# tongxyh/ImageCompression_Adversarial

Measured on AMD Instinct MI355X. Metric: attack-step·images/sec, Balle2018-hyper 768×512 1001-step PGD, 1/2/4/8 GPU, higher is better.
Workload: dtype f32 (fp32-accurate: exact 3-way bf16 operand splits, 6 MFMA products, f32 accumulate); 1 GPU; attack_rd -m hyper -q 3 -att_metric L2 -noise 1e-4, 32 images/GPU of 768x512, steps of the 1001-step loop, x6 conv operands; per_gpu_batch=32, global_batch=32, height=512, width=768, parallelism=image-shard x1 (no data-path collective)

## Files before the change

imagecompression_adversarial_amd/_lib.py:

```python
from __future__ import annotations

import ctypes as C
import os

import torch

_HERE = os.path.dirname(os.path.abspath(__file__))
LIB_PATH = os.environ.get("ICA_HIP_LIB", os.path.join(_HERE, "libica_hip.so"))

_p = C.c_void_p
_i = C.c_int
_l = C.c_long
_f = C.c_float
_sz = C.c_size_t

_SIGS = {
    "ica_conv_it": [_i],
    "ica_pack_conv_weight_size": [_i, _i, _i, _i, _i],
    "ica_pack_conv_weight": [_p, _p, _i, _i, _i, _l, _l, _i, _i, _i, _i, _p],
    "ica_pack_conv_weight_bf16": [_p, _p, _i, _i, _i, _l, _l, _i, _i, _i, _p],
    "ica_pack_conv_weight_bf16_size": [_i, _i, _i, _i],
    "ica_pack_conv_weight_x6": [_p, _p, _i, _i, _i, _l, _l, _i, _i, _p],
    "ica_pack_conv_weight_x6_size": [_i, _i, _i, _i],
    "ica_pack_gdn_x6": [_p, _p, _i, _p],
    "ica_pack_gdn_x6_size": [_i],
    "ica_pack_up3k3_x6_size": [_i],
    "ica_pack_up3k3_x6": [_p, _p, _p, _i, _p],
    "ica_conv_up3k3_x6": [_p, _p, _p, _p, _i, _i, _i, _i, _i, _i, _p],
    "ica_conv_ex": [_p, _p],
    "ica_last_launch": [_p, _i, _p],
    "ica_x6_tiling": [_i],
    "ica_pack_gdn": [_p, _p, _p, _p, _i, _i, _f, _p],
    "ica_pack_gdn_bf16": [_p, _p, _p, _p, _i, _i, _f, _p],
    "ica_pack_up3_size": [_i],
    "ica_pack_up3": [_p, _p, _i, _i, _p],
    "ica_conv_up3": [_p, _p, _p, _p, _i, _i, _i, _i, _i, _i, _p],
    "ica_elem_blocks_per_image": [],
    "ica_nchw_to_nc4": [_p, _p, _i, _i, _i, _i, _p],
    "ica_nc4_to_nchw": [_p, _p, _i, _i, _i, _i, _p],
    "ica_reduce_rows": [_p, _p, _i, _i, _f, _p],
    "ica_attack_prologue": [_p, _p, _p, _p, _i, _i, _i, _f, _p],
    "ica_attack_prologue_ex": [_p, _p, _p, _p, _i, _i, _i, _f, _i, _p],
    "ica_attack_loss": [_p, _p, _p, _p, _i, _i, _i, _f, _i, _i, _p],
    "ica_attack_adam": [_p, _p, _p, _p, _p, _p, _p, _p, _i, _i, _i, _f, _f, _f, _f, _f, _p, _p, _p, _p],
    "ica_attack_adam_ex": [_p, _p, _p, _p, _p, _p, _p, _p, _i, _i, _i, _f, _f, _f, _f, _f, _p, _p, _p, _i, _p],
    "ica_universal_prologue": [_p, _p, _p, _p, _i, _i, _i, _f, _p],
    "ica_universal_adam": [_p, _p, _p, _p, _p, _p, _p, _i, _i, _i, _f, _f, _f, _f, _f, _p, _p, _p],
    "ica_branch_select": [_p, _f, _i, _p, _p, _p],
    "ica_gather_images": [_p, _p, _p, _i, _l, _p],
    "ica_roi_prologue": [_p, _p, _p, _p, _i, _i, _i, _f, _i, _i, _i, _i, _f, _f, _p],
    "ica_roi_loss": [_p, _p, _p, _p, _p, _i, _i, _i, _i, _i, _i, _i, _f, _f, _i, _p],
    "ica_roi_adam": [_p, _p, _p, _p, _p, _p, _p, _i, _i, _i, _f, _f, _f, _f, _p, _i, _i, _i, _i, _f, _f, _p, _p, _p],
    "ica_ifgsm_step": [_p, _p, _p, _p, _p, _i, _i, _i, _f, _f, _i, _p],
    "ica_l1_partial": [_p, _p, _i, _i, _i, _p],
    "ica_cw_gate": [_p, _i, _f, _p, _p, _p, _p, _i, _p],
    "ica_cw_adam": [_p, _p, _p, _p, _p, _p, _p, _i, _i, _i, _f, _f, _p, _i, _p, _i, _p],
    "ica_cw_round": [_p, _p, _p, _p, _p, _p, _i, _i, _i, _i, _p, _p],
    "ica_cw_reset": [_p, _p, _p, _p, _i, _l, _p],
    "ica_gc_likelihood": [_p, _p, _p, _p, _p, _p, _p, _i, _i, _i, _i, _i, _p],
    "ica_eb_likelihood": [_p, _p, _p, _p, _p, _p, _p, _i, _i, _i, _i, _i, _p],
    "ica_pack_eb": [_p, _p, _p, _i, _p],
    "ica_abs": [_p, _p, _l, _p],
    "ica_cast_f32_bf16": [_p, _p, _l, _p],
    "ica_cast_bf16_f32": [_p, _p, _l, _p],
    "ica_flip_rot": [_p, _p, _l, _i, _i, _i, _p],
    "ica_bitdepth": [_p, _p, _l, _f, _p],
    "ica_resample_axis": [_p, _p, _l, _i, _i, _i, _i, _p, _p, _p, _i, _p],
    "ica_bitdepth_noise": [_p, _p, _p, _l, _f, _p],
    "ica_bitdepth_noise_bwd": [_p, _p, _l, _f, _p],
    "ica_add": [_p, _p, _p, _l, _p],
    "ica_ensemble_grad": [_p, _p, _p, _l, _f, _p],
    "ica_latent_range": [_p, _i, _i, _i, _i, _p, _p, _p, _p],
    "ica_latent_clamp": [_p, _p, _p, _p, _i, _i, _i, _i, _p, _p],
    "ica_latent_clamp_bwd": [_p, _p, _p, _p, _i, _i, _i, _i, _p],
    "ica_latent_detect": [_p, _p, _p, _p, _p, _i, _i, _p],
    "ica_latent_distrib_ws_size": [_i, _i, _i, _i, _i],
    "ica_latent_distrib": [_p, _p, _p, _p, _i, _i, _i, _i, _f, _i, _f, _f, _p, _p, _p, _p, _p],
    "ica_layer_sums_blocks": [_i, _i, _i],
    "ica_layer_sums_ws_size": [_i, _i],
    "ica_layer_sums": [_p, _i, _i, _p, _p, _p],
    "ica_rate_gc_blocks": [],
    "ica_rate_eb_blocks": [_i, _i, _i],
    "ica_rate_gc": [_p, _p, _p, _p, _p, _i, _i, _i, _i, _f, _p],
    "ica_rate_eb": [_p, _p, _p, _p, _i, _i, _i, _i, _f, _p],
    "ica_rd_metrics_blocks": [],
    "ica_rd_metrics": [_p, _p, _p, _p, _p, _p, _p, _i, _i, _i, _i, _i, _i, _i, _i, _i, _p],
    "ica_val_metrics": [_p, _p, _p, _p, _p, _p, _i, _i, _i, _i, _i, _i, _i, _i, _i, _p],
    "ica_patch_vi_ws_size": [_i, _i, _i, _i, _i],
    "ica_patch_vi": [_p, _p, _p, _p, _i, _i, _i, _i, _i, _i, _p, _p, _p, _p, _p, _p, _p, _p],
    "ica_patch_gather": [_p, _p, _p, _p, _p, _p, _i, _i, _i, _i, _i, _p],
    "ica_blur_sweep_chunk": [],
    "ica_gauss_blur_ws_size": [_i, _i, _i],
    "ica_gauss_blur": [_p, _p, _p, _i, _i, _i, _i, _i, _i, _p, _p, _p, _p, _p],
    "ica_blur_sweep_ws_size": [_i, _i, _i],
    "ica_blur_sweep": [_p, _p, _p, _i, _i, _i, _i, _i, _i, _f, _i, _p, _l, _p, _p, _p, _p, _p],
    "ica_noise_apply_ws_size": [_i, _i, _i],
    "ica_noise_apply": [_p, _p, _p, _i, _i, _i, _p, _p, _p, _p],
    "ica_jpeg_sweep_chunk": [],
    "ica_jpeg_roundtrip_ws_size": [_i, _i, _i, _i],
    "ica_jpeg_roundtrip": [_p, _p, _i, _i, _i, _i, _p, _p, _p, _p, _p],
    "ica_jpeg_sweep_ws_size": [_i, _i, _i, _i],
    "ica_jpeg_sweep": [_p, _p, _i, _i, _i, _i, _i, _f, _i, _p, _l, _p, _p, _p, _p, _p],
    "ica_transfer_apply_ws_size": [_i, _i, _i, _i],
    "ica_transfer_apply": [_p, _p, _p, _i, _i, _i, _i, _p, _p, _p],
    "ica_transfer_score_ws_size": [_i, _i, _i, _i],
    "ica_transfer_score": [_p, _p, _i, _i, _i, _i, _i, _p, _p, _p],
    "ica_requant8_ws_size": [_i, _i, _i],
    "ica_requant8": [_p, _p, _p, _i, _i, _i, _p, _p, _p, _p, _p, _p, _p, _p, _p],
    "ica_quant8_pack": [_p, _i, _i, _i, _p, _p, _p],
    "ica_floor_bits_ws_size": [_i, _i, _i, _i],
    "ica_floor_bits": [_p, _i, _i, _i, _i, _f, _p, _p, _p],
    "ica_gc_symbols": [_p, _p, _p, _p, _i, _f, _p, _p, _i, _i, _i, _i, _p],
    "ica_eb_symbols": [_p, _p, _p, _p, _i, _i, _i, _i, _p],
    "ica_dequantize": [_p, _p, _p, _p, _i, _i, _i, _i, _p],
    "ica_pmf_to_quantized_cdf": [_p, _i, _i, _p],
    "ica_rans_encode": [_p, _p, _l, _p, _i, _p, _p, _i, _p, _l, _p],
    "ica_rans_decode": [_p, _l, _p, _l, _p, _i, _p, _p, _i, _p],
    "ica_rans_dec_open": [_p, _l, _p],
    "ica_rans_dec_step": [_p, _i, _p, _l, _p, _i, _p, _p, _i, _p, _p],
    "ica_rans_dec_close": [_p],
    "ica_ar_lds_bytes": [_i, _i, _i],
    "ica_ar_step": [_p, _i, _i, _i, _p],
    "ica_round": [_p, _p, _l, _p],
    "ica_clamp01": [_p, _p, _l, _p],
    "ica_sqdiff_partial": [_p, _p, _p, _i, _l, _i, _p],
    "ica_nc4_bound_to_nchw": [_p, _p, _i, _i, _i, _i, _p],
    "ica_bound_bwd_nc4": [_p, _p, _p, _i, _i, _i, _i, _p],
    "ica_msssim_blocks": [_i, _i, _i, _i],
    "ica_msssim_level": [_p, _p, _i, _i, _i, _p, _i, _i, _f, _f, _p, _p, _p, _p, _p],
    "ica_msssim_level_bwd": [_p, _p, _p, _i, _i, _i, _p, _i, _i, _p, _p, _p],
    "ica_msssim_combine": [_p, _i, _i, _i, _p, _p, _p, _p, _p],
    "ica_avgpool2": [_p, _p, _i, _i, _i, _i, _i, _p],
    "ica_avgpool2_bwd": [_p, _p, _i, _i, _i, _i, _i, _p],
    "ica_scale": [_p, _l, _f, _p],
    "ica_wgrad_ws_size": [_i, _i, _i, _i],
    "ica_wgrad_nsplit": [_i, _i, _l],
    "ica_wgrad": [_p, _p, _p, _p, _i, _i, _i, _i, _i, _i, _i, _i, _i, _i, _i, _i, _p],
    "ica_channel_sum": [_p, _p, _i, _i, _i, _i, _i, _p],
    "ica_relu_bwd": [_p, _p, _l, _p],
    "ica_abs_bwd": [_p, _p, _l, _p],
    "ica_gdn_xsq": [_p, _p, _p, _l, _p],
    "ica_lrelu_bwd": [_p, _p, _p, _l, _p],
    "ica_gdn_t": [_p, _p, _p, _p, _l, _i, _p],
    "ica_reparam_bwd": [_p, _p, _p, _l, _f, _i, _p],
    "ica_bpp_grad": [_p, _p, _l, _f, _p],
    "ica_gc_bwd": [_p, _p, _p, _p, _p, _i, _i, _i, _i, _p],
    "ica_eb_bwd": [_p, _p, _p, _p, _p, _i, _i, _i, _i, _p],
    "ica_eb_param_scatter": [_p, _p, _p, _i, _p],
    "ica_mse_grad": [_p, _p, _p, _i, _i, _i, _f, _p],
}
_RESTYPES = {"ica_pack_conv_weight_size": _sz, "ica_pack_conv_weight_bf16_size": _sz,
             "ica_pack_conv_weight_x6_size": _sz, "ica_pack_gdn_x6_size": _sz, "ica_pack_up3k3_x6_size": _sz, "ica_pack_up3_size": _sz, "ica_wgrad_ws_size": _sz,
             "ica_rans_encode": _l, "ica_ar_lds_bytes": _sz, "ica_patch_vi_ws_size": _sz,
             "ica_gauss_blur_ws_size": _sz, "ica_blur_sweep_ws_size": _sz, "ica_noise_apply_ws_size": _sz,
             "ica_transfer_apply_ws_size": _sz, "ica_transfer_score_ws_size": _sz,
             "ica_requant8_ws_size": _sz, "ica_floor_bits_ws_size": _sz, "ica_latent_distrib_ws_size": _sz,
             "ica_layer_sums_ws_size": _sz, "ica_jpeg_roundtrip_ws_size": _sz, "ica_jpeg_sweep_ws_size": _sz}



class ConvArgs(C.Structure):
    _fields_ = ([(n, C.c_void_p) for n in ("x", "y", "wp", "bias", "gp", "beta", "save_x", "save_s", "in_x", "in_s",
                                            "save_t", "res", "mask")]
                + [(n, C.c_int) for n in ("N", "Cin", "Hin", "Win", "Cout", "Hout", "Wout", "kind", "KS", "S", "epi",
                                           "it", "fill_mode", "ps", "prec", "layout", "order")])


class ArArgs(C.Structure):
    _fields_ = ([(n, C.c_void_p) for n in ("y", "params", "yhat", "sym", "idx", "sym_in", "means", "wc", "bc", "w1",
                                            "b1", "w2", "b2", "w3", "b3", "table")]
                + [("T", C.c_int), ("bound", C.c_float)]
                + [(n, C.c_int) for n in ("B", "M", "H", "W", "E1", "E2")])


class LayerDesc(C.Structure):
    _fields_ = [(n, C.c_void_p) for n in ("a", "b", "c")] + [(n, C.c_int) for n in ("C", "H", "W", "mode")]


_lib = None


def lib():
    global _lib
    if _lib is None:
        if not os.path.exists(LIB_PATH):
            raise RuntimeError(
                f"libica_hip.so not found at {LIB_PATH}: build it with "
                "`python -c 'import __graft_entry__ as g; g.build()'` (hipcc, gfx950). "
                "There is no CPU/PyTorch fallback for the hot path.")
        L = C.CDLL(LIB_PATH)
        for name, args in _SIGS.items():
            fn = getattr(L, name)
            fn.argtypes = args
            fn.restype = _RESTYPES.get(name, _i)
        _lib = L
    return _lib


def exported_symbols():
    return list(_SIGS)


def call(name, *args):
    rc = getattr(lib(), name)(*args)
    if rc != 0:
        raise RuntimeError(f"{name} failed with status {rc}")
    return rc


def ptr(t):
    return None if t is None else C.c_void_p(t.data_ptr())


def stream():
    return C.c_void_p(torch.cuda.current_stream().cuda_stream)
```

imagecompression_adversarial_amd/attack.py:

```python
from __future__ import annotations

import math
import os
import time
from dataclasses import dataclass, field

import torch

from . import dist as D
from . import hip_ops as K
from . import msssim as MS
from ._lib import call, ptr, stream
from .engine import CodecKernels


ATTACK_GRAPH = os.environ.get("ICA_ATTACK_GRAPH", "1") != "0"
GRAPH_STATS = {"captures": 0, "replays": 0}


def _lr_table(steps, lr):
    out, cur, sch = [], lr, 0
    period = max(steps // 3, 1)
    for i in range(steps):
        out.append(cur)
        if i % period == 0:
            sch += 1
            if sch in (1, 2, 3):
                cur = cur * 0.33
    return out


@dataclass
class AttackResult:
    im_adv: torch.Tensor
    output_adv: torch.Tensor
    output_s: torch.Tensor
    bpp_ori: torch.Tensor
    bpp: torch.Tensor
    mse_in: torch.Tensor
    mse_out: torch.Tensor
    msim_in: torch.Tensor | None
    msim_out: torch.Tensor | None
    vi: list = field(default_factory=list)
    vi_msim: list = field(default_factory=list)
    noise: torch.Tensor | None = None
    branches: list = field(default_factory=list)
    output_t: torch.Tensor | None = None
    tar_mse: torch.Tensor | None = None


def eval_forward(kern: CodecKernels, x: torch.Tensor, clamp=True):
    B, _, H, W = x.shape
    res = kern.forward(K.to_nc4(x))
    out = torch.empty_like(x)
    call("ica_nc4_bound_to_nchw", ptr(res["x_hat4"]), ptr(out), B, H, W, int(clamp), stream())
    return out, K.bits_to_bpp(res["sumlog"], H * W)


def padded_eval_forward(kern: CodecKernels, x: torch.Tensor, pad: int, mode="reflect"):
    import torch.nn.functional as F
    B, _, H, W = x.shape
    xp = F.pad(x, (pad, pad, pad, pad), mode=mode).contiguous()
    Hp, Wp = xp.shape[2:]
    if Hp % 64 or Wp % 64:
        raise ValueError(f"-p {pad}: the padded size {Hp}x{Wp} must be a multiple of 64 (the codec's latent grid; "
                         "the reference's crop fails otherwise)")
    out_p, bpp_p = eval_forward(kern, xp, True)
    out = out_p[:, :, pad:pad + H, pad:pad + W].contiguous()
    return out, bpp_p * (Hp * Wp / (H * W))


def evaluate(kern, im_in, im_s, output_s, clamp=True, adv=False, msssim=True):
    im_ = K.clamp01(im_in) if clamp else im_in
    out, bpp = eval_forward(kern, im_, clamp)
    mse_in = K.sqdiff_mean(im_, im_s)
    mse_out = K.sqdiff_mean(out, output_s)
    msim_in = msim_out = None
    if msssim:
        msim_in = MS.ms_ssim_per_image(im_, im_s)
        msim_out = MS.ms_ssim_per_image(out, output_s)
    vi, vi_msim = [], []
    mi_l, mo_l = mse_in.tolist(), mse_out.tolist()
    si_l = msim_in.tolist() if msssim else [None] * len(mi_l)
    so_l = msim_out.tolist() if msssim else [None] * len(mi_l)
    for mi, mo, si, so in zip(mi_l, mo_l, si_l, so_l):
        v = vm = None
        if mi > 1e-20 and mo > 1e-20:
            v = 10.0 * math.log10(mo / mi)
            if not adv and si is not None and si < 0.9999:
                vm = 10.0 * math.log10((1 - so) / (1 - si))
        vi.append(v)
        vi_msim.append(vm)
    return im_, out, bpp, mse_in, mse_out, msim_in, msim_out, vi, vi_msim


class AttackLoop:

    def __init__(self, kern: CodecKernels, im_s: torch.Tensor, steps=1001, epsilon=16.0, noise_thr=1e-4,
                 lr=0.01, att_metric="L2", clamp=True, init_noise=None, coupled=False, group=None,
                 target=None, roi=None, la_tar=1.0, la_bkg_in=1.0, la_bkg_out=1.0, pad=None, padding_mode="reflect"):
        if att_metric not in ("L2", "ms-ssim"):
            raise ValueError(f"att_metric {att_metric!r} not supported (reference: L2, ms-ssim)")
        if target is not None and (att_metric != "L2" or coupled):
            raise NotImplementedError("the targeted / ROI attack is defined for att_metric L2, per-image")
        self.kern = kern
        self.im_s = im_s.contiguous()
        B, C, H, W = im_s.shape
        assert C == 3
        self.B, self.H, self.W = B, H, W
        self.steps, self.eps, self.thr = steps, float(epsilon) / 255.0, float(noise_thr)
        self.metric, self.clamp = att_metric, clamp
        self.invN = float(1.0 / (3 * H * W))
        self.coupled, self.group = coupled, group
        self.B_global = D.global_count(B, im_s.device, group) if coupled else B
        self.gscale = float(1.0 / (self.B_global * 3 * H * W)) if coupled else self.invN
        self.dval = 1.0 / self.B_global if coupled else 1.0
        dev = im_s.device
        self.clamp_in = bool(getattr(kern, "clamp_input", True))
        if init_noise is not None:
            self.noise = init_noise.clone().contiguous()
        elif not self.clamp_in:
            r = float(noise_thr) ** 0.5
            self.noise = torch.empty(tuple(im_s.shape)).uniform_(-r, r).to(dev)
        else:
            self.noise = torch.zeros_like(self.im_s)
        if target is not None and not self.clamp_in:
            raise NotImplementedError("the targeted / ROI attack is defined for the clamped-input models")
        self.m = torch.zeros_like(self.im_s)
        self.v = torch.zeros_like(self.im_s)
        self.im_in4 = K.empty_nc4(B, 3, H, W, dev)
        self.part = torch.empty(B * K.blocks_per_image(), device=dev)
        self.loss_i = torch.empty(B, device=dev)
        self.grad4 = K.empty_nc4(B, 3, H, W, dev)
        self.branch = torch.zeros(B, dtype=torch.int32, device=dev)
        self.im_in = torch.empty_like(self.im_s)
        self.lrs = _lr_table(steps, lr)
        self.t = 0
        self.compact = True
        self.sel = torch.zeros(B + 1, dtype=torch.int32, device=dev)
        self.gpos = torch.zeros(B, dtype=torch.int32, device=dev)
        self.sel_host = torch.zeros(B + 1, dtype=torch.int32).pin_memory() if dev.type == "cuda" else None
        self._sel_ev = torch.cuda.Event() if dev.type == "cuda" else None
        self._sel_pending = False
        self.census = torch.zeros(B, dtype=torch.int32, device=dev)
        self.steps_done = 0
        self.sync_steps = 0
        self.sync_wait_s = 0.0
        self.graph_ok = (ATTACK_GRAPH and dev.type == "cuda" and att_metric == "L2"
                         and type(self).network_grad is AttackLoop.network_grad)
        self._graph, self._graph_out = None, None
        self.graph_replays = 0
        if pad:
            self.output_s, self.bpp_ori = padded_eval_forward(kern, self.im_s, int(pad), padding_mode)
        else:
            self.output_s, self.bpp_ori = eval_forward(kern, self.im_s, clamp)
        self.output_s4 = None
        self.roi = None
        if target is not None:
            t = target.to(self.im_s.device).contiguous()
            if t.shape[0] == 1 and B > 1:
                t = t.expand(B, -1, -1, -1).contiguous()
            if t.shape != self.im_s.shape:
                raise ValueError(f"target {tuple(t.shape)} must match the source batch {tuple(self.im_s.shape)}")
            self.output_t, _ = eval_forward(kern, t, True)
            self.roi = roi_weights(H, W, roi, la_tar, la_bkg_in, la_bkg_out)

    def _adam_scalars(self, i):
        t = i + 1
        bc1 = 1 - 0.9 ** t
        bc2 = 1 - 0.999 ** t
        step_size = self.lrs[i] / bc1
        return float(bc2 ** 0.5), float(-step_size)

    def _select(self):
        B = self.B
        if not self.compact:
            return B, None
        call("ica_branch_select", ptr(self.loss_i), self.thr, B, ptr(self.sel), ptr(self.gpos), stream())
        prev_all = False
        if self._sel_pending:
            self._sel_ev.synchronize()
            prev_all = int(self.sel_host[0]) == B
            self._sel_pending = False
        self.sel_host.copy_(self.sel, non_blocking=True)
        self._sel_ev.record()
        if prev_all and (self.metric == "L2" or self.roi is not None):
            self._sel_pending = True
            return B, None
        t0 = time.perf_counter()
        self._sel_ev.synchronize()
        self.sync_wait_s += time.perf_counter() - t0
        self.sync_steps += 1
        E = int(self.sel_host[0])
        if E == B:
            self._sel_pending = True
            return B, None
        return E, self.sel[1:1 + E]

    def _gather(self, x, idx, E):
        if idx is None:
            return x
        per = x[0].numel()
        out = torch.empty((E,) + tuple(x.shape[1:]), dtype=x.dtype, device=x.device)
        call("ica_gather_images", ptr(x), ptr(out), ptr(idx), E, per, stream())
        return out

    def network_grad(self, idx=None, E=None):
        kern = self.kern
        H, W = self.H, self.W
        Bn = self.B if idx is None else E
        im4 = self._gather(self.im_in4, idx, Bn)
        out_s = self._gather(self.output_s, idx, Bn)
        grad4, part = self.grad4[:Bn], self.part[:Bn * K.blocks_per_image()]
        y4, sa = kern.g_a(im4, save=True)
        del im4
        xh4, ss = kern.g_s(y4, save=True)
        del y4
        if self.roi is not None:
            x0, x1, y0, y1, _, _, wot, wob = self.roi
            out_t = self._gather(self.output_t, idx, Bn)
            call("ica_roi_loss", ptr(xh4), ptr(out_s), ptr(out_t), ptr(grad4), ptr(part),
                 Bn, H, W, x0, x1, y0, y1, wot, wob, int(self.clamp), stream())
        elif self.metric == "L2":
            call("ica_attack_loss", ptr(xh4), ptr(out_s), ptr(grad4), ptr(part), Bn, H, W,
                 self.gscale, int(self.clamp), 0, stream())
        else:
            out = torch.empty_like(out_s)
            call("ica_nc4_bound_to_nchw", ptr(xh4), ptr(out), Bn, H, W, int(self.clamp), stream())
            ones = torch.full((Bn,), self.dval, device=out.device)
            _, gout, _ = MS.ms_ssim_value_and_grad(out, out_s, ones)
            call("ica_bound_bwd_nc4", ptr(xh4), ptr(gout), ptr(grad4), Bn, H, W, int(self.clamp), stream())
        gy4 = kern.g_s_backward(grad4, ss)
        del ss, xh4
        return kern.g_a_backward(gy4, sa)

    def _network_graph(self):
        if self._graph is None:
            hooks = (K.EVENT_HOOK, K.LAUNCH_HOOK)
            K.EVENT_HOOK = K.LAUNCH_HOOK = None
            g = torch.cuda.CUDAGraph()
            try:
                with torch.cuda.graph(g, capture_error_mode="relaxed"):
                    out = self.network_grad(None, self.B)
            finally:
                K.EVENT_HOOK, K.LAUNCH_HOOK = hooks
            self._graph, self._graph_out = g, out
            GRAPH_STATS["captures"] += 1
        self._graph.replay()
        self.graph_replays += 1
        GRAPH_STATS["replays"] += 1
        return self._graph_out

    def step(self, i, record_im_in=False, census=False):
        B, H, W = self.B, self.H, self.W
        if self.roi is not None:
            return self._step_roi(i, record_im_in, census)
        call("ica_attack_prologue_ex", ptr(self.noise), ptr(self.im_s), ptr(self.im_in4), ptr(self.part), B, H, W,
             self.eps, int(self.clamp_in), stream())
        K.reduce_rows(self.part, B, self.invN, out=self.loss_i)
        if self.coupled:
            D.couple_loss_i(self.loss_i, self.B_global, self.group)
        E, idx = self._select()
        if E == B and idx is None and self.graph_ok:
            gx4 = self._network_graph()
        else:
            gx4 = self.network_grad(idx, E) if E > 0 else None
        cheap_grad = None
        if self.metric == "ms-ssim" and E < B:
            im_in = torch.empty_like(self.im_s)
            call("ica_nc4_bound_to_nchw", ptr(self.im_in4), ptr(im_in), B, H, W, 0, stream())
            _, _, gY = MS.ms_ssim_value_and_grad(self.im_s, im_in, torch.full((B,), -self.dval, device=im_in.device))
            cheap_grad = gY
        bc2s, neg_step = self._adam_scalars(i)
        call("ica_attack_adam_ex", ptr(self.noise), ptr(self.im_s), ptr(gx4), ptr(self.loss_i), ptr(cheap_grad),
             ptr(self.m), ptr(self.v), ptr(self.im_in if record_im_in else None), B, H, W, self.eps, self.thr,
             self.gscale, bc2s, neg_step, ptr(self.branch), ptr(self.gpos if idx is not None else None),
             ptr(self.census), int(self.clamp_in), stream())
        self.steps_done += 1
        if census:
            return self.branch.tolist()
        return None

    def _step_roi(self, i, record_im_in, census):
        B, H, W = self.B, self.H, self.W
        x0, x1, y0, y1, wit, wib, _, _ = self.roi
        call("ica_roi_prologue", ptr(self.noise), ptr(self.im_s), ptr(self.im_in4), ptr(self.part), B, H, W,
             self.eps, x0, x1, y0, y1, wit, wib, stream())
        K.reduce_rows(self.part, B, 1.0, out=self.loss_i)
        E, idx = self._select()
        if E == B and idx is None and self.graph_ok:
            gx4 = self._network_graph()
        else:
            gx4 = self.network_grad(idx, E) if E > 0 else None
        bc2s, neg_step = self._adam_scalars(i)
        call("ica_roi_adam", ptr(self.noise), ptr(self.im_s), ptr(gx4), ptr(self.loss_i), ptr(self.m), ptr(self.v),
             ptr(self.im_in if record_im_in else None), B, H, W, self.eps, self.thr, bc2s, neg_step,
             ptr(self.branch), x0, x1, y0, y1, wit, wib, ptr(self.gpos if idx is not None else None),
             ptr(self.census), stream())
        self.steps_done += 1
        if census:
            return self.branch.tolist()
        return None

    def expensive_image_steps(self):
        return self.B * self.steps_done - int(self.census.sum())

    def run(self, record=False):
        branches = []
        for i in range(self.steps):
            br = self.step(i, record_im_in=(i == self.steps - 1), census=record)
            if record:
                branches.append(br)
        return branches


def roi_weights(H, W, roi, la_tar=1.0, la_bkg_in=1.0, la_bkg_out=1.0):
    x0, x1, y0, y1 = (0, W, 0, H) if roi is None else (int(v) for v in roi)
    x0, x1 = max(0, min(x0, W)), max(0, min(x1, W))
    y0, y1 = max(0, min(y0, H)), max(0, min(y1, H))
    area = max(x1 - x0, 0) * max(y1 - y0, 0)
    if area == 0:
        raise ValueError(f"empty ROI {roi} for a {W}x{H} image")
    cnt_t, cnt_b = 3.0 * area, 3.0 * (H * W - area)
    wb = (lambda la: float(la / cnt_b) if cnt_b > 0 else 0.0)
    return (x0, x1, y0, y1, float(1.0 / cnt_t), wb(la_bkg_in), float(la_tar / cnt_t), wb(la_bkg_out))


def roi_mse(a, b, roi4):
    x0, x1, y0, y1 = roi4
    d = (a - b)[:, :, y0:y1, x0:x1]
    return (d * d).flatten(1).mean(1)


def attack_batch(kern: CodecKernels, im_s, steps=1001, epsilon=16.0, noise_thr=1e-4, lr=0.01, att_metric="L2",
                 clamp=True, init_noise=None, eval_msssim=True, record=False, coupled=False,
                 group=None, target=None, roi=None, la_tar=1.0, la_bkg_in=1.0, la_bkg_out=1.0, pad=None,
                 padding_mode="reflect") -> AttackResult:
    loop = AttackLoop(kern, im_s, steps, epsilon, noise_thr, lr, att_metric, clamp, init_noise, coupled, group,
                      target, roi, la_tar, la_bkg_in, la_bkg_out, pad, padding_mode)
    branches = loop.run(record=record)
    im_, out, bpp, mse_in, mse_out, msim_in, msim_out, vi, vi_msim = evaluate(
        kern, loop.im_in, loop.im_s, loop.output_s, clamp, adv=False, msssim=eval_msssim)
    res = AttackResult(im_adv=im_, output_adv=out, output_s=loop.output_s, bpp_ori=loop.bpp_ori, bpp=bpp,
                       mse_in=mse_in, mse_out=mse_out, msim_in=msim_in, msim_out=msim_out, vi=vi, vi_msim=vi_msim,
                       noise=loop.noise, branches=branches)
    if loop.roi is not None:
        res.output_t = loop.output_t
        res.tar_mse = roi_mse(out, loop.output_t, loop.roi[:4])
    return res


RATE_MODELS = ("hyper", "factorized")


def rate_attack_guard(model=None, precision=None, att_metric="L2", coupled=False, target=None, roi=None):
    if coupled:
        raise NotImplementedError("the rate attack is per-image: the batch-coupled semantics belong to the "
                                  "adversarial fine-tune's distortion attack")
    if target is not None or roi is not None:
        raise NotImplementedError("the rate attack has no target / ROI form: its loss is the whole image's bitrate")
    if att_metric != "L2":
        raise NotImplementedError(f"the rate attack's input budget is the L2 one (att_metric {att_metric!r}): its "
                                  "cheap branch is the L2 input loss, its expensive branch uses no image metric")
    if precision == "bf16":
        raise NotImplementedError("the rate attack runs fp32 / x6 operands: the entropy models read an fp32 latent")
    if model is not None and model not in RATE_MODELS:
        raise NotImplementedError(f"the rate attack covers {RATE_MODELS}, not {model!r}: the rounding inside the "
                                  "context models (and the debug model's mean-scale prior) has no stated relaxation")


class RateAttackLoop(AttackLoop):

    def __init__(self, kern: CodecKernels, im_s: torch.Tensor, steps=1001, epsilon=16.0, noise_thr=1e-4, lr=0.01,
                 att_metric="L2", clamp=True, init_noise=None, coupled=False, group=None, target=None, roi=None,
                 pad=None, padding_mode="reflect"):
        model = kern.model if isinstance(kern, CodecKernels) else type(kern).__name__
# ... 86 lines not shown
```

imagecompression_adversarial_amd/csrc/ica_conv.hip:

```cpp
#include <cxxabi.h>

#include <algorithm>
#include <cstdio>
#include <cstdlib>
#include <type_traits>

#include "ica_conv_epi.h"

#define ICA_WLOAD_BF(w, it, g) ((w)[(it) * 64])

template <int IT, int KH>
ICA_DEV void load_frag(float (&a)[IT][KH], const float* w) {
#pragma unroll
  for (int it = 0; it < IT; ++it) {
    if constexpr (KH == 8) {
      const f32x4 w0 = ld4(w + it * 64 * KH), w1 = ld4(w + it * 64 * KH + 4);
#pragma unroll
      for (int e = 0; e < 4; ++e) {
        a[it][e] = w0[e];
        a[it][4 + e] = w1[e];
      }
    } else {
      const f32x2 w0 = *reinterpret_cast<const f32x2*>(w + it * 64 * KH);
      a[it][0] = w0[0];
// ... 1132 lines not shown
        }
#pragma unroll
        for (int it = 0; it < 3; ++it) {
          const float* wt = wl + ((size_t)it * nch + ch) * 512;
          const f32x4 w0 = ld4(wt), w1 = ld4(wt + 4);
#pragma unroll
          for (int e = 0; e < 4; ++e) {
            a[it][e] = w0[e];
            a[it][4 + e] = w1[e];
          }
        }
      };
      auto compute = [&](const f32x4& v0, const f32x4& v1, const float (&a)[3][8]) {
        const float b[8] = {v0[0], v0[1], v0[2], v0[3], v1[0], v1[1], v1[2], v1[3]};
#pragma unroll
        for (int s2 = 0; s2 < 8; ++s2)
#pragma unroll
          for (int it = 0; it < 3; ++it) acc[it] = mfma32(a[it][s2], b[s2], acc[it]);
      };
      f32x4 pa0, pa1, pb0, pb1;
      float aa[3][8], ab[3][8];
      load(0, pa0, pa1, aa);
      int ch = 0;
#pragma unroll 1
      for (; ch + 1 < nch; ch += 2) {
        load(ch + 1, pb0, pb1, ab);
        compute(pa0, pa1, aa);
        load(min(ch + 2, nch - 1), pa0, pa1, aa);
        compute(pb0, pb1, ab);
      }
      if (ch < nch) compute(pa0, pa1, aa);
    }
    if (q < T3_NPX) {
#pragma unroll
      for (int it = 0; it < 3; ++it)
#pragma unroll
        for (int r = 0; r < 16; ++r) {
          const int row = it * 32 + acc_row(r, h);
          if (row < T3_ROWS) zs[row * T3_NPX + q] = acc[it][r];
        }
    }
  }
gather:
  __syncthreads();
  const int al = threadIdx.x / T3_TW, bl = threadIdx.x % T3_TW;
  const int a = a0 + al, b = b0 + bl;
  if (al >= T3_TH || a >= p.Hin || b >= p.Win) return;
  const float bias0 = p.bias ? p.bias[0] : 0.f, bias1 = p.bias ? p.bias[1] : 0.f, bias2 = p.bias ? p.bias[2] : 0.f;
#pragma unroll
  for (int py = 0; py < 2; ++py) {
#pragma unroll
    for (int px = 0; px < 2; ++px) {
      float o0 = 0.f, o1 = 0.f, o2 = 0.f;
#pragma unroll
      for (int ky = py; ky < 5; ky += 2) {
#pragma unroll
        for (int kx = px; kx < 5; kx += 2) {
          const int dy = (py + 2 - ky) / 2, dx = (px + 2 - kx) / 2;
          const int q = (al + 1 + dy) * T3_HC + (bl + 1 + dx);
          const int tap = ky * 5 + kx;
          o0 += zs[(0 * 25 + tap) * T3_NPX + q];
          o1 += zs[(1 * 25 + tap) * T3_NPX + q];
          o2 += zs[(2 * 25 + tap) * T3_NPX + q];
        }
      }
      const int y = 2 * a + py, x = 2 * b + px;
      if (y < p.Hout && x < p.Wout)
        st4(p.y + (((size_t)n * p.Hout + y) * p.Wout + x) * 4, f32x4{o0 + bias0, o1 + bias1, o2 + bias2, 0.f});
    }
  }
}

constexpr int U3_OW = 30, U3_HW = 32;
template <int CT>
constexpr int u3_rows() { return 4 * CT - 2; }
template <int CT>
constexpr int u3_npx() { return 4 * CT * U3_HW; }

template <int NCH, int CT, bool BF = false>
__global__ __launch_bounds__(256, 1) void conv_up3_x6p_kernel(ConvParams p) {
  constexpr int R = u3_rows<CT>(), NPX = u3_npx<CT>();
  __shared__ float zs[T3_ROWS * NPX];
  const int tiles_x = (p.Win + U3_OW - 1) / U3_OW, tiles_y = (p.Hin + R - 1) / R;
  const int total = tiles_x * tiles_y * p.N;
  const int nb = (int)(gridDim.x >> 3), xcd = (int)(blockIdx.x & 7), bi = (int)(blockIdx.x >> 3);
  const int q8 = total >> 3, r8 = total & 7;
  const int t_end = xcd * q8 + min(xcd, r8) + q8 + (xcd < r8 ? 1 : 0);
  const int t_begin = xcd * q8 + min(xcd, r8) + bi;
  if (t_begin >= t_end) return;
  const int lane = threadIdx.x & 63, h = lane >> 5, j = lane & 31;
  const int wave = __builtin_amdgcn_readfirstlane(threadIdx.x >> 6);
  const int Cin4 = p.Cin >> 2;
  const unsigned plane = (unsigned)p.Hin * p.Win;
  auto coords = [&](int t, int& n, int& a0, int& b0) {
    const int tx = t % tiles_x, r = t / tiles_x;
    a0 = (r % tiles_y) * R;
    b0 = tx * U3_OW;
    n = r / tiles_y;
  };
  const bool split_in = (p.pl & PL_IN) != 0;
  constexpr unsigned QB = BF ? 8u : 16u;
  const unsigned qs = plane * QB, cs = 4u * qs;
  constexpr unsigned OOB = 0xFFFFFFF0u;
  auto prep = [&](int t, bool real, __amdgpu_buffer_rsrc_t& r, unsigned (&vb)[CT]) __attribute__((always_inline)) {
    int n, a0, b0;
    coords(real ? t : t_begin, n, a0, b0);
    r = uniform_rsrc(reinterpret_cast<const char*>(p.x) + (size_t)n * Cin4 * plane * QB, (unsigned)(Cin4 * plane * QB));
    const int ix = b0 - 1 + j;
#pragma unroll
    for (int ct = 0; ct < CT; ++ct) {
      const int iy = a0 - 1 + wave + 4 * ct;
      const bool ok = real && iy >= 0 && iy < p.Hin && ix >= 0 && ix < p.Win;
      vb[ct] = ok ? ((unsigned)(2 * h) * plane + pix_at(iy, ix, p.Hin, p.Win, split_in)) * QB : OOB;
    }
  };
  f32x4 xa[CT][NCH][BF ? 1 : 2];
  auto load = [&](const __amdgpu_buffer_rsrc_t& r, const unsigned (&vb)[CT], int ct, int ch)
      __attribute__((always_inline)) {
    const bool ok = vb[ct] != OOB;
    const unsigned o = vb[ct] + (unsigned)ch * cs;
    if constexpr (BF) {
      const u32x2 lo = __builtin_bit_cast(u32x2, __builtin_amdgcn_raw_buffer_load_b64(r, ok ? o : OOB, 0, 0));
      const u32x2 hi = __builtin_bit_cast(u32x2, __builtin_amdgcn_raw_buffer_load_b64(r, ok ? o + qs : OOB, 0, 0));
      xa[ct][ch][0] = __builtin_bit_cast(f32x4, (u32x4_t){lo[0], lo[1], hi[0], hi[1]});
    } else {
      xa[ct][ch][0] = __builtin_bit_cast(f32x4, __builtin_amdgcn_raw_buffer_load_b128(r, ok ? o : OOB, 0, 0));
      xa[ct][ch][BF ? 0 : 1] = __builtin_bit_cast(f32x4, __builtin_amdgcn_raw_buffer_load_b128(r, ok ? o + qs : OOB, 0, 0));
    }
  };
  __amdgpu_buffer_rsrc_t rn;
  unsigned vbn[CT];
  prep(t_begin, true, rn, vbn);
#pragma unroll
  for (int ct = 0; ct < CT; ++ct)
#pragma unroll
    for (int ch = 0; ch < NCH; ++ch) load(rn, vbn, ct, ch);
  constexpr long pst = 3L * NCH * 64;
  constexpr int NPL = BF ? 1 : 3;
  const __amdgpu_buffer_rsrc_t wr = uniform_rsrc(p.wp, (unsigned)(NPL * pst * 16));
  int wz = 0;
  auto ldw = [&](bf16x8 (&a)[3][3], int ch) {
#pragma unroll
    for (int it = 0; it < 3; ++it)
#pragma unroll
      for (int q = 0; q < NPL; ++q) a[it][q] = ld_bf8(wr, lane * 16, wz + (int)((q * pst + ((long)it * NCH + ch) * 64) * 16));
  };
  auto split = [&](int ct, int ch, bf16x8 (&b)[3]) __attribute__((always_inline)) {
    if constexpr (BF) {
      b[0] = f4_as_bf8(xa[ct][ch][0]);
    } else {
      const float v[8] = {xa[ct][ch][0][0], xa[ct][ch][0][1], xa[ct][ch][0][2], xa[ct][ch][0][3],
                          xa[ct][ch][BF ? 0 : 1][0], xa[ct][ch][BF ? 0 : 1][1], xa[ct][ch][BF ? 0 : 1][2],
                          xa[ct][ch][BF ? 0 : 1][3]};
      split3x8(v, b);
    }
  };
  const float bias0 = p.bias ? p.bias[0] : 0.f, bias1 = p.bias ? p.bias[1] : 0.f, bias2 = p.bias ? p.bias[2] : 0.f;
#pragma unroll 1
  for (int t = t_begin; t < t_end; t += nb) {
    wz = 0;
    asm volatile("" : "+s"(wz));
    prep(t + nb, t + nb < t_end, rn, vbn);
    f32x16 acc[CT][3];
#pragma unroll
    for (int ct = 0; ct < CT; ++ct)
#pragma unroll
      for (int it = 0; it < 3; ++it) acc[ct][it] = f32x16{0};
    bf16x8 wa[2][3][3];
    ldw(wa[0], 0);
    bf16x8 bc[3];
    split(0, 0, bc);
#pragma unroll
    for (int ch = 0; ch < NCH; ++ch) {
      if (ch + 1 < NCH) ldw(wa[(ch + 1) & 1], ch + 1);
      __builtin_amdgcn_sched_barrier(0);
#pragma unroll
      for (int ct = 0; ct < CT; ++ct) {
        const int nct = ct + 1 < CT ? ct + 1 : 0, nch = ct + 1 < CT ? ch : ch + 1;
        bf16x8 bn[3];
        if (nch < NCH) split(nct, nch, bn);
#pragma unroll
// ... 459 lines not shown
        case EPI_RELU: return launch_up<5, 4, EPI_RELU, 0>(p, st);
        case EPI_LRELU: return launch_up<5, 4, EPI_LRELU, 0>(p, st);
        case EPI_GDN: return launch_up<5, 4, EPI_GDN, 0>(p, st);
        case EPI_IGDN: return launch_up<5, 4, EPI_IGDN, 0>(p, st);
        case EPI_GDN_BWD: return launch_up<5, 4, EPI_GDN_BWD, 0>(p, st);
        case EPI_IGDN_BWD: return launch_up<5, 4, EPI_IGDN_BWD, 0>(p, st);
        default: return -5;
      }
    }
    return -3;
  }
  if (epi != EPI_BIAS || (fx & ~FX_RES) != 0) return -4;
  if (KS == 3) {
    if (fx == 0) {
      if (it == 1) return launch_up<3, 1, EPI_BIAS, 0>(p, st);
      if (it == 4) return launch_up<3, 4, EPI_BIAS, 0>(p, st);
      if (it == 6) return launch_up<3, 6, EPI_BIAS, 0>(p, st);
    } else {
      if (it == 1) return launch_up<3, 1, EPI_BIAS, FX_RES>(p, st);
      if (it == 4) return launch_up<3, 4, EPI_BIAS, FX_RES>(p, st);
      if (it == 6) return launch_up<3, 6, EPI_BIAS, FX_RES>(p, st);
    }
    return -3;
  }
  if (KS == 1) {
    if (fx != 0) return -4;
    if (it == 1) return launch_up<1, 1, EPI_BIAS, 0>(p, st);
    if (it == 4) return launch_up<1, 4, EPI_BIAS, 0>(p, st);
    if (it == 6) return launch_up<1, 6, EPI_BIAS, 0>(p, st);
    return -3;
  }
  return -6;
}

int ica_conv_x6_dispatch(const ConvParams& p, int kind, int KS, int S, int it, int epi, int fx, int order,
                         hipStream_t st);
int ica_rgb5_bf16_dispatch(const ConvParams& p, int epi, hipStream_t st);
int ica_pack_rgb5_planes(const float* w, void* dst, int O, int C, long so, long sc, int it, int planes, hipStream_t st);

extern "C" {
#ifdef ICA_CLOCK_STAMP
int ica_diag_stamp_buffer(unsigned long long* buf, unsigned slots) {
  if (hipMemcpyToSymbol(HIP_SYMBOL(ica_stamp_buf), &buf, sizeof(buf)) != hipSuccess) return -1;
  if (hipMemcpyToSymbol(HIP_SYMBOL(ica_stamp_slots), &slots, sizeof(slots)) != hipSuccess) return -1;
  return 0;
}
#endif

int ica_last_launch(char* name, int cap, unsigned long long* threads) {
  const IcaLaunchRec r = ica_launch_rec();
  ica_launch_rec() = IcaLaunchRec{nullptr, 0, 0};
  if (!r.fn) return 0;
  if (threads) *threads = r.threads;
  if (name && cap > 0) {
    const char* m = hipKernelNameRefByPtr(r.fn, nullptr);
    int st = -1;
    char* d = m ? abi::__cxa_demangle(m, nullptr, nullptr, &st) : nullptr;
    const char* src = (st == 0 && d) ? d : (m ? m : "");
    std::snprintf(name, (size_t)cap, "%s", src);
    std::free(d);
  }
  return r.count;
}

typedef struct ica_conv_args {
  const float* x;
  float* y;
  const float* wp;
  const float* bias;
  const float* gp;
  const float* beta;
  float* save_x;
  float* save_s;
  const float* in_x;
  const float* in_s;
  float* save_t;
  const float* res;
  const float* mask;
  int N, Cin, Hin, Win, Cout, Hout, Wout;
  int kind, KS, S, epi, it, fill_mode, ps;
  int prec;
  int layout;
  int order;
} ica_conv_args;

int ica_conv_it(int cout) {
  if (cout <= 32) return 1;
  if (cout % 128 == 0) return 4;
  if (cout % 96 == 0) return 3;
  return 4;
}

static inline int resolve_it(int O, int it) { return it > 0 ? it : ica_conv_it(O); }

size_t ica_pack_conv_weight_size(int O, int C, int KS, int CC, int it) {
  const int IT = resolve_it(O, it);
  const int ncb = (O + IT * 32 - 1) / (IT * 32);
  const int C4 = (C + 3) / 4, nch = (C4 * 4 + CC - 1) / CC;
  return (size_t)ncb * nch * KS * KS * IT * 64 * (CC / 2);
}

int ica_pack_conv_weight(const float* w, float* dst, int O, int C, int KS, long so, long sc, int CC, int order,
                         int flip, int it, hipStream_t st) {
  const int IT = resolve_it(O, it);
  const long total = (long)ica_pack_conv_weight_size(O, C, KS, CC, IT);
  ICA_LAUNCH(pack_conv_kernel<float>, dim3((total + 255) / 256), dim3(256), 0, st, w, dst, O, C, KS, so, sc,
                     IT, CC, order, total, flip);
  ICA_CHECK_LAUNCH();
  return 0;
}

__global__ void pack_conv_tg_kernel(const float* __restrict__ w, __bf16* __restrict__ dst, int O, int C, int KS,
                                    long so, long sc, int IT, long total, int flip) {
  const long i = (long)blockIdx.x * blockDim.x + threadIdx.x;
  if (i >= total) return;
  const int KK = KS * KS, TG = (KK + 3) / 4;
  long t = i;
  const int s = t % 8; t /= 8;
  const int lane = t % 64; t /= 64;
  const int it = t % IT; t /= IT;
  const int tg = t % TG; t /= TG;
  const int cb = (int)t;
  const int o = cb * IT * 32 + it * 32 + (lane & 31);
  const int tap = 4 * tg + 2 * (lane >> 5) + (s >> 2), c = s & 3;
  float v = 0.f;
  if (o < O && c < C && tap < KK) {
    const int wt = flip ? KK - 1 - tap : tap;
    v = w[o * so + c * sc + (wt / KS) * KS + (wt % KS)];
  }
  dst[i] = (__bf16)v;
}

size_t ica_pack_conv_weight_bf16_size(int O, int C, int KS, int it) {
  if (C > 4) return ica_pack_conv_weight_size(O, C, KS, 16, it);
  const int IT = resolve_it(O, it);
  const int ncb = (O + IT * 32 - 1) / (IT * 32);
  return (size_t)ncb * ((KS * KS + 3) / 4) * IT * 64 * 8;
}

int ica_pack_conv_weight_bf16(const float* w, void* dst, int O, int C, int KS, long so, long sc, int order, int flip,
                              int it, hipStream_t st) {
  const int IT = resolve_it(O, it);
  if (C <= 4) {
    if (order == 2) {
      if (KS != 5 || flip) return -4;
      return ica_pack_rgb5_planes(w, dst, O, C, so, sc, IT, 1, st);
    }
    if (order != 0) return -4;
    const long tot = (long)ica_pack_conv_weight_bf16_size(O, C, KS, IT);
    ICA_LAUNCH(pack_conv_tg_kernel, dim3((tot + 255) / 256), dim3(256), 0, st, w, reinterpret_cast<__bf16*>(dst),
                       O, C, KS, so, sc, IT, tot, flip);
    ICA_CHECK_LAUNCH();
    return 0;
  }
  const long total = (long)ica_pack_conv_weight_size(O, C, KS, 16, IT);
  ICA_LAUNCH(pack_conv_kernel<__bf16>, dim3((total + 255) / 256), dim3(256), 0, st, w,
                     reinterpret_cast<__bf16*>(dst), O, C, KS, so, sc, IT, 16, order, total, flip);
  ICA_CHECK_LAUNCH();
  return 0;
}

size_t ica_pack_up3_size(int Cin) { return (size_t)3 * (Cin / 16) * 64 * 8; }

int ica_pack_up3(const float* w, void* dst, int Cin, int prec, hipStream_t st) {
  if (Cin % 16 != 0) return -2;
  if (prec < 0 || prec > 2) return -4;
  const long total = (long)ica_pack_up3_size(Cin);
  const dim3 grid((total + 255) / 256), block(256);
  if (prec == 0) {
    ICA_LAUNCH(pack_up3_kernel<float>, grid, block, 0, st, w, reinterpret_cast<float*>(dst), Cin, total);
  } else if (prec == 1) {
    ICA_LAUNCH(pack_up3_kernel<__bf16>, grid, block, 0, st, w, reinterpret_cast<__bf16*>(dst), Cin, total);
  } else {
    ICA_LAUNCH(pack_up3_x6_kernel, grid, block, 0, st, w, reinterpret_cast<__bf16*>(dst), Cin, total);
  }
  ICA_CHECK_LAUNCH();
  return 0;
}

static int up3_layout_ok(int layout, int Hin, int Win) {
  if (layout & ~PL_IN) return -4;
  if ((layout & PL_IN) && ((Hin | Win) & 1)) return -2;
  return 0;
}

int ica_conv_up3(const float* x, float* y, const void* wp, const float* bias, int N, int Cin, int Hin, int Win,
                 int layout, int prec, hipStream_t st) {
  if (Cin % 16 != 0) return -2;
  if (const int rc = up3_layout_ok(layout, Hin, Win)) return rc;
  if (prec < 0 || prec > 2) return -4;
  ConvParams p{x, y, reinterpret_cast<const float*>(wp), bias, nullptr, nullptr, nullptr, nullptr, nullptr, nullptr,
               N, Cin, Hin, Win, 3, 2 * Hin, 2 * Win, nullptr};
  p.pl = layout;
  auto tiled = [&](auto kern) {
    const int tiles = ((Win + T3_TW - 1) / T3_TW) * ((Hin + T3_TH - 1) / T3_TH) * N;
    ICA_LAUNCH(kern, dim3(tiles), dim3(256), 0, st, p);
  };
  auto persistent = [&](auto kern, int R) {
    const int tiles = ((Win + U3_OW - 1) / U3_OW) * ((Hin + R - 1) / R) * N;
    const int nb = std::max(1, std::min((tiles + 7) / 8, ica_cu_count() / 8));
    ICA_LAUNCH(kern, dim3(8 * nb), dim3(256), 0, st, p);
  };
  if (prec == 0) {
    tiled(conv_up3_kernel<false>);
  } else if (prec == 2) {
    if (Cin == 128) persistent(conv_up3_x6p_kernel<8, 3>, u3_rows<3>());
    else if (Cin == 192) persistent(conv_up3_x6p_kernel<12, 2>, u3_rows<2>());
    else tiled(conv_up3_kernel<false, true>);
  } else {
    if (Cin == 128) persistent(conv_up3_x6p_kernel<8, 3, true>, u3_rows<3>());
    else tiled(conv_up3_kernel<true>);
  }
  ICA_CHECK_LAUNCH();
  return 0;
}

__global__ void pack_gdn_bf16_kernel(const float* __restrict__ gamma, const float* __restrict__ beta,
                                     __bf16* __restrict__ gp, float* __restrict__ beta_eff, int C, int transpose,
                                     float beta_bound) {
  const int T = C / 32;
  const long total = (long)T * T * 2048;
  const long i = (long)blockIdx.x * blockDim.x + threadIdx.x;
  const float ped = 1.4551915228366852e-11f;
  const float gbound = 3.814697265625e-06f;
  if (i < total) {
    long t = i;
    const int j = t % 8; t /= 8;
    const int lane = t % 64; t /= 64;
    const int hl = t % 2; t /= 2;
    const int s = t % 2; t /= 2;
    const int b = t % T; t /= T;
    const int a = (int)t;
    const int row = a * 32 + (lane & 31), col = b * 32 + 16 * s + 8 * (j >> 2) + 4 * (lane >> 5) + (j & 3);
    const int gi = transpose ? (col * C + row) : (row * C + col);
    const float g0 = fmaxf(gamma[gi], gbound);
    const float g = fsub_rn(fmul_rn(g0, g0), ped);
    __bf16 hi, lo;
    split_bf(g, hi, lo);
    gp[i] = hl ? lo : hi;
  }
  if (i < C) {
    const float bb = fmaxf(beta[i], beta_bound);
    beta_eff[i] = fsub_rn(fmul_rn(bb, bb), ped);
  }
}

int ica_pack_gdn_bf16(const float* gamma, const float* beta, void* gpb, float* beta_eff, int C, int transpose,
                      float beta_bound, hipStream_t st) {
  if (C % 32 != 0) return -2;
  const long total = (long)(C / 32) * (C / 32) * 2048;
  ICA_LAUNCH(pack_gdn_bf16_kernel, dim3((total + 255) / 256), dim3(256), 0, st, gamma, beta,
                     reinterpret_cast<__bf16*>(gpb), beta_eff, C, transpose, beta_bound);
  ICA_CHECK_LAUNCH();
  return 0;
}

int ica_pack_gdn(const float* gamma, const float* beta, float* gp, float* beta_eff, int C, int transpose,
                 float beta_bound, hipStream_t st) {
  if (C % 32 != 0) return -2;
  const long total = (long)(C / 32) * (C / 32) * 64 * 16;
  ICA_LAUNCH(pack_gdn_kernel, dim3((total + 255) / 256), dim3(256), 0, st, gamma, beta, gp, beta_eff, C,
                     transpose, beta_bound);
  ICA_CHECK_LAUNCH();
  return 0;
}

int ica_conv_ex(const ica_conv_args* a, hipStream_t st) {
  ConvParams p{a->x,    a->y,    a->wp,   a->bias, a->gp,   a->beta, a->save_x, a->save_s, a->in_x, a->in_s,
               a->N,    a->Cin,  a->Hin,  a->Win,  a->Cout, a->Hout, a->Wout,   a->save_t, a->res,  a->mask,
               a->fill_mode, a->ps, a->prec, a->layout};
  if (a->prec < 0 || a->prec > 3) return -4;
  if (a->layout & ~(PL_IN | PL_OUT)) return -4;
  if (a->layout && (a->KS != 5 || a->S != 2 || a->fill_mode != 0 || a->ps)) return -4;
  if (((a->layout & PL_IN) && ((a->Hin | a->Win) & 1)) || ((a->layout & PL_OUT) && ((a->Hout | a->Wout) & 1)))
    return -2;
  const int it = resolve_it(a->Cout, a->it);
  if (a->epi >= EPI_GDN && a->epi <= EPI_IGDN_BWD && a->Cout != it * 32) return -4;
  if (a->ps && (a->Cout % 16 != 0 || !(a->epi == EPI_BIAS || a->epi == EPI_RELU || a->epi == EPI_LRELU))) return -4;
  if (a->fill_mode == 1 && !a->mask) return -4;
  if (a->fill_mode == 2 && a->Cin % 16 != 0) return -2;
  if (a->epi == EPI_LRELU_BWD && !a->in_x) return -4;
  const int fx = ((a->res || a->save_x) ? FX_RES : 0) | (a->ps ? FX_PS : 0) | (a->fill_mode == 1 ? FX_MASK : 0) |
                 (a->fill_mode == 2 ? FX_UNSHUF : 0) | (a->save_t ? FX_T : 0);
  const int want = a->kind == 1 ? ORDER_UP : ORDER_DOWN;
  if (a->prec == 2) {
    if (a->kind == 0 && a->KS == 3)
      return a->order == want ? pick_x6o<3>(p, a->kind, a->KS, a->S, a->epi, it, fx, st) : -4;
    return ica_conv_x6_dispatch(p, a->kind, a->KS, a->S, it, a->epi, fx, a->order, st);
  }
  if (a->prec == 3) return a->order == want ? pick_x6o<1>(p, a->kind, a->KS, a->S, a->epi, it, fx, st) : -4;
  if (a->prec == 1 && a->order == ORDER_RGB5) {
    if (a->kind != 0 || a->KS != 5 || a->S != 2 || it != 4 || fx != 0 || a->fill_mode != 0 ||
        !(a->epi == EPI_BIAS || a->epi == EPI_GDN || a->epi == EPI_IGDN_BWD))
      return -4;
    return ica_rgb5_bf16_dispatch(p, a->epi, st);
  }
  if (a->order != (a->prec == 1 && a->kind == 0 && a->Cin <= 4 ? ORDER_TG : want)) return -4;
  if (a->kind == 0) return pick_down(p, a->KS, a->S, it, a->epi, fx, st);
  if (a->kind == 1) return a->S == 2 ? pick_up(p, a->KS, it, a->epi, fx, st) : -6;
  return -6;
}

}
```

imagecompression_adversarial_amd/csrc/ica_conv_epi.h:

```cpp
#pragma once
#include "ica_common.h"

enum {
  EPI_BIAS = 0,
  EPI_RELU = 1,
  EPI_GDN = 2,
  EPI_IGDN = 3,
  EPI_GDN_BWD = 4,
  EPI_IGDN_BWD = 5,
  EPI_LRELU = 6,
  EPI_LRELU_BWD = 7,
};
enum { FX_RES = 1, FX_PS = 2, FX_MASK = 4, FX_UNSHUF = 8, FX_T = 16 };

struct ConvParams {
  const float* x;
  float* y;
  const float* wp;
  const float* bias;
  const float* gp;
  const float* beta;
  float* save_x;
  float* save_s;
  const float* in_x;
  const float* in_s;
  int N, Cin, Hin, Win, Cout, Hout, Wout;
  float* save_t;
  const float* res;
  const float* mask;
  int fill_mode;
  int ps;
  int prec;
  int pl;
};
enum { PL_IN = 1, PL_OUT = 2 };
enum { ORDER_DOWN = 0, ORDER_UP = 1, ORDER_RGB5 = 2, ORDER_TG = 3 };

ICA_DEV void split3(f32x4 v, u32x2& hi, u32x2& mid, u32x2& lo) {
  bf16x4 a, b, c;
#pragma unroll
  for (int e = 0; e < 4; ++e) {
    const __bf16 h = (__bf16)v[e];
    const float r1 = v[e] - (float)h;
    const __bf16 m = (__bf16)r1;
    const float r2 = r1 - (float)m;
    a[e] = h;
    b[e] = m;
    c[e] = (__bf16)r2;
  }
  hi = __builtin_bit_cast(u32x2, a);
  mid = __builtin_bit_cast(u32x2, b);
  lo = __builtin_bit_cast(u32x2, c);
}

ICA_DEV f32x16 mfma_x6(const bf16x8 (&a)[3], const bf16x8 (&b)[3], f32x16 c) {
  c = mfma32bf(a[2], b[0], c);
  c = mfma32bf(a[0], b[2], c);
  c = mfma32bf(a[1], b[1], c);
  c = mfma32bf(a[1], b[0], c);
  c = mfma32bf(a[0], b[1], c);
  c = mfma32bf(a[0], b[0], c);
  return c;
}
template <int NPL>
ICA_DEV f32x16 mfma_np(const bf16x8 (&a)[3], const bf16x8 (&b)[3], f32x16 c) {
  if constexpr (NPL == 1) return mfma32bf(a[0], b[0], c);
  else return mfma_x6(a, b, c);
}

ICA_DEV __amdgpu_buffer_rsrc_t chan_rsrc(const float* v, int C) { return uniform_rsrc(v, v ? (unsigned)((C + 3) & ~3) * 4u : 0u); }
ICA_DEV f32x4 ld_chan4(__amdgpu_buffer_rsrc_t r, int c0) {
  return __builtin_bit_cast(f32x4, __builtin_amdgcn_raw_buffer_load_b128(r, c0 * 4, 0, 0));
}

ICA_DEV void split3x8(const float (&v)[8], bf16x8 (&o)[3]) {
  u32x2 a0, b0, c0, a1, b1, c1;
  split3(f32x4{v[0], v[1], v[2], v[3]}, a0, b0, c0);
  split3(f32x4{v[4], v[5], v[6], v[7]}, a1, b1, c1);
  o[0] = __builtin_bit_cast(bf16x8, u32x4_t{a0[0], a0[1], a1[0], a1[1]});
  o[1] = __builtin_bit_cast(bf16x8, u32x4_t{b0[0], b0[1], b1[0], b1[1]});
  o[2] = __builtin_bit_cast(bf16x8, u32x4_t{c0[0], c0[1], c1[0], c1[1]});
}

template <int EPI>
constexpr bool epi_gdn() { return EPI == EPI_GDN || EPI == EPI_IGDN || EPI == EPI_GDN_BWD || EPI == EPI_IGDN_BWD; }
template <int IT, int EPI>
constexpr int epi_lds_entries() { return 16 * IT + (epi_gdn<EPI>() ? IT * IT * 128 : 0); }

template <int IT, int EPI>
ICA_DEV void epi_params_to_lds(const ConvParams& p, f32x4* lp, int co_base) {
  constexpr int NG = epi_gdn<EPI>() ? IT * IT * 128 : 0, NP = 16 * IT;
  constexpr int NI = (NP + NG + 255) / 256;
  const __amdgpu_buffer_rsrc_t brs = chan_rsrc(p.bias, p.Cout);
  const __amdgpu_buffer_rsrc_t ers = chan_rsrc((EPI == EPI_GDN || EPI == EPI_IGDN) ? p.beta : nullptr, p.Cout);
  const __amdgpu_buffer_rsrc_t grs = uniform_rsrc(epi_gdn<EPI>() ? p.gp : nullptr, epi_gdn<EPI>() ? IT * IT * 4096 : 0);
  f32x4 v[NI];
#pragma unroll
  for (int i = 0; i < NI; ++i) {
    const int e = threadIdx.x + 256 * i;
    if (e < 8 * IT) v[i] = ld_chan4(brs, co_base + 4 * e);
    else if (e < NP) v[i] = ld_chan4(ers, 4 * (e - 8 * IT));
    else if (e < NP + NG) {
      const int k = (e - NP) >> 6, l = (e - NP) & 63;
      v[i] = __builtin_bit_cast(f32x4, __builtin_amdgcn_raw_buffer_load_b128(grs, k * 2048 + l * 16, 0, 0));
    } else {
      v[i] = f32x4{0.f, 0.f, 0.f, 0.f};
    }
  }
#pragma unroll
  for (int i = 0; i < NI; ++i) {
    const int e = threadIdx.x + 256 * i;
    if (e < NP + NG) lp[e] = v[i];
  }
}

ICA_DEV unsigned pix_at(int y, int x, int H, int W, bool split) {
  return split ? ((unsigned)((((y & 1) << 1) | (x & 1)) * (H >> 1) + (y >> 1))) * (unsigned)(W >> 1) + (x >> 1)
               : (unsigned)y * W + x;
// ... 885 lines not shown
```

imagecompression_adversarial_amd/csrc/ica_conv_x6.hip:

```cpp
#include <algorithm>
#include <atomic>
#include <type_traits>

#include "ica_conv_epi.h"

namespace {

constexpr int X6_PT = 2;
constexpr int XD_TW = 32;
template <int PT, int CS = 1>
constexpr int xd_th() { return CS == 1 ? 4 * PT : 4; }
template <int PT, int CS = 1>
constexpr int xd_tw() { return CS == 1 ? XD_TW : 16 * PT; }

template <int IT, int EPI, int PT = X6_PT, int CS = 1>
__global__ __launch_bounds__(256, 1) void conv_down_x6_kernel(ConvParams p, long ps) {
  ICA_STAMP_BEGIN();
  static_assert(CS == 1 || (CS == 2 && EPI == EPI_BIAS), "conv_down_x6 over two channel blocks: bias epilogue only");
  constexpr int KS = 5, S = 2, PAD = 2, KK = 25, TW = xd_tw<PT, CS>(), TH = xd_th<PT, CS>();
  constexpr int PR = S * (TH - 1) + KS, PC = S * (TW - 1) + KS, PLANE = PR * PC;
  constexpr int NF = (4 * PLANE + 255) / 256, NB = (NF + 1) / 2;
  __shared__ f32x4 patch[3 * 2 * PLANE];
  const int tiles_x = (p.Wout + TW - 1) / TW, tiles_y = (p.Hout + TH - 1) / TH;
  int bid, cb;
  xcd_block<true>(bid, cb);
  const int tx = bid % tiles_x;
  bid /= tiles_x;
  const int ty = bid % tiles_y;
  const int n = bid / tiles_y;
  const int lane = threadIdx.x & 63, wave = threadIdx.x >> 6, h = lane >> 5, j = lane & 31;
  if constexpr (CS == 2) cb = __builtin_amdgcn_readfirstlane(wave >> 1);
  auto trow = [&](int t) { return CS == 1 ? wave * PT + t : 2 * (wave & 1) + (j >> 4); };
  auto tcol = [&](int t) { return CS == 1 ? j : 16 * t + (j & 15); };
  const int oy0 = ty * TH, ox0 = tx * TW;
  const int iy0 = oy0 * S - PAD, ix0 = ox0 * S - PAD;
  const int Cin4 = (p.Cin + 3) >> 2, nch = (Cin4 * 4 + 15) / 16;
  f32x16 acc[PT][IT];
#pragma unroll
  for (int t = 0; t < PT; ++t)
#pragma unroll
    for (int it = 0; it < IT; ++it) acc[t][it] = f32x16{0};

  const unsigned xplane = (unsigned)p.Hin * p.Win;
  const __amdgpu_buffer_rsrc_t xr =
      uniform_rsrc(reinterpret_cast<const char*>(p.x) + (size_t)n * Cin4 * xplane * 16, Cin4 * xplane * 16u);
  u32x2* p2 = reinterpret_cast<u32x2*>(patch);
  auto batch = [&](int ch, int i0, f32x4 (&v)[NB]) {
#pragma unroll
    for (int i = 0; i < NB; ++i) {
      const int e = threadIdx.x + 256 * (i0 + i);
      const int q = e / PLANE, rem = e - q * PLANE, pr = rem / PC, pc = rem - pr * PC;
      const int iy = iy0 + pr, ix = ix0 + pc, c4 = ch * 4 + q;
      const bool ok = i0 + i < NF && e < 4 * PLANE && c4 < Cin4 && iy >= 0 && iy < p.Hin && ix >= 0 && ix < p.Win;
      const unsigned vo = ((unsigned)c4 * xplane + pix_at(iy, ix, p.Hin, p.Win, p.pl & PL_IN)) * 16u;
      v[i] = __builtin_bit_cast(f32x4, __builtin_amdgcn_raw_buffer_load_b128(xr, ok ? vo : 0xFFFFFFF0u, 0, 0));
    }
  };
  auto put = [&](int i0, const f32x4 (&v)[NB]) {
#pragma unroll
    for (int i = 0; i < NB; ++i) {
      const int e = threadIdx.x + 256 * (i0 + i);
      if (i0 + i < NF && e < 4 * PLANE) {
        const int q = e / PLANE, pix = e - q * PLANE;
        u32x2 a, b, c;
        split3(v[i], a, b, c);
        const int ent = (q >> 1) * PLANE + pix;
        p2[(0 * 2 * PLANE + ent) * 2 + (q & 1)] = a;
        p2[(1 * 2 * PLANE + ent) * 2 + (q & 1)] = b;
        p2[(2 * 2 * PLANE + ent) * 2 + (q & 1)] = c;
      }
    }
  };
  const int total = nch * KK;
  const __amdgpu_buffer_rsrc_t wr = uniform_rsrc(p.wp, (unsigned)(3 * ps * 16));
  const int wbase = cb * total * IT * 64;
  auto ldw = [&](bf16x8 (&a)[IT][3], int g) {
    const int f = wbase + min(g, total - 1) * IT * 64;
#pragma unroll
    for (int it = 0; it < IT; ++it)
#pragma unroll
      for (int q = 0; q < 3; ++q) a[it][q] = ld_bf8(wr, lane * 16, (int)((q * ps + f + it * 64) * 16));
  };
  auto step = [&](bf16x8 (&cur)[IT][3], bf16x8 (&nxt)[IT][3], int g, int tap, auto hook) __attribute__((always_inline)) {
    ldw(nxt, g + 1);
    hook();
    __builtin_amdgcn_sched_barrier(0);
    const int ky = tap / 5, kx = tap - ky * 5;
#pragma unroll
    for (int t = 0; t < PT; ++t) {
      const int o = h * PLANE + (S * trow(t) + ky) * PC + S * tcol(t) + kx;
      const bf16x8 b[3] = {f4_as_bf8(patch[o]), f4_as_bf8(patch[2 * PLANE + o]), f4_as_bf8(patch[4 * PLANE + o])};
#pragma unroll
      for (int it = 0; it < IT; ++it) acc[t][it] = mfma_x6(cur[it], b, acc[t][it]);
    }
  };
  auto none = []() {};
  constexpr int TPF = 20;
  f32x4 v1[NB], v2[NB];
  auto chunk = [&](bf16x8 (&fa)[IT][3], bf16x8 (&fb)[IT][3], int ch) __attribute__((always_inline)) {
    batch(ch, NB, v2);
    __syncthreads();
    put(0, v1);
    put(NB, v2);
    __syncthreads();
    const int g0 = ch * KK, cn = min(ch + 1, nch - 1);
#pragma unroll 1
    for (int tp = 0; tp < TPF; tp += 2) {
      step(fa, fb, g0 + tp, tp, none);
      step(fb, fa, g0 + tp + 1, tp + 1, none);
    }
    step(fa, fb, g0 + TPF, TPF, [&]() { batch(cn, 0, v1); });
#pragma unroll
// ... 146 lines not shown
        const int itg = chh * ITW + it;
        f32x4 yq[4], sq[4];
#pragma unroll
        for (int g = 0; g < 4; ++g) {
          yq[g] = IX.ld(vl[t], (unsigned)(itg * 8 + 2 * g) * plane);
          sq[g] = IS.ld(vl[t], (unsigned)(itg * 8 + 2 * g) * plane);
        }
#pragma unroll
        for (int g = 0; g < 4; ++g) {
          f32x4 tv;
#pragma unroll
          for (int e = 0; e < 4; ++e) {
            const float sg = sq[g][e], rs = __builtin_amdgcn_rcpf(sg), xs = yq[g][e] * rs;
            const float gx = acc[t][it][4 * g + e] * xs;
            tv[e] = (EPI == EPI_GDN_BWD) ? (-0.5f * gx) * (sg * sg * sg) : (0.5f * gx) * rs;
            float gs = acc[t][it][4 * g + e] * sg;
            asm volatile("" : "+v"(gs));
            acc[t][it][4 * g + e] = gs;
          }
          xch(wave, t, it, g) = tv;
        }
      }
    __syncthreads();
#pragma unroll
    for (int il = 0; il < ITW; ++il) {
      const int jt = chh * ITW + il;
      __builtin_amdgcn_sched_barrier(0);
      f32x16 ux[PT];
#pragma unroll
      for (int t = 0; t < PT; ++t) ux[t] = f32x16{0};
      bf16x8 ga[2][3];
      ldg(ga[0], jt, 0);
#pragma unroll
      for (int k = 0; k < 2 * IT; ++k) {
        if (k + 1 < 2 * IT) ldg(ga[(k + 1) & 1], jt, k + 1);
        __builtin_amdgcn_sched_barrier(0);
        const int itg = k >> 1, s = k & 1, hw = itg / ITW, ilk = itg - hw * ITW;
#pragma unroll
        for (int t = 0; t < PT; ++t) {
          const f32x4 a = xch(hw == chh ? wave : (wave ^ 4), t, ilk, 2 * s),
                      b = xch(hw == chh ? wave : (wave ^ 4), t, ilk, 2 * s + 1);
          const float v[8] = {a[0], a[1], a[2], a[3], b[0], b[1], b[2], b[3]};
          bf16x8 tq[3];
          split3x8(v, tq);
          ux[t] = mfma_x6(ga[k & 1], tq, ux[t]);
        }
      }
      __builtin_amdgcn_sched_barrier(0);
#pragma unroll
      for (int t = 0; t < PT; ++t) {
        if (!ok[t]) continue;
#pragma unroll
        for (int g = 0; g < 4; ++g) {
          const unsigned ss = (unsigned)(jt * 8 + 2 * g) * plane;
          const f32x4 yv = IX.ld(vo[t], ss), sv = IS.ld(vo[t], ss);
          f32x4 o;
#pragma unroll
          for (int e = 0; e < 4; ++e) {
            float x2 = 2.0f * (yv[e] * __builtin_amdgcn_rcpf(sv[e]));
            asm volatile("" : "+v"(x2));
            o[e] = acc[t][il][4 * g + e] + x2 * ux[t][4 * g + e];
          }
          Y.st(vo[t], ss, o);
        }
      }
    }
  }
}
}


template <int EPI, int PT>
__global__ __launch_bounds__(512, 1) void conv_down_x6w_kernel(ConvParams p, long ps2) {
  ICA_STAMP_BEGIN();
  constexpr int IT = 4, ITW = 2, KS = 5, S = 2, PAD = 2, TW = 32, TH = 4 * PT, NS = XW_NS;
  constexpr int PR = S * (TH - 1) + KS, PC = S * (TW - 1) + KS, PLANE = PR * PC;
  constexpr int PCE = (PC + 1) / 2;
  constexpr int NF = (2 * PLANE + 511) / 512;
  constexpr int BUF = 3 * PLANE;
  constexpr int XCH = 8 * PT * ITW * 4 * 64;
  __shared__ f32x4 lds[(2 * BUF > XCH) ? 2 * BUF : XCH];
  const int tiles_x = (p.Wout + TW - 1) / TW, tiles_y = (p.Hout + TH - 1) / TH;
  int bid, cb;
  xcd_block<true>(bid, cb);
  const int tx = bid % tiles_x;
  bid /= tiles_x;
  const int ty = bid % tiles_y;
  const int n = bid / tiles_y;
  const int lane = threadIdx.x & 63, h = lane >> 5, j = lane & 31;
  const int wave = __builtin_amdgcn_readfirstlane(threadIdx.x >> 6);
  const int rp = wave & 3, chh = wave >> 2;
  const int oy0 = ty * TH, ox0 = tx * TW;
  const int iy0 = oy0 * S - PAD, ix0 = ox0 * S - PAD;
  const int Cin4 = (p.Cin + 3) >> 2, nch = (Cin4 + 1) >> 1;
  const unsigned xplane = (unsigned)p.Hin * p.Win;
  const __amdgpu_buffer_rsrc_t xr =
      uniform_rsrc(reinterpret_cast<const char*>(p.x) + (size_t)n * Cin4 * xplane * 16, Cin4 * xplane * 16u);
  u32x2* l2 = reinterpret_cast<u32x2*>(lds);
  auto fill_load = [&](int ch, f32x4 (&v)[NF]) {
#pragma unroll
    for (int i = 0; i < NF; ++i) {
      const int e = threadIdx.x + 512 * i;
      const int q = e >= PLANE ? 1 : 0, pix = e - q * PLANE, pr = pix / PC, pc = pix - pr * PC;
      const int iy = iy0 + pr, ix = ix0 + pc, c4 = 2 * ch + q;
      const bool ok = e < 2 * PLANE && c4 < Cin4 && iy >= 0 && iy < p.Hin && ix >= 0 && ix < p.Win;
      const unsigned vo = ((unsigned)c4 * xplane + pix_at(iy, ix, p.Hin, p.Win, p.pl & PL_IN)) * 16u;
      v[i] = __builtin_bit_cast(f32x4, __builtin_amdgcn_raw_buffer_load_b128(xr, ok ? vo : 0xFFFFFFF0u, 0, 0));
    }
  };
  auto fill_put = [&](int buf, const f32x4 (&v)[NF]) {
#pragma unroll
    for (int i = 0; i < NF; ++i) {
      const int e = threadIdx.x + 512 * i;
      if (e < 2 * PLANE) {
        const int q = e >= PLANE ? 1 : 0, pix = e - q * PLANE, pr = pix / PC, pc = pix - pr * PC;
        u32x2 a, b, c;
        split3(v[i], a, b, c);
        const int ent = buf * BUF + xw_pos(pr, pc);
        l2[(ent + 0 * PLANE) * 2 + q] = a;
        l2[(ent + 1 * PLANE) * 2 + q] = b;
        l2[(ent + 2 * PLANE) * 2 + q] = c;
      }
    }
  };
  const int total = (nch >> 1) * 25 + (nch & 1) * NS;
  const __amdgpu_buffer_rsrc_t wr = uniform_rsrc(p.wp, (unsigned)(3 * ps2 * 16));
  const int wbase = cb * total * IT * 64 + chh * ITW * 64;
  auto ldw = [&](bf16x8 (&a)[3], int g, int it) {
    const int f = wbase + min(g, total - 1) * IT * 64 + it * 64;
#pragma unroll
    for (int q = 0; q < 3; ++q) a[q] = ld_bf8(wr, lane * 16, (int)((q * ps2 + f) * 16));
  };
  auto ldb = [&](bf16x8 (&b)[PT][3], int buf, int s) {
    const int tap = min(2 * s + h, KS * KS - 1);
    const int ky = tap / KS, kx = tap - ky * KS;
#pragma unroll
    for (int t = 0; t < PT; ++t) {
      const int o = buf * BUF + (S * (PT * rp + t) + ky) * PC + (kx & 1) * PCE + j + (kx >> 1);
      b[t][0] = f4_as_bf8(lds[o]);
      b[t][1] = f4_as_bf8(lds[o + PLANE]);
      b[t][2] = f4_as_bf8(lds[o + 2 * PLANE]);
    }
  };
  f32x16 acc[PT][ITW];
#pragma unroll
  for (int t = 0; t < PT; ++t)
#pragma unroll
    for (int it = 0; it < ITW; ++it) acc[t][it] = f32x16{0};
  bf16x8 w[ITW][3], bq[2][PT][3];
  f32x4 v[NF];
  auto mm = [&](const bf16x8 (&b)[PT][3], int g) __attribute__((always_inline)) {
#pragma unroll
    for (int it = 0; it < ITW; ++it) {
      __builtin_amdgcn_sched_barrier(0);
#pragma unroll
      for (int t = 0; t < PT; ++t) acc[t][it] = mfma_x6(w[it], b[t], acc[t][it]);
      ldw(w[it], g + 1, it);
    }
    __builtin_amdgcn_sched_barrier(0);
  };
  auto run12 = [&](int buf, int g0, bool put, int pbuf) __attribute__((always_inline)) {
    ldb(bq[0], buf, 0);
#pragma unroll
    for (int s = 0; s < 12; ++s) {
      if (s + 1 < 12) ldb(bq[(s + 1) & 1], buf, s + 1);
      mm(bq[s & 1], g0 + s);
      if (s == 3 && chh == 0 && put) fill_put(pbuf, v);
      if (s == 8 && chh == 1 && put) fill_put(pbuf, v);
    }
  };
  fill_load(0, v);
// ... 194 lines not shown
#pragma unroll
          for (int e = 0; e < 4; ++e) {
            const float nv = nx[4 * g + e];
            const float sc = (EPI == EPI_GDN) ? __builtin_amdgcn_rsqf(nv) : __builtin_amdgcn_sqrtf(nv);
            sv[e] = sc;
            yv[e] = acc[ct][4 * g + e] * sc;
          }
          const unsigned ss = (unsigned)(ct * 8 + 2 * g) * plane;
          if (p.save_s) SS.st(vo, ss, sv);
          Y.st(vo, ss, yv);
        }
      }
    }
  }
}

template <int EPI>
ICA_DEV void rgb5_epi_bwd(const ConvParams& p, const char* lds, f32x16 (&acc)[RGB5_IT], int n, int oy, int ox,
                          bool valid, const f32x4 (&yq)[RGB5_IT][4], const f32x4 (&sq)[RGB5_IT][4]) {
  constexpr int IT = RGB5_IT;
  const int lane = threadIdx.x & 63, h = lane >> 5;
  const unsigned plane = (unsigned)p.Hout * p.Wout;
  const size_t img = (size_t)((p.Cout + 3) >> 2) * plane;
  const Img4 Y(p.y, img, n);
  const unsigned vo = valid ? h * plane + pix_at(oy, ox, p.Hout, p.Wout, p.pl & PL_OUT) : 0u;
  f32x16 xx[IT];
  bf16x8 tq[IT][2][3];
  float tw[8];
#pragma unroll
  for (int it = 0; it < IT; ++it)
#pragma unroll
    for (int g = 0; g < 4; ++g) {
      const f32x4 yv = yq[it][g], sv = sq[it][g];
#pragma unroll
      for (int e = 0; e < 4; ++e) {
        const float sg = sv[e], rs = __builtin_amdgcn_rcpf(sg), xs = yv[e] * rs;
        const float gx = acc[it][4 * g + e] * xs;
        tw[4 * (g & 1) + e] = (EPI == EPI_GDN_BWD) ? (-0.5f * gx) * (sg * sg * sg) : (0.5f * gx) * rs;
        float gs = acc[it][4 * g + e] * sg;
        float x2 = 2.0f * xs;
        asm volatile("" : "+v"(gs), "+v"(x2));
        acc[it][4 * g + e] = gs;
        xx[it][4 * g + e] = x2;
      }
      if (g & 1) split3x8(tw, tq[it][g >> 1]);
    }
  const char* gl = lds + RGB5_W_BYTES;
  f32x16 ux[IT];
#pragma unroll
  for (int jt = 0; jt < IT; ++jt) ux[jt] = f32x16{0};
  __builtin_amdgcn_sched_barrier(0);
  bf16x8 ga[2][3];
  auto ldg = [&](bf16x8 (&a)[3], int r) {
    const int k = r / IT, jt = r % IT;
#pragma unroll
    for (int pl = 0; pl < 3; ++pl)
      a[pl] = lds_frag(gl, (((jt * IT + (k >> 1)) * 2 + (k & 1)) * 1024) + pl * IT * IT * 2048 + lane * 16);
  };
  ldg(ga[0], 0);
#pragma unroll
  for (int r = 0; r < 2 * IT * IT; ++r) {
    if (r + 1 < 2 * IT * IT) ldg(ga[(r + 1) & 1], r + 1);
    __builtin_amdgcn_sched_barrier(0);
    const int k = r / IT, jt = r % IT;
    ux[jt] = mfma_x6(ga[r & 1], tq[k >> 1][k & 1], ux[jt]);
  }
  if (valid) {
#pragma unroll
    for (int jt = 0; jt < IT; ++jt)
#pragma unroll
      for (int g = 0; g < 4; ++g) {
        f32x4 v;
#pragma unroll
        for (int e = 0; e < 4; ++e) v[e] = acc[jt][4 * g + e] + xx[jt][4 * g + e] * ux[jt][4 * g + e];
        Y.st(vo, (unsigned)(jt * 8 + 2 * g) * plane, v);
      }
  }
}

template <int EPI>
__global__ __launch_bounds__(512, 1) void conv_rgb5_x6_kernel(ConvParams p, long ps, int nblk) {
  extern __shared__ __attribute__((aligned(16))) char rgb5_lds[];
  constexpr bool GDN = EPI == EPI_GDN || EPI == EPI_IGDN;
  rgb5_stage<GDN>(p, ps, rgb5_lds);
  const int tiles_x = (p.Wout + 31) / 32, total = tiles_x * p.Hout * p.N, per = (total + nblk - 1) / nblk;
  int b, cb;
  xcd_block<true>(b, cb);
  const int t_end = min(total, b * per + per), wave = __builtin_amdgcn_readfirstlane(threadIdx.x >> 6);
#pragma unroll 1
  for (int t = b * per + wave; t < t_end; t += 8) {
    const int tx = t % tiles_x, r = t / tiles_x;
    const int oy = r % p.Hout, n = r / p.Hout, ox = tx * 32 + (threadIdx.x & 31);
    const bool valid = ox < p.Wout;
    f32x4 q[RGB5_KY][3];
    rgb5_load(p, n, oy, ox, valid, q);
    f32x16 acc[RGB5_IT];
#pragma unroll
    for (int it = 0; it < RGB5_IT; ++it) acc[it] = f32x16{0};
    rgb5_main(rgb5_lds, q, acc);
    rgb5_epi_fwd<EPI>(p, rgb5_lds, acc, n, oy, ox, valid);
  }
}

constexpr int RGB5B_W_BYTES = RGB5_KY * RGB5_IT * 64 * 16;

template <int EPI>
constexpr int rgb5b_lds_bytes() { return RGB5B_W_BYTES + epi_lds_entries<RGB5_IT, EPI>() * 16; }

template <int EPI>
__global__ __launch_bounds__(512, 1) void conv_rgb5_bf16_kernel(ConvParams p, int nblk) {
  extern __shared__ __attribute__((aligned(16))) char rgb5_lds[];
  constexpr int IT = RGB5_IT;
  {
    const __amdgpu_buffer_rsrc_t wr = uniform_rsrc(p.wp, (unsigned)RGB5B_W_BYTES);
    for (int e = threadIdx.x; e < RGB5B_W_BYTES / 16; e += blockDim.x)
      *reinterpret_cast<f32x4*>(rgb5_lds + (size_t)e * 16) =
          __builtin_bit_cast(f32x4, __builtin_amdgcn_raw_buffer_load_b128(wr, e * 16, 0, 0));
  }
  const f32x4* lp = reinterpret_cast<const f32x4*>(rgb5_lds + RGB5B_W_BYTES);
  if (threadIdx.x < 256) epi_params_to_lds<IT, EPI>(p, reinterpret_cast<f32x4*>(rgb5_lds + RGB5B_W_BYTES), 0);
  __syncthreads();
  const int tiles_x = (p.Wout + 31) / 32, total = tiles_x * p.Hout * p.N, per = (total + nblk - 1) / nblk;
  int b, cb;
  xcd_block<true>(b, cb);
  const int t_end = min(total, b * per + per), wave = __builtin_amdgcn_readfirstlane(threadIdx.x >> 6);
  const int lane = threadIdx.x & 63, h = lane >> 5;
#pragma unroll 1
  for (int t = b * per + wave; t < t_end; t += 8) {
    const int tx = t % tiles_x, r = t / tiles_x;
    const int oy = r % p.Hout, n = r / p.Hout, ox = tx * 32 + (threadIdx.x & 31);
    const bool valid = ox < p.Wout;
    f32x4 q[RGB5_KY][3];
    rgb5_load(p, n, oy, ox, valid, q);
    f32x16 acc[IT];
#pragma unroll
    for (int it = 0; it < IT; ++it) acc[it] = f32x16{0};
    auto ldw = [&](bf16x8 (&a)[IT], int g) {
#pragma unroll
      for (int it = 0; it < IT; ++it) a[it] = lds_frag(rgb5_lds, ((g * IT + it) * 64 + lane) * 16);
    };
    bf16x8 fa[IT], fb[IT];
    ldw(fa, 0);
    auto step = [&](bf16x8 (&cur)[IT], bf16x8 (&nxt)[IT], int ky) __attribute__((always_inline)) {
      if (ky + 1 < RGB5_KY) ldw(nxt, ky + 1);
      __builtin_amdgcn_sched_barrier(0);
      const f32x4 a = q[ky][0], bq = q[ky][1], c = q[ky][2];
      const bf16x8 bs = {(__bf16)a[0], (__bf16)a[1], (__bf16)a[2], (__bf16)bq[0], (__bf16)bq[1], (__bf16)bq[2],
                         (__bf16)(h ? c[2] : c[0]), (__bf16)(h ? 0.f : c[1])};
#pragma unroll
      for (int it = 0; it < IT; ++it) acc[it] = mfma32bf(cur[it], bs, acc[it]);
    };
#pragma unroll
    for (int ky = 0; ky < RGB5_KY; ++ky) {
      if (ky & 1) step(fb, fa, ky);
      else step(fa, fb, ky);
    }
    __builtin_amdgcn_sched_barrier(0);
    conv_epilogue<IT, EPI, 0, true, 0, true, 1>(p, acc, n, oy, ox, valid, 0, lp);
  }
}

template <int EPI>
__global__ __launch_bounds__(256, 1) void conv_rgb5_bwd_x6_kernel(ConvParams p, long ps, int nblk) {
  extern __shared__ __attribute__((aligned(16))) char rgb5_lds[];
  static_assert(EPI == EPI_IGDN_BWD || EPI == EPI_GDN_BWD, "GDN-backward epilogues");
  rgb5_stage<true>(p, ps, rgb5_lds);
  const int tiles_x = (p.Wout + 31) / 32, total = tiles_x * p.Hout * p.N, per = (total + nblk - 1) / nblk;
  int b, cb;
  xcd_block<true>(b, cb);
  const int t_end = min(total, b * per + per), wave = __builtin_amdgcn_readfirstlane(threadIdx.x >> 6);
  auto coords = [&](int t, int& n, int& oy, int& ox) {
    const int tx = t % tiles_x, r = t / tiles_x;
    oy = r % p.Hout;
    n = r / p.Hout;
    ox = tx * 32 + (threadIdx.x & 31);
  };
  int t = b * per + wave;
  if (t >= t_end) return;
  f32x4 q[RGB5_KY][3];
  {
    int n, oy, ox;
    coords(t, n, oy, ox);
    rgb5_load(p, n, oy, ox, ox < p.Wout, q);
  }
#pragma unroll 1
  for (; t < t_end; t += 4) {
    int n, oy, ox;
    coords(t, n, oy, ox);
    const bool valid = ox < p.Wout;
    f32x4 yq[RGB5_IT][4], sq[RGB5_IT][4];
    gdn_bwd_x6_load<RGB5_IT>(p, n, oy, ox, valid, yq, sq);
    f32x16 acc[RGB5_IT];
#pragma unroll
    for (int it = 0; it < RGB5_IT; ++it) acc[it] = f32x16{0};
    rgb5_main(rgb5_lds, q, acc);
    if (t + 4 < t_end) {
      int n1, oy1, ox1;
      coords(t + 4, n1, oy1, ox1);
      rgb5_load(p, n1, oy1, ox1, ox1 < p.Wout, q);
    }
    rgb5_epi_bwd<EPI>(p, rgb5_lds, acc, n, oy, ox, valid, yq, sq);
  }
}

constexpr int XU_TW = 16, XU_PC = XU_TW + 2;
template <int PT>
constexpr int xu_th() { return 4 * PT; }
template <int PT>
constexpr int xu_plane() { return (xu_th<PT>() + 2) * XU_PC; }

template <int CG, int PT>
constexpr int xu_lds_bytes() { return 3 * (CG / 8) * xu_plane<PT>() * 16; }

template <int PY, int PX, int IT, int CG, int PT, int KS = 5>
ICA_DEV void conv_up_x6_class(const ConvParams& p, const f32x4* patch, int jt, int cb, int nch, int grp, long ps,
                              f32x16 (&acc)[PT][IT]) {
  constexpr int PAD = KS / 2, XU_PLANE = xu_plane<PT>();
  constexpr int KY0 = (PY + PAD) & 1, KX0 = (PX + PAD) & 1;
  constexpr int NY = (KS - KY0 + 1) / 2, NX = (KS - KX0 + 1) / 2, NT = NY * NX;
  constexpr int NCG = CG / 16;
  if constexpr (NT == 0) return;
  const int lane = threadIdx.x & 63, h = lane >> 5, j = lane & 31;
  const int a_rel = jt * 2 * PT + (j >> 4), b_rel = j & 15;
  const __amdgpu_buffer_rsrc_t wr = uniform_rsrc(p.wp, (unsigned)(3 * ps * 16));
  const int wbase = cb * KS * KS * nch * IT * 64;
  const int total = NT * NCG;
  auto wofs = [&](int u) -> int {
    const int ti = u / NCG, c = u - ti * NCG;
    const int ky = KY0 + 2 * (ti / NX), kx = KX0 + 2 * (ti % NX);
    return (ky * KS + kx) * nch + grp * NCG + c;
  };
  auto ldw = [&](bf16x8 (&a)[IT][3], int u) {
    const int f = wbase + wofs(min(u, total - 1)) * IT * 64;
#pragma unroll
    for (int it = 0; it < IT; ++it)
#pragma unroll
      for (int q = 0; q < 3; ++q) a[it][q] = ld_bf8(wr, lane * 16, (int)((q * ps + f + it * 64) * 16));
  };
  auto ldb = [&](bf16x8 (&b)[PT][3], int u) {
    u = min(u, total - 1);
    const int ti = u / NCG, c = u - ti * NCG;
    const int ky = KY0 + 2 * (ti / NX), kx = KX0 + 2 * (ti % NX);
    const int pr = a_rel + 1 + (PY + PAD - ky) / 2, pc = b_rel + 1 + (PX + PAD - kx) / 2;
    const int e = (2 * c + h) * XU_PLANE + pr * XU_PC + pc;
#pragma unroll
    for (int t = 0; t < PT; ++t) {
      const int o = e + t * 2 * XU_PC;
      b[t][0] = f4_as_bf8(patch[o]);
      b[t][1] = f4_as_bf8(patch[(CG / 8) * XU_PLANE + o]);
      b[t][2] = f4_as_bf8(patch[2 * (CG / 8) * XU_PLANE + o]);
    }
  };
  auto step = [&](bf16x8 (&cur)[IT][3], bf16x8 (&nxt)[IT][3], bf16x8 (&bc)[PT][3], bf16x8 (&bn)[PT][3], int u) {
    ldw(nxt, u + 1);
    ldb(bn, u + 1);
    __builtin_amdgcn_sched_barrier(0);
#pragma unroll
    for (int t = 0; t < PT; ++t)
#pragma unroll
      for (int it = 0; it < IT; ++it) acc[t][it] = mfma_x6(cur[it], bc[t], acc[t][it]);
  };
  bf16x8 fa[IT][3], fb[IT][3], ba[PT][3], bb[PT][3];
  ldw(fa, 0);
  ldb(ba, 0);
  int u = 0;
#pragma unroll 1
  for (; u + 1 < total; u += 2) {
    step(fa, fb, ba, bb, u);
    step(fb, fa, bb, ba, u + 1);
  }
  if (u < total) step(fa, fb, ba, bb, u);
}

template <int IT, int EPI, int CG, int PT = X6_PT, int KS = 5, int FX = 0>
__global__ __launch_bounds__(256, 1) void conv_up_x6_kernel(ConvParams p, long ps) {
  ICA_STAMP_BEGIN();
  constexpr int NQ = CG / 4, XU_TH = xu_th<PT>(), XU_PLANE = xu_plane<PT>();
  extern __shared__ f32x4 patch[];
  const int tiles_x = (p.Win + XU_TW - 1) / XU_TW, tiles_y = (p.Hin + XU_TH - 1) / XU_TH;
  int bid, cb;
  xcd_block<true>(bid, cb);
  const int tx = bid % tiles_x;
  bid /= tiles_x;
  const int ty = bid % tiles_y;
  const int n = bid / tiles_y;
  const int a0 = ty * XU_TH, b0 = tx * XU_TW;
  const int Cin4 = p.Cin >> 2, nch = p.Cin / 16, ngrp = p.Cin / CG;
  const unsigned xplane = (unsigned)p.Hin * p.Win;
  const __amdgpu_buffer_rsrc_t xr =
      uniform_rsrc(reinterpret_cast<const char*>(p.x) + (size_t)n * Cin4 * xplane * 16, Cin4 * xplane * 16u);
  u32x2* p2 = reinterpret_cast<u32x2*>(patch);
  auto fill = [&](int grp) __attribute__((always_inline)) {
    constexpr int FB = 8, TOT = NQ * XU_PLANE;
    __syncthreads();
    for (int e0 = threadIdx.x; e0 < TOT; e0 += 256 * FB) {
      f32x4 v[FB];
#pragma unroll
      for (int i = 0; i < FB; ++i) {
        const int e = e0 + 256 * i;
        const int q = e / XU_PLANE, rem = e - q * XU_PLANE, pr = rem / XU_PC, pc = rem - pr * XU_PC;
        const int iy = a0 - 1 + pr, ix = b0 - 1 + pc;
        const bool ok = e < TOT && iy >= 0 && iy < p.Hin && ix >= 0 && ix < p.Win;
        const unsigned vo = ((unsigned)(grp * NQ + q) * xplane + pix_at(iy, ix, p.Hin, p.Win, p.pl & PL_IN)) * 16u;
        v[i] = __builtin_bit_cast(f32x4, __builtin_amdgcn_raw_buffer_load_b128(xr, ok ? vo : 0xFFFFFFF0u, 0, 0));
      }
#pragma unroll
      for (int i = 0; i < FB; ++i) {
        const int e = e0 + 256 * i;
        if (e < TOT) {
          const int q = e / XU_PLANE, pix = e - q * XU_PLANE;
          u32x2 a, b, c;
          split3(v[i], a, b, c);
          const int ent = (q >> 1) * XU_PLANE + pix;
          p2[(0 * (CG / 8) * XU_PLANE + ent) * 2 + (q & 1)] = a;
          p2[(1 * (CG / 8) * XU_PLANE + ent) * 2 + (q & 1)] = b;
          p2[(2 * (CG / 8) * XU_PLANE + ent) * 2 + (q & 1)] = c;
        }
      }
    }
    __syncthreads();
  };
  const int wave = __builtin_amdgcn_readfirstlane(threadIdx.x >> 6);
  const int jt = wave & 1;
  const int j = threadIdx.x & 31;
  const int a_rel = jt * 2 * PT + (j >> 4), b_rel = j & 15;
  auto run_class = [&](auto py_c, auto px_c, bool refill, int tk) __attribute__((always_inline)) {
    constexpr int PY = decltype(py_c)::value, PX = decltype(px_c)::value;
    f32x16 acc[PT][IT];
#pragma unroll
    for (int t = 0; t < PT; ++t)
#pragma unroll
      for (int it = 0; it < IT; ++it) acc[t][it] = f32x16{0};
    for (int grp = 0; grp < ngrp; ++grp) {
      if (refill) fill(grp);
      conv_up_x6_class<PY, PX, IT, CG, PT, KS>(p, patch, jt, cb, nch, grp, ps, acc);
    }
    ICA_STAMP_AT(tk - 2);
    if constexpr ((EPI == EPI_GDN || EPI == EPI_IGDN) && PT == 2) {
      const int oy[2] = {2 * (a0 + a_rel) + PY, 2 * (a0 + a_rel + 2) + PY};
      const int ox[2] = {2 * (b0 + b_rel) + PX, 2 * (b0 + b_rel) + PX};
      gdn_fwd_x6_pair<IT, EPI>(p, acc, n, oy, ox);
    } else {
#pragma unroll
      for (int t = 0; t < PT; ++t) {
        const int oy = 2 * (a0 + a_rel + 2 * t) + PY, ox = 2 * (b0 + b_rel) + PX;
        conv_epilogue<IT, EPI, FX, false, 1>(p, acc[t], n, oy, ox, oy < p.Hout && ox < p.Wout, cb * IT * 32);
      }
    }
    ICA_STAMP_AT(tk - 1);
  };
  using I0 = std::integral_constant<int, 0>;
  using I1 = std::integral_constant<int, 1>;
  const bool multi = ngrp > 1;
  if (!multi) fill(0);
  if (wave < 2) {
    run_class(I0{}, I0{}, multi, 2);
    run_class(I1{}, I1{}, multi, 4);
  } else {
    run_class(I0{}, I1{}, multi, 2);
    run_class(I1{}, I0{}, multi, 4);
  }
  ICA_STAMP_END();
}

template <int PY, int PX, int IT, int CG, int PT>
ICA_DEV void conv_up_x6w_class(const ConvParams& p, const f32x4* patch, int jt, int cb, int nch, int grp, long ps,
                               f32x16 (&acc)[PT][IT]) {
  constexpr int KS = 5, PAD = 2, XU_PLANE = xu_plane<PT>();
// ... 89 lines not shown
      a[q] = ld_bf8(grs, lane * 16, (((jt * IT + (k >> 1)) * 2 + (k & 1)) * 1024) + q * IT * IT * 2048);
  };
  f32x16 xx[PT == 1 ? IT : 1];
#pragma unroll
  for (int t = 0; t < PT; ++t) {
    if (t == 1) {
      x6w_ys(p, n, px.vl[1], 0, ry[0], rs[0]);
      x6w_ys(p, n, px.vl[1], 1, ry[1], rs[1]);
    }
#pragma unroll
    for (int it = 0; it < IT; ++it) {
      __builtin_amdgcn_sched_barrier(0);
#pragma unroll
      for (int g = 0; g < 4; ++g) {
        f32x4 tv;
#pragma unroll
        for (int e = 0; e < 4; ++e) {
          const float sg = rs[it & 1][g][e], rc = __builtin_amdgcn_rcpf(sg), xs = ry[it & 1][g][e] * rc;
          const float gx = acc[t][it][4 * g + e] * xs;
          tv[e] = (EPI == EPI_GDN_BWD) ? (-0.5f * gx) * (sg * sg * sg) : (0.5f * gx) * rc;
          float gs = acc[t][it][4 * g + e] * sg;
          float x2 = 2.0f * xs;
          asm volatile("" : "+v"(gs), "+v"(x2));
          acc[t][it][4 * g + e] = gs;
          if constexpr (PT == 1) xx[it][4 * g + e] = x2;
        }
        slab[((2 * it + (g >> 1)) * 2 + (g & 1)) * 64 + lane] = tv;
      }
      if (it + 2 < IT) x6w_ys(p, n, px.vl[t], it + 2, ry[it & 1], rs[it & 1]);
    }
#pragma unroll
    for (int jt = 0; jt < IT; ++jt) {
      __builtin_amdgcn_sched_barrier(0);
      f32x4 yq[4], sq[4];
      if constexpr (PT != 1) x6w_ys(p, n, px.vl[t], jt, yq, sq);
      f32x16 ux = f32x16{0};
      bf16x8 ga[2][3];
      ldg(ga[0], jt, 0);
#pragma unroll
      for (int k = 0; k < 2 * IT; ++k) {
        if (k + 1 < 2 * IT) ldg(ga[(k + 1) & 1], jt, k + 1);
        __builtin_amdgcn_sched_barrier(0);
        const f32x4 a = slab[(2 * k) * 64 + lane], b = slab[(2 * k + 1) * 64 + lane];
        const float v[8] = {a[0], a[1], a[2], a[3], b[0], b[1], b[2], b[3]};
        bf16x8 tq[3];
        split3x8(v, tq);
        ux = mfma_x6(ga[k & 1], tq, ux);
      }
      __builtin_amdgcn_sched_barrier(0);
      if (px.valid[t]) {
#pragma unroll
        for (int g = 0; g < 4; ++g) {
          f32x4 o;
#pragma unroll
          for (int e = 0; e < 4; ++e) {
            float x2;
            if constexpr (PT == 1) {
              x2 = xx[jt][4 * g + e];
            } else {
              x2 = 2.0f * (yq[g][e] * __builtin_amdgcn_rcpf(sq[g][e]));
              asm volatile("" : "+v"(x2));
            }
            o[e] = acc[t][jt][4 * g + e] + x2 * ux[4 * g + e];
          }
          Y.st(px.vo[t], (unsigned)(jt * 8 + 2 * g) * plane, o);
        }
      }
    }
    ICA_STAMP_AT(2 + t);
  }
}

ICA_DEV void barrier_lds_only() {
  asm volatile("s_waitcnt lgkmcnt(0)\n\ts_barrier" ::: "memory");
}

template <int IT, int EPI, int CG, int PT = 2>
__global__ __launch_bounds__(512, 1) void conv_up_x6w_kernel(ConvParams p, long ps) {
  ICA_STAMP_BEGIN();
  constexpr int NQ = CG / 4, XU_TH = xu_th<PT>(), XU_PLANE = xu_plane<PT>();
  extern __shared__ f32x4 patch[];
  const int tiles_x = (p.Win + XU_TW - 1) / XU_TW, tiles_y = (p.Hin + XU_TH - 1) / XU_TH;
  int bid, cb;
  xcd_block<true>(bid, cb);
  const int tx = bid % tiles_x;
  bid /= tiles_x;
  const int ty = bid % tiles_y;
  const int n = bid / tiles_y;
  const int a0 = ty * XU_TH, b0 = tx * XU_TW;
  const int Cin4 = p.Cin >> 2, nch = p.Cin / 16, ngrp = p.Cin / CG;
  const unsigned xplane = (unsigned)p.Hin * p.Win;
  const __amdgpu_buffer_rsrc_t xr =
      uniform_rsrc(reinterpret_cast<const char*>(p.x) + (size_t)n * Cin4 * xplane * 16, Cin4 * xplane * 16u);
  u32x2* p2 = reinterpret_cast<u32x2*>(patch);
  auto fill = [&](int grp) __attribute__((always_inline)) {
    constexpr int FB = 6, TOT = NQ * XU_PLANE;
    __syncthreads();
    for (int e0 = threadIdx.x; e0 < TOT; e0 += 512 * FB) {
      f32x4 v[FB];
#pragma unroll
      for (int i = 0; i < FB; ++i) {
        const int e = e0 + 512 * i;
        const int q = e / XU_PLANE, rem = e - q * XU_PLANE, pr = rem / XU_PC, pc = rem - pr * XU_PC;
        const int iy = a0 - 1 + pr, ix = b0 - 1 + pc;
        const bool ok = e < TOT && iy >= 0 && iy < p.Hin && ix >= 0 && ix < p.Win;
        const unsigned vo = ((unsigned)(grp * NQ + q) * xplane + pix_at(iy, ix, p.Hin, p.Win, p.pl & PL_IN)) * 16u;
        v[i] = __builtin_bit_cast(f32x4, __builtin_amdgcn_raw_buffer_load_b128(xr, ok ? vo : 0xFFFFFFF0u, 0, 0));
      }
#pragma unroll
      for (int i = 0; i < FB; ++i) {
        const int e = e0 + 512 * i;
        if (e < TOT) {
          const int q = e / XU_PLANE, pix = e - q * XU_PLANE;
          u32x2 a, b, c;
          split3(v[i], a, b, c);
          const int ent = (q >> 1) * XU_PLANE + pix;
          p2[(0 * (CG / 8) * XU_PLANE + ent) * 2 + (q & 1)] = a;
          p2[(1 * (CG / 8) * XU_PLANE + ent) * 2 + (q & 1)] = b;
          p2[(2 * (CG / 8) * XU_PLANE + ent) * 2 + (q & 1)] = c;
        }
      }
    }
    __syncthreads();
  };
  const int wave = __builtin_amdgcn_readfirstlane(threadIdx.x >> 6);
  const int jt = wave & 1;
  const int j = threadIdx.x & 31;
  const int a_rel = jt * 2 * PT + (j >> 4), b_rel = j & 15;
  auto run_class = [&](auto py_c, auto px_c, bool refill) __attribute__((always_inline)) {
    constexpr int PY = decltype(py_c)::value, PX = decltype(px_c)::value;
    f32x16 acc[PT][IT];
#pragma unroll
    for (int t = 0; t < PT; ++t)
#pragma unroll
      for (int it = 0; it < IT; ++it) acc[t][it] = f32x16{0};
    for (int grp = 0; grp < ngrp; ++grp) {
      if (refill) fill(grp);
      conv_up_x6w_class<PY, PX, IT, CG, PT>(p, patch, jt, cb, nch, grp, ps, acc);
    }
    int oy[2], ox[2];
#pragma unroll
    for (int t = 0; t < 2; ++t) {
      oy[t] = 2 * (a0 + a_rel + 2 * t) + PY;
      ox[t] = 2 * (b0 + b_rel) + PX;
    }
    static_assert(EPI == EPI_BIAS || EPI == EPI_GDN || EPI == EPI_IGDN || EPI == EPI_GDN_BWD ||
                      EPI == EPI_IGDN_BWD, "conv_up_x6w: bias, GDN / IGDN and their backward epilogues");
    if constexpr (EPI == EPI_GDN_BWD || EPI == EPI_IGDN_BWD) {
      const X6wPix px = x6w_pix<IT>(p, oy, ox);
      f32x4 ry[2][4], rs[2][4];
      x6w_ys(p, n, px.vl[0], 0, ry[0], rs[0]);
      x6w_ys(p, n, px.vl[0], 1, ry[1], rs[1]);
      ICA_STAMP_AT(0);
      ICA_STAMP_WAVE();
      barrier_lds_only();
      ICA_STAMP_AT(1);
      gdn_bwd_x6w_slab<IT, EPI, PT>(p, acc, n, px, ry, rs, patch + wave * (4 * IT * 64));
    } else if constexpr (EPI == EPI_GDN || EPI == EPI_IGDN) {
#pragma unroll
      for (int t = 0; t < PT; ++t) gdn_fwd_x6_tile_narrow<IT, EPI>(p, acc[t], n, oy[t], ox[t]);
    } else {
#pragma unroll
      for (int t = 0; t < PT; ++t)
        conv_epilogue<IT, EPI, 0, false, 2>(p, acc[t], n, oy[t], ox[t], oy[t] < p.Hout && ox[t] < p.Wout,
                                            cb * IT * 32);
    }
  };
  using I0 = std::integral_constant<int, 0>;
  using I1 = std::integral_constant<int, 1>;
  const bool multi = ngrp > 1;
  if (!multi) fill(0);
  switch (wave >> 1) {
    case 0: run_class(I0{}, I0{}, multi); break;
    case 1: run_class(I0{}, I1{}, multi); break;
    case 2: run_class(I1{}, I1{}, multi); break;
    default: run_class(I1{}, I0{}, multi); break;
  }
  ICA_STAMP_END();
}

constexpr int XSD_TW = 8, XSD_TH = 4;
template <int IT>
constexpr int xs_red_entries() { return 3 * IT * 4 * 64; }

template <int IT>
ICA_DEV bool xs_reduce(f32x16 (&acc)[IT], f32x4* red, int wave, int lane) {
  if (wave > 0) {
#pragma unroll
    for (int it = 0; it < IT; ++it)
#pragma unroll
      for (int g = 0; g < 4; ++g)
        red[(((wave - 1) * IT + it) * 4 + g) * 64 + lane] =
            f32x4{acc[it][4 * g], acc[it][4 * g + 1], acc[it][4 * g + 2], acc[it][4 * g + 3]};
  }
  __syncthreads();
  if (wave != 0) return false;
#pragma unroll 1
  for (int w = 0; w < 3; ++w) {
#pragma unroll
    for (int it = 0; it < IT; ++it)
#pragma unroll
      for (int g = 0; g < 4; ++g) {
        const f32x4 r = red[((w * IT + it) * 4 + g) * 64 + lane];
#pragma unroll
        for (int e = 0; e < 4; ++e) acc[it][4 * g + e] += r[e];
      }
  }
  return true;
}

template <int IT, int EPI>
__global__ __launch_bounds__(256, 2) void conv_down_small_x6_kernel(ConvParams p, long ps) {
  constexpr int KS = 5, S = 2, PAD = 2, KK = 25, TW = XSD_TW, TH = XSD_TH;
  constexpr int PR = S * (TH - 1) + KS, PC = S * (TW - 1) + KS, PLANE = PR * PC;
  constexpr int NF = (4 * PLANE + 255) / 256;
  __shared__ f32x4 patch[3 * 2 * PLANE];
  __shared__ f32x4 red[xs_red_entries<IT>()];
  const int tiles_x = (p.Wout + TW - 1) / TW, tiles_y = (p.Hout + TH - 1) / TH;
  int bid, cb;
  xcd_block<true>(bid, cb);
  const int tx = bid % tiles_x;
  bid /= tiles_x;
  const int ty = bid % tiles_y;
  const int n = bid / tiles_y;
  const int lane = threadIdx.x & 63, wave = __builtin_amdgcn_readfirstlane(threadIdx.x >> 6), h = lane >> 5,
            j = lane & 31;
  const int oy0 = ty * TH, ox0 = tx * TW, iy0 = oy0 * S - PAD, ix0 = ox0 * S - PAD;
  const int Cin4 = (p.Cin + 3) >> 2, nch = (Cin4 * 4 + 15) / 16;
  const int oyl = j / TW, oxl = j % TW, lbase = S * oyl * PC + S * oxl;
  const unsigned xplane = (unsigned)p.Hin * p.Win;
  const __amdgpu_buffer_rsrc_t xr =
      uniform_rsrc(reinterpret_cast<const char*>(p.x) + (size_t)n * Cin4 * xplane * 16, Cin4 * xplane * 16u);
  u32x2* p2 = reinterpret_cast<u32x2*>(patch);
  auto fill = [&](int ch) {
    f32x4 v[NF];
#pragma unroll
    for (int i = 0; i < NF; ++i) {
      const int e = threadIdx.x + 256 * i;
      const int q = e / PLANE, rem = e - q * PLANE, pr = rem / PC, pc = rem - pr * PC;
      const int iy = iy0 + pr, ix = ix0 + pc, c4 = ch * 4 + q;
      const bool ok = e < 4 * PLANE && c4 < Cin4 && iy >= 0 && iy < p.Hin && ix >= 0 && ix < p.Win;
      const unsigned vo = ((unsigned)c4 * xplane + pix_at(iy, ix, p.Hin, p.Win, p.pl & PL_IN)) * 16u;
      v[i] = __builtin_bit_cast(f32x4, __builtin_amdgcn_raw_buffer_load_b128(xr, ok ? vo : 0xFFFFFFF0u, 0, 0));
    }
    __syncthreads();
#pragma unroll
    for (int i = 0; i < NF; ++i) {
      const int e = threadIdx.x + 256 * i;
      if (e < 4 * PLANE) {
        const int q = e / PLANE, pix = e - q * PLANE;
        u32x2 a, b, c;
        split3(v[i], a, b, c);
        const int ent = (q >> 1) * PLANE + pix;
        p2[(0 * 2 * PLANE + ent) * 2 + (q & 1)] = a;
        p2[(1 * 2 * PLANE + ent) * 2 + (q & 1)] = b;
        p2[(2 * 2 * PLANE + ent) * 2 + (q & 1)] = c;
      }
    }
    __syncthreads();
  };
  const int t0 = wave * KK / 4, nt = (wave + 1) * KK / 4 - t0, total = nch * nt;
  const __amdgpu_buffer_rsrc_t wr = uniform_rsrc(p.wp, (unsigned)(3 * ps * 16));
  const int wbase = cb * nch * KK * IT * 64;
  auto ldw = [&](bf16x8 (&a)[IT][3], int u) {
    u = min(u, total - 1);
    const int ch = u / nt, tap = t0 + (u - ch * nt);
    const int f = wbase + (ch * KK + tap) * IT * 64;
#pragma unroll
    for (int it = 0; it < IT; ++it)
#pragma unroll
      for (int q = 0; q < 3; ++q) a[it][q] = ld_bf8(wr, lane * 16, (int)((q * ps + f + it * 64) * 16));
  };
  f32x16 acc[IT];
#pragma unroll
  for (int it = 0; it < IT; ++it) acc[it] = f32x16{0};
  auto step = [&](bf16x8 (&cur)[IT][3], bf16x8 (&nxt)[IT][3], int u) __attribute__((always_inline)) {
    ldw(nxt, u + 1);
    __builtin_amdgcn_sched_barrier(0);
    const int ch = u / nt, tap = t0 + (u - ch * nt);
    const int ky = tap / KS, kx = tap - ky * KS;
    const int o = h * PLANE + lbase + ky * PC + kx;
    const bf16x8 b[3] = {f4_as_bf8(patch[o]), f4_as_bf8(patch[2 * PLANE + o]), f4_as_bf8(patch[4 * PLANE + o])};
#pragma unroll
    for (int it = 0; it < IT; ++it) acc[it] = mfma_x6(cur[it], b, acc[it]);
  };
  bf16x8 fa[IT][3], fb[IT][3];
  ldw(fa, 0);
  int u = 0;
#pragma unroll 1
  for (int ch = 0; ch < nch; ++ch) {
    fill(ch);
    const int ue = u + nt;
#pragma unroll 1
    for (; u + 1 < ue; u += 2) {
      step(fa, fb, u);
      step(fb, fa, u + 1);
    }
    if (u < ue) {
      step(fa, fb, u);
      ++u;
#pragma unroll
      for (int it = 0; it < IT; ++it)
#pragma unroll
        for (int q = 0; q < 3; ++q) fa[it][q] = fb[it][q];
    }
  }
  if (!xs_reduce<IT>(acc, red, wave, lane)) return;
  const int oy = oy0 + oyl, ox = ox0 + oxl;
  conv_epilogue<IT, EPI, 0, false, 2>(p, acc, n, oy, ox, oy < p.Hout && ox < p.Wout, cb * IT * 32);
}

constexpr int XSU_TH = 2, XSU_PC = 18, XSU_PLANE = (XSU_TH + 2) * XSU_PC;
template <int IT, int EPI>
__global__ __launch_bounds__(256, 2) void conv_up_small_x6_kernel(ConvParams p, long ps) {
  constexpr int KS = 5, PAD = 2, TW = 16;
  extern __shared__ f32x4 patch[];
  const int tiles_x = (p.Win + TW - 1) / TW, tiles_y = (p.Hin + XSU_TH - 1) / XSU_TH;
  int bid, cb;
  xcd_block<true>(bid, cb);
  const int cls = bid & 3;
  bid >>= 2;
  const int tx = bid % tiles_x;
  bid /= tiles_x;
  const int ty = bid % tiles_y;
  const int n = bid / tiles_y;
  const int a0 = ty * XSU_TH, b0 = tx * TW;
  const int Cin4 = p.Cin >> 2, nch = p.Cin / 16, NQ8 = p.Cin / 8;
  const unsigned xplane = (unsigned)p.Hin * p.Win;
  const __amdgpu_buffer_rsrc_t xr =
      uniform_rsrc(reinterpret_cast<const char*>(p.x) + (size_t)n * Cin4 * xplane * 16, Cin4 * xplane * 16u);
  u32x2* p2 = reinterpret_cast<u32x2*>(patch);
  {
    constexpr int FB = 8;
    const int TOT = Cin4 * XSU_PLANE;
    for (int e0 = threadIdx.x; e0 < TOT; e0 += 256 * FB) {
      f32x4 v[FB];
#pragma unroll
      for (int i = 0; i < FB; ++i) {
        const int e = e0 + 256 * i;
        const int q = e / XSU_PLANE, rem = e - q * XSU_PLANE, pr = rem / XSU_PC, pc = rem - pr * XSU_PC;
        const int iy = a0 - 1 + pr, ix = b0 - 1 + pc;
        const bool ok = e < TOT && iy >= 0 && iy < p.Hin && ix >= 0 && ix < p.Win;
        const unsigned vo = ((unsigned)q * xplane + pix_at(iy, ix, p.Hin, p.Win, p.pl & PL_IN)) * 16u;
        v[i] = __builtin_bit_cast(f32x4, __builtin_amdgcn_raw_buffer_load_b128(xr, ok ? vo : 0xFFFFFFF0u, 0, 0));
      }
#pragma unroll
      for (int i = 0; i < FB; ++i) {
        const int e = e0 + 256 * i;
        if (e < TOT) {
          const int q = e / XSU_PLANE, pix = e - q * XSU_PLANE;
          u32x2 a, b, c;
          split3(v[i], a, b, c);
          const int ent = (q >> 1) * XSU_PLANE + pix;
          p2[(0 * NQ8 * XSU_PLANE + ent) * 2 + (q & 1)] = a;
          p2[(1 * NQ8 * XSU_PLANE + ent) * 2 + (q & 1)] = b;
          p2[(2 * NQ8 * XSU_PLANE + ent) * 2 + (q & 1)] = c;
        }
      }
    }
  }
  __syncthreads();
  const int lane = threadIdx.x & 63, wave = __builtin_amdgcn_readfirstlane(threadIdx.x >> 6), h = lane >> 5,
            j = lane & 31;
  const int c0 = wave * nch / 4, cn = (wave + 1) * nch / 4 - c0;
  const int a_rel = j >> 4, b_rel = j & 15;
  const __amdgpu_buffer_rsrc_t wr = uniform_rsrc(p.wp, (unsigned)(3 * ps * 16));
  const int wbase = cb * KS * KS * nch * IT * 64;
  auto run = [&](auto py_c, auto px_c) __attribute__((always_inline)) {
    constexpr int PY = decltype(py_c)::value, PX = decltype(px_c)::value;
    constexpr int KY0 = (PY + PAD) & 1, KX0 = (PX + PAD) & 1;
    constexpr int NY = (KS - KY0 + 1) / 2, NX = (KS - KX0 + 1) / 2, NT = NY * NX;
    const int total = NT * cn;
    auto ldw = [&](bf16x8 (&a)[IT][3], int u) {
      u = min(u, total - 1);
      const int ti = u / cn, c = c0 + (u - ti * cn);
      const int ky = KY0 + 2 * (ti / NX), kx = KX0 + 2 * (ti % NX);
      const int f = wbase + ((ky * KS + kx) * nch + c) * IT * 64;
#pragma unroll
      for (int it = 0; it < IT; ++it)
#pragma unroll
        for (int q = 0; q < 3; ++q) a[it][q] = ld_bf8(wr, lane * 16, (int)((q * ps + f + it * 64) * 16));
    };
    f32x16 acc[IT];
#pragma unroll
    for (int it = 0; it < IT; ++it) acc[it] = f32x16{0};
    auto step = [&](bf16x8 (&cur)[IT][3], bf16x8 (&nxt)[IT][3], int u) __attribute__((always_inline)) {
      ldw(nxt, u + 1);
      __builtin_amdgcn_sched_barrier(0);
      const int ti = u / cn, c = c0 + (u - ti * cn);
      const int ky = KY0 + 2 * (ti / NX), kx = KX0 + 2 * (ti % NX);
      const int pr = a_rel + 1 + (PY + PAD - ky) / 2, pc = b_rel + 1 + (PX + PAD - kx) / 2;
      const int o = (2 * c + h) * XSU_PLANE + pr * XSU_PC + pc;
      const bf16x8 b[3] = {f4_as_bf8(patch[o]), f4_as_bf8(patch[NQ8 * XSU_PLANE + o]),
                           f4_as_bf8(patch[2 * NQ8 * XSU_PLANE + o])};
#pragma unroll
      for (int it = 0; it < IT; ++it) acc[it] = mfma_x6(cur[it], b, acc[it]);
    };
    bf16x8 fa[IT][3], fb[IT][3];
    ldw(fa, 0);
    int u = 0;
#pragma unroll 1
    for (; u + 1 < total; u += 2) {
      step(fa, fb, u);
      step(fb, fa, u + 1);
    }
    if (u < total) step(fa, fb, u);
    __syncthreads();
    if (!xs_reduce<IT>(acc, patch, wave, lane)) return;
// ... 628 lines not shown
```

imagecompression_adversarial_amd/csrc/ica_elem.hip:

```cpp
#include "ica_reduce.h"

__global__ void nchw_to_nc4_kernel(const float* __restrict__ src, float* __restrict__ dst, int N, int C, int H,
                                   int W) {
  const int C4 = (C + 3) >> 2;
  const long HW = (long)H * W;
  const long total = (long)N * C4 * HW;
  for (long i = (long)blockIdx.x * blockDim.x + threadIdx.x; i < total; i += (long)gridDim.x * blockDim.x) {
    const long pix = i % HW;
    const long t = i / HW;
    const int c4 = t % C4, n = t / C4;
    f32x4 v;
#pragma unroll
    for (int e = 0; e < 4; ++e) {
      const int c = c4 * 4 + e;
      v[e] = c < C ? src[((long)n * C + c) * HW + pix] : 0.f;
    }
    st4(dst + i * 4, v);
  }
}

__global__ void nc4_to_nchw_kernel(const float* __restrict__ src, float* __restrict__ dst, int N, int C, int H,
                                   int W) {
  const int C4 = (C + 3) >> 2;
  const long HW = (long)H * W;
  const long total = (long)N * C4 * HW;
  for (long i = (long)blockIdx.x * blockDim.x + threadIdx.x; i < total; i += (long)gridDim.x * blockDim.x) {
    const long pix = i % HW;
    const long t = i / HW;
    const int c4 = t % C4, n = t / C4;
    const f32x4 v = ld4(src + i * 4);
#pragma unroll
    for (int e = 0; e < 4; ++e) {
      const int c = c4 * 4 + e;
      if (c < C) dst[((long)n * C + c) * HW + pix] = v[e];
    }
  }
}

__global__ void reduce_rows_kernel(const float* __restrict__ part, float* __restrict__ out, int nblk, float scale) {
  __shared__ float sh[4];
  const int b = blockIdx.x;
  float v = 0.f;
  for (int k = threadIdx.x; k < nblk; k += 256) v += part[(long)b * nblk + k];
  const float r = block_sum_paired(v, sh);
  if (threadIdx.x == 0) out[b] = r * scale;
}

constexpr int ELEM_BLOCKS_PER_IMAGE = 256;

__global__ void attack_prologue_kernel(const float* __restrict__ noise, const float* __restrict__ im_s,
                                       float* __restrict__ im_in4, float* __restrict__ part, long HW, float eps,
                                       int clamp_in, long nstride) {
  __shared__ float sh[4];
  const int b = blockIdx.y;
  const float* nz = noise + (long)b * nstride;
  const float* is = im_s + (long)b * 3 * HW;
  float* o4 = im_in4 + (long)b * 4 * HW;
  float acc = 0.f;
  for (long pix = (long)blockIdx.x * 256 + threadIdx.x; pix < HW; pix += (long)gridDim.x * 256) {
    f32x4 v = {0.f, 0.f, 0.f, 0.f};
#pragma unroll
    for (int c = 0; c < 3; ++c) {
      const float nc = fminf(fmaxf(nz[c * HW + pix], -eps), eps);
      const float s = is[c * HW + pix];
      const float u = fadd_rn(s, nc);
      const float ii = clamp_in ? fminf(fmaxf(u, 0.f), 1.f) : u;
      v[c] = ii;
      const float d = fsub_rn(s, ii);
      acc = fadd_rn(acc, fmul_rn(d, d));
    }
    st4(o4 + pix * 4, v);
  }
  const float r = block_sum_paired(acc, sh);
  if (threadIdx.x == 0) part[(long)b * gridDim.x + blockIdx.x] = r;
}

__global__ void attack_loss_kernel(const float* __restrict__ xhat4, const float* __restrict__ out_s,
                                   float* __restrict__ grad4, float* __restrict__ part, long HW, float invN,
                                   int clamp, int mode) {
  __shared__ float sh[4];
  const int b = blockIdx.y;
  const float* x4 = xhat4 + (long)b * 4 * HW;
  const float* os = out_s + (long)b * 3 * HW;
  float* g4 = grad4 + (long)b * 4 * HW;
  float acc = 0.f;
  for (long pix = (long)blockIdx.x * 256 + threadIdx.x; pix < HW; pix += (long)gridDim.x * 256) {
    const f32x4 xv = ld4(x4 + pix * 4);
    f32x4 gv = {0.f, 0.f, 0.f, 0.f};
#pragma unroll
    for (int c = 0; c < 3; ++c) {
      const float xh = xv[c];
      const float lo = fmaxf(xh, 0.f);
      const float o = (clamp && mode == 0) ? fminf(lo, 1.f) : xh;
      const float d = fsub_rn(os[c * HW + pix], o);
      acc = fadd_rn(acc, fmul_rn(d, d));
      const float t = fmul_rn(invN, d);
      float g = mode == 0 ? fadd_rn(t, t) : -fadd_rn(t, t);
      if (clamp && mode == 0) {
        g = (lo <= 1.f || g > 0.f) ? g : g * 0.f;
        g = (xh >= 0.f || g < 0.f) ? g : g * 0.f;
      }
      gv[c] = g;
    }
    st4(g4 + pix * 4, gv);
  }
  const float r = block_sum_paired(acc, sh);
  if (threadIdx.x == 0) part[(long)b * gridDim.x + blockIdx.x] = r;
}

__global__ void roi_prologue_kernel(const float* __restrict__ noise, const float* __restrict__ im_s,
                                    float* __restrict__ im_in4, float* __restrict__ part, long HW, long W, float eps,
                                    RoiBox roi) {
  __shared__ float sh[4];
  const int b = blockIdx.y;
  const float* nz = noise + (long)b * 3 * HW;
  const float* is = im_s + (long)b * 3 * HW;
  float* o4 = im_in4 + (long)b * 4 * HW;
  float acc = 0.f;
  for (long pix = (long)blockIdx.x * 256 + threadIdx.x; pix < HW; pix += (long)gridDim.x * 256) {
    const float w = roi_inside(roi, pix, W) ? roi.w_in_tar : roi.w_in_bkg;
    f32x4 v = {0.f, 0.f, 0.f, 0.f};
#pragma unroll
    for (int c = 0; c < 3; ++c) {
      const float nc = fminf(fmaxf(nz[c * HW + pix], -eps), eps);
      const float s = is[c * HW + pix];
      const float u = fadd_rn(s, nc);
      const float ii = fminf(fmaxf(u, 0.f), 1.f);
      v[c] = ii;
      const float d = fsub_rn(s, ii);
      acc = fadd_rn(acc, fmul_rn(w, fmul_rn(d, d)));
    }
    st4(o4 + pix * 4, v);
  }
  const float r = block_sum_paired(acc, sh);
  if (threadIdx.x == 0) part[(long)b * gridDim.x + blockIdx.x] = r;
}

__global__ void roi_loss_kernel(const float* __restrict__ xhat4, const float* __restrict__ out_s,
                                const float* __restrict__ out_t, float* __restrict__ grad4, float* __restrict__ part,
                                long HW, long W, RoiBox roi, int clamp) {
  __shared__ float sh[4];
  const int b = blockIdx.y;
  const float* x4 = xhat4 + (long)b * 4 * HW;
  const float* os = out_s + (long)b * 3 * HW;
  const float* ot = out_t + (long)b * 3 * HW;
  float* g4 = grad4 + (long)b * 4 * HW;
  float acc = 0.f;
  for (long pix = (long)blockIdx.x * 256 + threadIdx.x; pix < HW; pix += (long)gridDim.x * 256) {
    const bool tar = roi_inside(roi, pix, W);
    const float w = tar ? roi.w_out_tar : roi.w_out_bkg;
    const float* ref = tar ? ot : os;
    const f32x4 xv = ld4(x4 + pix * 4);
    f32x4 gv = {0.f, 0.f, 0.f, 0.f};
#pragma unroll
    for (int c = 0; c < 3; ++c) {
      const float xh = xv[c];
      const float lo = fmaxf(xh, 0.f);
      const float o = clamp ? fminf(lo, 1.f) : xh;
      const float d = fsub_rn(ref[c * HW + pix], o);
      acc = fadd_rn(acc, fmul_rn(w, fmul_rn(d, d)));
      const float t = fmul_rn(w, d);
      float g = -fadd_rn(t, t);
      if (clamp) {
        g = (lo <= 1.f || g > 0.f) ? g : g * 0.f;
        g = (xh >= 0.f || g < 0.f) ? g : g * 0.f;
      }
      gv[c] = g;
    }
    st4(g4 + pix * 4, gv);
  }
  const float r = block_sum_paired(acc, sh);
  if (threadIdx.x == 0) part[(long)b * gridDim.x + blockIdx.x] = r;
}

template <bool ROI>
__global__ void attack_adam_kernel(float* __restrict__ noise, const float* __restrict__ im_s,
                                   const float* __restrict__ gnet4, const float* __restrict__ loss_i,
                                   const float* __restrict__ cheap_grad, float* __restrict__ m,
                                   float* __restrict__ v, float* __restrict__ im_in_out, long HW, float eps,
                                   float thr, float invN, float bc2s, float neg_step, int* __restrict__ branch,
                                   RoiBox roi, long W, const int* __restrict__ gpos, int* __restrict__ census,
                                   int clamp_in) {
  const int b = blockIdx.y;
  const bool cheap = loss_i[b] > thr;
  if (blockIdx.x == 0 && threadIdx.x == 0) {
    if (branch) branch[b] = cheap ? 1 : 0;
    if (census) census[b] += cheap ? 1 : 0;
  }
  const long off = (long)b * 3 * HW;
  const long grow = cheap ? 0 : (gpos ? gpos[b] : b);
  auto update = [&](long pix, float nz, float s, float g_in, float cg, float mo, float vo, float& nz_out,
                    float& m_out, float& v_out, float& ii_out) {
    const float lowN = fmaxf(nz, -eps);
    const float nc = fminf(lowN, eps);
    const float u = fadd_rn(s, nc);
    const float lowU = clamp_in ? fmaxf(u, 0.f) : u;
    const float ii = clamp_in ? fminf(lowU, 1.f) : u;
    ii_out = ii;
    float g;
    if (cheap) {
      if (cheap_grad) {
        g = cg;
      } else {
        float w = invN;
        if constexpr (ROI) w = roi_inside(roi, pix, W) ? roi.w_in_tar : roi.w_in_bkg;
        const float t = fmul_rn(w, fsub_rn(s, ii));
        g = -fadd_rn(t, t);
      }
    } else {
      g = g_in;
    }
    if (clamp_in) {
      g = (lowU <= 1.f || g > 0.f) ? g : g * 0.f;
      g = (u >= 0.f || g < 0.f) ? g : g * 0.f;
    }
    g = (lowN <= eps || g > 0.f) ? g : g * 0.f;
    g = (nz >= -eps || g < 0.f) ? g : g * 0.f;
    const float mn = __fmaf_rn(0.1f, fsub_rn(g, mo), mo);
    const float vn = fadd_rn(fmul_rn(vo, 0.999f), fmul_rn(fmul_rn(0.001f, g), g));
    const float denom = fadd_rn(fdiv_rn(sqrtf(vn), bc2s), 1e-8f);
    m_out = mn;
    v_out = vn;
    nz_out = fadd_rn(nz, fmul_rn(neg_step, fdiv_rn(mn, denom)));
  };
  if ((HW & 3) == 0) {
// ... 271 lines not shown
  for (long pix = (long)blockIdx.x * 256 + threadIdx.x; pix < HW; pix += (long)gridDim.x * 256) {
    const f32x4 v = ld4(x4 + ((long)b * HW + pix) * 4);
#pragma unroll
    for (int c = 0; c < 3; ++c) out[((long)b * 3 + c) * HW + pix] = clamp ? fminf(fmaxf(v[c], 0.f), 1.f) : v[c];
  }
}

__global__ void bound_bwd_nc4_kernel(const float* __restrict__ x4, const float* __restrict__ g,
                                     float* __restrict__ g4, long HW, int clamp) {
  const int b = blockIdx.y;
  for (long pix = (long)blockIdx.x * 256 + threadIdx.x; pix < HW; pix += (long)gridDim.x * 256) {
    const f32x4 v = ld4(x4 + ((long)b * HW + pix) * 4);
    f32x4 o = {0.f, 0.f, 0.f, 0.f};
#pragma unroll
    for (int c = 0; c < 3; ++c) {
      float gg = g[((long)b * 3 + c) * HW + pix];
      if (clamp) {
        const float xh = v[c], lo = fmaxf(xh, 0.f);
        gg = (lo <= 1.f || gg > 0.f) ? gg : gg * 0.f;
        gg = (xh >= 0.f || gg < 0.f) ? gg : gg * 0.f;
      }
      o[c] = gg;
    }
    st4(g4 + ((long)b * HW + pix) * 4, o);
  }
}

__global__ void clamp01_kernel(const float* __restrict__ x, float* __restrict__ y, long n) {
  for (long i = (long)blockIdx.x * blockDim.x + threadIdx.x; i < n; i += (long)gridDim.x * blockDim.x)
    y[i] = fminf(fmaxf(x[i], 0.f), 1.f);
}

static inline int grid_1d(long n) {
  long g = (n + 255) / 256;
  return (int)(g > 8192 ? 8192 : (g < 1 ? 1 : g));
}

extern "C" {

int ica_elem_blocks_per_image() { return ELEM_BLOCKS_PER_IMAGE; }

int ica_nchw_to_nc4(const float* src, float* dst, int N, int C, int H, int W, hipStream_t st) {
  const long total = (long)N * ((C + 3) / 4) * H * W;
  ICA_LAUNCH(nchw_to_nc4_kernel, dim3(grid_1d(total)), dim3(256), 0, st, src, dst, N, C, H, W);
  ICA_CHECK_LAUNCH();
  return 0;
}

int ica_nc4_to_nchw(const float* src, float* dst, int N, int C, int H, int W, hipStream_t st) {
  const long total = (long)N * ((C + 3) / 4) * H * W;
  ICA_LAUNCH(nc4_to_nchw_kernel, dim3(grid_1d(total)), dim3(256), 0, st, src, dst, N, C, H, W);
  ICA_CHECK_LAUNCH();
  return 0;
}

int ica_reduce_rows(const float* part, float* out, int B, int nblk, float scale, hipStream_t st) {
  ICA_LAUNCH(reduce_rows_kernel, dim3(B), dim3(256), 0, st, part, out, nblk, scale);
  ICA_CHECK_LAUNCH();
  return 0;
}

int ica_attack_prologue_ex(const float* noise, const float* im_s, float* im_in4, float* part, int B, int H, int W,
                           float eps, int clamp_in, hipStream_t st) {
  ICA_LAUNCH(attack_prologue_kernel, dim3(ELEM_BLOCKS_PER_IMAGE, B), dim3(256), 0, st, noise, im_s, im_in4,
                     part, (long)H * W, eps, clamp_in, 3L * H * W);
  ICA_CHECK_LAUNCH();
  return 0;
}

int ica_universal_prologue(const float* noise, const float* im_s, float* im_in4, float* part, int B, int H, int W,
                           float eps, hipStream_t st) {
  if (B < 1 || H < 1 || W < 1) return (int)hipErrorInvalidValue;
  ICA_LAUNCH(attack_prologue_kernel, dim3(ELEM_BLOCKS_PER_IMAGE, B), dim3(256), 0, st, noise, im_s, im_in4,
                     part, (long)H * W, eps, 1, 0L);
  ICA_CHECK_LAUNCH();
  return 0;
}

int ica_attack_prologue(const float* noise, const float* im_s, float* im_in4, float* part, int B, int H, int W,
                        float eps, hipStream_t st) {
  return ica_attack_prologue_ex(noise, im_s, im_in4, part, B, H, W, eps, 1, st);
}

int ica_attack_loss(const float* xhat4, const float* out_s, float* grad4, float* part, int B, int H, int W,
                    float invN, int clamp, int mode, hipStream_t st) {
  ICA_LAUNCH(attack_loss_kernel, dim3(ELEM_BLOCKS_PER_IMAGE, B), dim3(256), 0, st, xhat4, out_s, grad4, part,
                     (long)H * W, invN, clamp, mode);
  ICA_CHECK_LAUNCH();
  return 0;
}

int ica_attack_adam_ex(float* noise, const float* im_s, const float* gnet4, const float* loss_i,
                       const float* cheap_grad, float* m, float* v, float* im_in_out, int B, int H, int W, float eps,
                       float thr, float invN, float bc2s, float neg_step, int* branch, const int* gpos, int* census,
                       int clamp_in, hipStream_t st) {
  ICA_LAUNCH(attack_adam_kernel<false>, dim3(ELEM_BLOCKS_PER_IMAGE, B), dim3(256), 0, st, noise, im_s, gnet4,
                     loss_i, cheap_grad, m, v, im_in_out, (long)H * W, eps, thr, invN, bc2s, neg_step, branch,
                     RoiBox{}, (long)W, gpos, census, clamp_in);
  ICA_CHECK_LAUNCH();
  return 0;
}

int ica_attack_adam(float* noise, const float* im_s, const float* gnet4, const float* loss_i, const float* cheap_grad,
                    float* m, float* v, float* im_in_out, int B, int H, int W, float eps, float thr, float invN,
                    float bc2s, float neg_step, int* branch, const int* gpos, int* census, hipStream_t st) {
  return ica_attack_adam_ex(noise, im_s, gnet4, loss_i, cheap_grad, m, v, im_in_out, B, H, W, eps, thr, invN, bc2s,
                            neg_step, branch, gpos, census, 1, st);
}

int ica_roi_prologue(const float* noise, const float* im_s, float* im_in4, float* part, int B, int H, int W, float eps,
                     int x0, int x1, int y0, int y1, float w_in_tar, float w_in_bkg, hipStream_t st) {
  const RoiBox roi{x0, x1, y0, y1, w_in_tar, w_in_bkg, 0.f, 0.f};
  ICA_LAUNCH(roi_prologue_kernel, dim3(ELEM_BLOCKS_PER_IMAGE, B), dim3(256), 0, st, noise, im_s, im_in4, part,
                     (long)H * W, (long)W, eps, roi);
  ICA_CHECK_LAUNCH();
  return 0;
}

int ica_roi_loss(const float* xhat4, const float* out_s, const float* out_t, float* grad4, float* part, int B, int H,
                 int W, int x0, int x1, int y0, int y1, float w_out_tar, float w_out_bkg, int clamp, hipStream_t st) {
  const RoiBox roi{x0, x1, y0, y1, 0.f, 0.f, w_out_tar, w_out_bkg};
  ICA_LAUNCH(roi_loss_kernel, dim3(ELEM_BLOCKS_PER_IMAGE, B), dim3(256), 0, st, xhat4, out_s, out_t, grad4,
                     part, (long)H * W, (long)W, roi, clamp);
  ICA_CHECK_LAUNCH();
  return 0;
}

int ica_roi_adam(float* noise, const float* im_s, const float* gnet4, const float* loss_i, float* m, float* v,
                 float* im_in_out, int B, int H, int W, float eps, float thr, float bc2s, float neg_step, int* branch,
                 int x0, int x1, int y0, int y1, float w_in_tar, float w_in_bkg, const int* gpos, int* census,
                 hipStream_t st) {
  const RoiBox roi{x0, x1, y0, y1, w_in_tar, w_in_bkg, 0.f, 0.f};
  ICA_LAUNCH(attack_adam_kernel<true>, dim3(ELEM_BLOCKS_PER_IMAGE, B), dim3(256), 0, st, noise, im_s, gnet4,
                     loss_i, nullptr, m, v, im_in_out, (long)H * W, eps, thr, 0.f, bc2s, neg_step, branch, roi,
                     (long)W, gpos, census, 1);
  ICA_CHECK_LAUNCH();
  return 0;
}

int ica_branch_select(const float* loss_i, float thr, int B, int* sel, int* gpos, hipStream_t st) {
  ICA_LAUNCH(branch_select_kernel, dim3(1), dim3(64), 0, st, loss_i, thr, B, sel, gpos);
  ICA_CHECK_LAUNCH();
  return 0;
}

int ica_gather_images(const float* src, float* dst, const int* idx, int E, long floats_per_image, hipStream_t st) {
  if (E <= 0) return 0;
  if (floats_per_image % 4) return (int)hipErrorInvalidValue;
  const long quads = floats_per_image / 4;
  const int gx = (int)((quads + 255) / 256 < 1024 ? (quads + 255) / 256 : 1024);
  ICA_LAUNCH(gather_images_kernel, dim3(gx, E), dim3(256), 0, st, reinterpret_cast<const f32x4*>(src),
                     reinterpret_cast<f32x4*>(dst), idx, quads);
  ICA_CHECK_LAUNCH();
  return 0;
}

int ica_ifgsm_step(float* x, const float* im_s, const float* grad4, float* gacc, const float* l1, int B, int H,
                   int W, float alpha, float eps, int momentum, hipStream_t st) {
  ICA_LAUNCH(ifgsm_kernel, dim3(ELEM_BLOCKS_PER_IMAGE, B), dim3(256), 0, st, x, im_s, grad4, gacc, l1,
                     (long)H * W, alpha, eps, momentum);
  ICA_CHECK_LAUNCH();
  return 0;
}

int ica_l1_partial(const float* g4, float* part, int B, int H, int W, hipStream_t st) {
  ICA_LAUNCH(l1_partial_kernel, dim3(ELEM_BLOCKS_PER_IMAGE, B), dim3(256), 0, st, g4, part, (long)H * W);
  ICA_CHECK_LAUNCH();
  return 0;
}

int ica_gc_likelihood(const float* y, const float* scales, const float* means, const float* qnoise, float* y_hat,
                      float* lik, float* part, int B, int C, int H, int W, int training, hipStream_t st) {
  const long per_image = 4L * ((C + 3) / 4) * H * W;
  ICA_LAUNCH(gc_kernel, dim3(ELEM_BLOCKS_PER_IMAGE, B), dim3(256), 0, st, y, scales, means, qnoise, y_hat,
                     lik, part, C, per_image, training);
  ICA_CHECK_LAUNCH();
  return 0;
}

int ica_eb_likelihood(const float* z, const float* prm, const float* med, const float* qnoise, float* z_hat,
                      float* lik, float* part, int B, int C, int H, int W, int training, hipStream_t st) {
  const long per_image = 4L * ((C + 3) / 4) * H * W;
  ICA_LAUNCH(eb_kernel, dim3(ELEM_BLOCKS_PER_IMAGE, B), dim3(256), 0, st, z, prm, med, qnoise, z_hat, lik,
                     part, C, per_image, training);
  ICA_CHECK_LAUNCH();
  return 0;
}

int ica_pack_eb(const float* const* params, float* prm, float* med, int C, hipStream_t st) {
  const float* const* p = params;
  ICA_LAUNCH(pack_eb_kernel, dim3((C + 63) / 64), dim3(64), 0, st, p[0], p[1], p[2], p[3], p[4], p[5], p[6],
                     p[7], p[8], p[9], p[10], p[11], p[12], p[13], p[14], prm, med, C);
  ICA_CHECK_LAUNCH();
  return 0;
}

int ica_round(const float* x, float* y, long n, hipStream_t st) {
  ICA_LAUNCH(round_kernel, dim3(grid_1d(n)), dim3(256), 0, st, x, y, n);
  ICA_CHECK_LAUNCH();
  return 0;
}

int ica_cast_f32_bf16(const float* x, void* y, long n, hipStream_t st) {
  if (n % 4) return -2;
  ICA_LAUNCH(cast_f32_bf16_kernel, dim3(grid_1d(n / 4)), dim3(256), 0, st, reinterpret_cast<const f32x4*>(x),
                     reinterpret_cast<u32x2*>(y), n / 4);
  ICA_CHECK_LAUNCH();
  return 0;
// ... 45 lines not shown
```

imagecompression_adversarial_amd/hip_ops.py:

```python
from __future__ import annotations

import math

import torch

from ._lib import ConvArgs, LayerDesc, call, lib, ptr, stream

EPI_BIAS, EPI_RELU, EPI_GDN, EPI_IGDN, EPI_GDN_BWD, EPI_IGDN_BWD, EPI_LRELU, EPI_LRELU_BWD = range(8)
FILL_PLAIN, FILL_LRELU_MASK, FILL_UNSHUFFLE = range(3)
ORDER_DOWN, ORDER_UP = 0, 1
ORDER_RGB5 = 2
ORDER_TG = 3
ORDER_UP3 = 4
_ORDER_NAME = ("DOWN", "UP", "RGB5", "TG", "UP3")
LAYOUT_IN, LAYOUT_OUT = 1, 2
GDN_BETA_BOUND = float((1e-6 + 2.0 ** -36) ** 0.5)


EVENT_HOOK = None


def _ev_begin(tag, n):
    if EVENT_HOOK is None or tag is None:
        return None
    if LAUNCH_HOOK is not None:
        last_launch()
    e0 = torch.cuda.Event(enable_timing=True)
    e0.record()
    return (tag, e0, n)


def _ev_end(h, flops=None):
    if h is not None:
        e1 = torch.cuda.Event(enable_timing=True)
        e1.record()
        EVENT_HOOK.setdefault(h[0], []).append((h[1], e1, h[2]))
        if flops is not None:
            FLOPS_HOOK[h[0]] = flops / max(h[2], 1)
        if LAUNCH_HOOK is not None:
            LAUNCH_HOOK.setdefault(h[0], set()).add(last_launch())


LAUNCH_HOOK = None


def source_hash() -> str:
    import glob
    import hashlib
    import os
    h = hashlib.sha256()
    d = os.path.join(os.path.dirname(os.path.abspath(__file__)), "csrc")
    for f in sorted(glob.glob(os.path.join(d, "*.hip")) + glob.glob(os.path.join(d, "*.h"))):
        h.update(os.path.basename(f).encode())
        with open(f, "rb") as fh:
            h.update(fh.read())
    return h.hexdigest()[:16]


def last_launch():
    import ctypes as C
    buf = C.create_string_buffer(512)
    thr = C.c_ulonglong(0)
    n = lib().ica_last_launch(buf, 512, C.byref(thr))
    if n <= 0:
        return None
    if n > 1:
        return f"<{n} launches>", 0
    return buf.value.decode(errors="replace"), int(thr.value)


X6_TILING_AUTO, X6_TILING_PREVIOUS, X6_TILING_BALANCED = 0, 1, 2


def x6_tiling(mode: int = X6_TILING_AUTO) -> None:
    call("ica_x6_tiling", int(mode))


PREC_HOOK = {}


_PREC_SUFFIX = {0: "fp32", 1: "bf16", 2: "x6", 3: "b1"}


def _prec_note(tag, prec):
    if EVENT_HOOK is None or tag is None:
        return tag
    first = PREC_HOOK.setdefault(tag, prec)
    if first != prec:
        tag = f"{tag}[{_PREC_SUFFIX.get(prec, prec)}]"
        PREC_HOOK.setdefault(tag, prec)
    return tag


FLOPS_HOOK = {}


def _dev_check(t: torch.Tensor, name="tensor"):
    if not t.is_cuda:
        raise RuntimeError(f"{name} must be a HIP device tensor (no CPU fallback on the hot path)")
    if t.dtype != torch.float32:
        raise RuntimeError(f"{name} must be float32")
    if not t.is_contiguous():
        raise RuntimeError(f"{name} must be contiguous")


def check_image(x, name, dev=True):
    if not isinstance(x, torch.Tensor) or x.dim() != 4 or x.shape[1] != 3 or x.shape[0] < 1:
        shape = tuple(x.shape) if isinstance(x, torch.Tensor) else type(x).__name__
        raise ValueError(f"{name} {shape} is not a [B, 3, H, W] batch")
    if dev:
        _dev_check(x, name)
    return x.shape[0], x.shape[2], x.shape[3]


def check_nc4(x, name):
    if x.dim() != 5 or x.shape[1] != 1 or x.shape[4] != 4 or x.shape[0] < 1:
        raise ValueError(f"{name} {tuple(x.shape)} is not a 3-channel nChw4c batch [B, 1, H, W, 4]")
    _dev_check(x, name)
    return x.shape[0], x.shape[2], x.shape[3]


def positive_int(name, v):
    if not isinstance(v, int) or isinstance(v, bool) or v < 1:
        raise ValueError(f"{name} must be a positive int, got {v!r}")


def c4(C: int) -> int:
    return (C + 3) // 4


def empty_nc4(N, C, H, W, device, dtype=torch.float32):
    return torch.empty((N, c4(C), H, W, 4), dtype=dtype, device=device)


def cast_nc4(x4: torch.Tensor, dtype) -> torch.Tensor:
    if x4.dtype == dtype:
        return x4
    if not x4.is_cuda or not x4.is_contiguous():
        raise RuntimeError("cast_nc4 needs a contiguous HIP tensor")
    y = torch.empty(x4.shape, dtype=dtype, device=x4.device)
    if dtype == torch.bfloat16 and x4.dtype == torch.float32:
        call("ica_cast_f32_bf16", ptr(x4), ptr(y), x4.numel(), stream())
    elif dtype == torch.float32 and x4.dtype == torch.bfloat16:
        call("ica_cast_bf16_f32", ptr(x4), ptr(y), x4.numel(), stream())
    else:
        raise RuntimeError(f"cast_nc4 {x4.dtype} -> {dtype}")
    return y


def to_nc4(x: torch.Tensor) -> torch.Tensor:
    x = x.contiguous()
    _dev_check(x, "x")
    N, C, H, W = x.shape
    y = empty_nc4(N, C, H, W, x.device)
    call("ica_nchw_to_nc4", ptr(x), ptr(y), N, C, H, W, stream())
    return y


def from_nc4(x4: torch.Tensor, C: int) -> torch.Tensor:
    _dev_check(x4, "x4")
    N, _, H, W, _ = x4.shape
    y = torch.empty((N, C, H, W), dtype=torch.float32, device=x4.device)
    call("ica_nc4_to_nchw", ptr(x4), ptr(y), N, C, H, W, stream())
    return y


PREC_FP32, PREC_BF16, PREC_X6 = 0, 1, 2
PREC_B1 = 3


def x6_it(O: int) -> int:
    return int(lib().ica_conv_it(O))


class Pack:
    __slots__ = ("data", "O", "C", "KS", "kind", "order", "prec", "it", "flip")

# ... 122 lines not shown
        self.C = C
        T = C // 32
        dev = beta.device
        beta = beta.detach().contiguous()
        gamma = gamma.detach().reshape(C, C).contiguous()
        self.gp = torch.empty(T * T * 64 * 16, device=dev)
        self.gpT = torch.empty(T * T * 64 * 16, device=dev)
        self.beta = torch.empty(C, device=dev)
        call("ica_pack_gdn", ptr(gamma), ptr(beta), ptr(self.gp), ptr(self.beta), C, 0, GDN_BETA_BOUND, stream())
        call("ica_pack_gdn", ptr(gamma), ptr(beta), ptr(self.gpT), ptr(self.beta), C, 1, GDN_BETA_BOUND, stream())
        self._src = (gamma, beta)
        self.gpb = self.gpbT = None
        self.gpx = self.gpxT = None

    def x6(self):
        if self.gpx is None:
            n = int(lib().ica_pack_gdn_x6_size(self.C))
            self.gpx = torch.empty(n // 2, dtype=torch.bfloat16, device=self.gp.device)
            self.gpxT = torch.empty_like(self.gpx)
            call("ica_pack_gdn_x6", ptr(self.gp), ptr(self.gpx), self.C, stream())
            call("ica_pack_gdn_x6", ptr(self.gpT), ptr(self.gpxT), self.C, stream())
        return self

    def bf16(self):
        if self.gpb is None:
            gamma, beta = self._src
            T = self.C // 32
            self.gpb = torch.empty(T * T * 2048, dtype=torch.bfloat16, device=gamma.device)
            self.gpbT = torch.empty_like(self.gpb)
            call("ica_pack_gdn_bf16", ptr(gamma), ptr(beta), ptr(self.gpb), ptr(self.beta), self.C, 0,
                 GDN_BETA_BOUND, stream())
            call("ica_pack_gdn_bf16", ptr(gamma), ptr(beta), ptr(self.gpbT), ptr(self.beta), self.C, 1,
                 GDN_BETA_BOUND, stream())
        return self


def _out_hw(H, W, KS, S, kind):
    if kind == 0:
        return (H + 2 * (KS // 2) - KS) // S + 1, (W + 2 * (KS // 2) - KS) // S + 1
    return 2 * H, 2 * W


def _check_pack(wp, Cin, Cout, KS, kind, prec=None, it=0):
    if not isinstance(wp, Pack):
        raise TypeError(f"conv launch: wp must be a hip_ops.Pack (from a packer or a PackedConv), not "
                        f"{type(wp).__name__}")
    if (wp.O, wp.C, wp.KS, wp.kind) != (Cout, Cin, KS, kind):
        raise ValueError(f"conv launch (O={Cout}, C={Cin}, KS={KS}, kind={kind}) on {wp!r}")
    if (wp.data.dtype == torch.float32) != (wp.prec == PREC_FP32):
        raise ValueError(f"{wp!r} holds {wp.data.dtype} fragments")
    if (prec is not None and prec != wp.prec) or (it and it != wp.it):
        raise ValueError(f"conv launch stated prec={prec}, it={it} for {wp!r}")


def _conv3(x4, Cin, wp, bias, Cout, KS, S, kind, epi, gdn, save, saved, out, tag, save_t, layout, prec, it):
    _check_pack(wp, Cin, Cout, KS, kind, prec, it)
    ss = None
    if save and epi in (EPI_GDN, EPI_IGDN):
        N, _, H, W, _ = x4.shape
        ss = empty_nc4(N, Cout, *_out_hw(H, W, KS, S, kind), x4.device,
                       torch.bfloat16 if wp.prec == PREC_BF16 else torch.float32)
    y = conv_ex(x4, Cin, wp, bias, Cout, KS, S, kind, epi, gdn, save_s=ss, saved=saved, save_t=save_t, out=out,
                tag=tag, layout=layout, _flops=False)
    return y, (y if ss is not None else None), ss


def conv_down(x4, Cin, wp: Pack, bias, Cout, KS, S, epi=EPI_BIAS, gdn: PackedGDN | None = None, save=False,
              saved=None, out=None, tag=None, save_t=None, layout=0, prec=None, it=0):
    return _conv3(x4, Cin, wp, bias, Cout, KS, S, 0, epi, gdn, save, saved, out, tag, save_t, layout, prec, it)


def conv_up(x4, Cin, wp: Pack, bias, Cout, epi=EPI_BIAS, gdn: PackedGDN | None = None, save=False, saved=None,
            out=None, tag=None, save_t=None, layout=0, prec=None, it=0):
    if Cout != 3:
        return _conv3(x4, Cin, wp, bias, Cout, 5, 2, 1, epi, gdn, save, saved, out, tag, save_t, layout, prec, it)
    _check_pack(wp, Cin, 3, 5, 1, prec, it)
    if wp.order != ORDER_UP3:
        raise ValueError(f"conv_up to 3 channels reads the Z-gather pack (ORDER_UP3), not {wp!r}")
    if epi != EPI_BIAS:
        raise RuntimeError("conv_up to 3 channels supports the bias epilogue only")
    N, _, H, W, _ = x4.shape
    y = out if out is not None else empty_nc4(N, 3, 2 * H, 2 * W, x4.device)
    ev = _ev_begin(_prec_note(tag, wp.prec), N)
    call("ica_conv_up3", ptr(x4), ptr(y), ptr(wp.data), ptr(bias), N, Cin, H, W, int(layout), int(wp.prec), stream())
    _ev_end(ev)
    return y, None, None


def conv_ex(x4, Cin, wp: Pack, bias, Cout, KS, S, kind=0, epi=EPI_BIAS, gdn: PackedGDN | None = None, res=None,
            save_x=None, save_s=None, saved=None, save_t=None, mask=None, fill_mode=FILL_PLAIN, ps=False,
            out=None, tag=None, alg_rows=None, layout=0, prec=None, it=0, _flops=True):
    _check_pack(wp, Cin, Cout, KS, kind, prec, it)
    if wp.order == ORDER_UP3:
        raise ValueError(f"{wp!r} is launched by conv_up to 3 channels only")
    if wp.order == ORDER_RGB5 and (epi not in (EPI_BIAS, EPI_GDN, EPI_IGDN_BWD) or fill_mode != FILL_PLAIN or ps
                                   or any(t is not None for t in (res, save_x, save_t, mask))):
        raise ValueError(f"{wp!r}: the dense tap-row pack is read by conv_rgb5 only (bias / GDN / IGDN_BWD epilogue, "
                         f"plain fill, no extra tensors)")
    prec = wp.prec
    N, C4x, H, W, _ = x4.shape
    if fill_mode == FILL_UNSHUFFLE:
        if Cin != 16 * C4x:
            raise RuntimeError("unshuffled conv input: Cin must be 16 * input channel groups")
        H, W = H // 2, W // 2
    Ho, Wo = _out_hw(H, W, KS, S, kind)
    dt = torch.bfloat16 if prec == PREC_BF16 else torch.float32
    if out is not None:
        y = out
    elif ps:
        y = torch.empty((N, Cout // 16, 2 * Ho, 2 * Wo, 4), dtype=dt, device=x4.device)
    else:
        y = empty_nc4(N, Cout, Ho, Wo, x4.device, dt)
    in_x = in_s = None
    if saved is not None:
        in_x, in_s = saved
    gp = None
    if gdn is not None:
        if prec == PREC_BF16:
            gdn.bf16()
            gp = gdn.gpbT if epi in (EPI_GDN_BWD, EPI_IGDN_BWD) else gdn.gpb
        elif prec in (PREC_X6, PREC_B1):
            gdn.x6()
            gp = gdn.gpxT if epi in (EPI_GDN_BWD, EPI_IGDN_BWD) else gdn.gpx
        else:
            gp = gdn.gpT if epi in (EPI_GDN_BWD, EPI_IGDN_BWD) else gdn.gp
    a = ConvArgs(ptr(x4), ptr(y), ptr(wp.data), ptr(bias), ptr(gp), ptr(None if gdn is None else gdn.beta),
                 ptr(save_x), ptr(save_s), ptr(in_x), ptr(in_s), ptr(save_t), ptr(res), ptr(mask), N, Cin, H, W, Cout,
                 Ho, Wo, kind, KS, S, epi, wp.it, fill_mode, int(bool(ps)), prec, int(layout), wp.order)
    import ctypes
    tag = _prec_note(tag, prec)
    ev = _ev_begin(tag, N)
    call("ica_conv_ex", ctypes.c_void_p(ctypes.addressof(a)), stream())
    if ev is not None:
        fl = None
        if _flops:
            px = N * (H * W if kind == 1 else Ho * Wo)
            cin_alg = alg_rows if (fill_mode == FILL_UNSHUFFLE and alg_rows) else Cin
            cout_alg = alg_rows if (ps and alg_rows) else Cout
            fl = 2.0 * cin_alg * cout_alg * KS * KS * px
            if epi in (EPI_GDN, EPI_IGDN, EPI_GDN_BWD, EPI_IGDN_BWD):
                fl += 2.0 * Cout * Cout * N * Ho * Wo
        _ev_end(ev, fl)
    return y


def pack_up3k3_x6(w1: torch.Tensor, ws: torch.Tensor) -> torch.Tensor:
    w1, ws = w1.detach().contiguous(), ws.detach().contiguous()
    _dev_check(w1, "weight")
    _dev_check(ws, "weight")
    Cg = w1.shape[0]
    if tuple(w1.shape) != (Cg, 3, 3, 3) or tuple(ws.shape) != (Cg, 3, 1, 1):
        raise RuntimeError("pack_up3k3_x6: conv1 [Cg][3][3][3] and skip [Cg][3][1][1] weights")
    dst = torch.empty(int(lib().ica_pack_up3k3_x6_size(Cg)) // 2, dtype=torch.bfloat16, device=w1.device)
    call("ica_pack_up3k3_x6", ptr(w1), ptr(ws), ptr(dst), Cg, stream())
    return dst


def conv_up3k3_x6(g1: torch.Tensor, gs: torch.Tensor, wp: torch.Tensor, Hout: int, Wout: int, tag=None):
    for t, nm in ((g1, "g1"), (gs, "gs")):
        _dev_check(t, nm)
        if not t.is_contiguous() or t.dtype != torch.float32:
            raise RuntimeError(f"conv_up3k3_x6: {nm} must be contiguous fp32 nChw4c")
    if g1.shape != gs.shape:
        raise RuntimeError("conv_up3k3_x6: g1 and gs shapes differ")
    N, C4, H, W, _ = g1.shape
    dx = empty_nc4(N, 3, Hout, Wout, g1.device)
    ev = _ev_begin(tag, N)
    call("ica_conv_up3k3_x6", ptr(g1), ptr(gs), ptr(wp), ptr(dx), N, 4 * C4, H, W, Hout, Wout, stream())
    _ev_end(ev, 2.0 * 4 * C4 * 3 * (9 + 1) * N * H * W)
    return dx


def blocks_per_image() -> int:
    return int(lib().ica_elem_blocks_per_image())


def reduce_rows(part: torch.Tensor, B: int, scale: float = 1.0, out=None):
    nblk = part.numel() // B
    o = out if out is not None else torch.empty(B, device=part.device)
    call("ica_reduce_rows", ptr(part), ptr(o), B, nblk, float(scale), stream())
    return o


def abs_(x: torch.Tensor) -> torch.Tensor:
    y = torch.empty_like(x)
    call("ica_abs", ptr(x), ptr(y), x.numel(), stream())
    return y


def round_(x: torch.Tensor) -> torch.Tensor:
    y = torch.empty_like(x)
    call("ica_round", ptr(x), ptr(y), x.numel(), stream())
    return y


def clamp01(x: torch.Tensor) -> torch.Tensor:
    y = torch.empty_like(x)
    call("ica_clamp01", ptr(x), ptr(y), x.numel(), stream())
    return y


def sqdiff_mean(a: torch.Tensor, b: torch.Tensor, clamp_a=False) -> torch.Tensor:
    B = a.shape[0]
    length = a[0].numel()
    part = torch.empty(B * blocks_per_image(), device=a.device)
    call("ica_sqdiff_partial", ptr(a.contiguous()), ptr(b.contiguous()), ptr(part), B, length, int(clamp_a), stream())
    return reduce_rows(part, B, 1.0 / length)


class PackedEB:
    NAMES = ([f"_matrix{i}" for i in range(5)] + [f"_bias{i}" for i in range(5)]
# ... 259 lines not shown
```

include/ica_hip.h:

```cpp
#ifndef ICA_HIP_H
#define ICA_HIP_H

#include <stddef.h>
#include <stdint.h>

#ifdef __cplusplus
extern "C" {
#endif

typedef struct ihipStream_t* hipStream_t;

enum { ICA_EPI_BIAS = 0, ICA_EPI_RELU = 1, ICA_EPI_GDN = 2, ICA_EPI_IGDN = 3, ICA_EPI_GDN_BWD = 4, ICA_EPI_IGDN_BWD = 5 };

int ica_conv_it(int cout);
size_t ica_pack_conv_weight_size(int O, int C, int KS, int CC, int it);
int ica_pack_conv_weight(const float* w, float* dst, int O, int C, int KS, long so, long sc, int CC, int order,
                         int flip, int it, hipStream_t stream);
int ica_pack_gdn(const float* gamma, const float* beta, float* gp, float* beta_eff, int C, int transpose,
                 float beta_bound, hipStream_t stream);
int ica_pack_conv_weight_bf16(const float* w, void* dst, int O, int C, int KS, long so, long sc, int order,
                              int flip, int it, hipStream_t stream);
int ica_pack_gdn_bf16(const float* gamma, const float* beta, void* gpb, float* beta_eff, int C, int transpose,
                      float beta_bound, hipStream_t stream);
int ica_pack_conv_weight_x6(const float* w, void* dst, int O, int C, int KS, long so, long sc, int order, int it,
                            hipStream_t stream);
size_t ica_pack_conv_weight_x6_size(int O, int C, int KS, int it);
int ica_pack_gdn_x6(const float* gp, void* dst, int C, hipStream_t stream);
size_t ica_pack_gdn_x6_size(int C);
size_t ica_pack_conv_weight_bf16_size(int O, int C, int KS, int it);
int ica_pack_up3k3_x6(const float* w1, const float* ws, void* dst, int Cg, hipStream_t stream);
size_t ica_pack_up3k3_x6_size(int Cg);
int ica_conv_up3k3_x6(const float* g1, const float* gs, const void* wp, float* dx, int N, int Cg, int Hin, int Win,
                      int Hout, int Wout, hipStream_t stream);
int ica_cast_f32_bf16(const float* x, void* y, long n, hipStream_t stream);
int ica_cast_bf16_f32(const void* x, float* y, long n, hipStream_t stream);

int ica_flip_rot(const float* x, float* y, long planes, int H, int W, int op, hipStream_t stream);
int ica_bitdepth(const float* x, float* y, long n, float scale, hipStream_t stream);
int ica_resample_axis(const float* x, float* y, long planes, int H, int W, int axis, int out_len, const int* xmin,
                      const int* xsize, const float* w, int K, hipStream_t stream);
int ica_bitdepth_noise(const float* x, const float* u, float* y, long n, float scale, hipStream_t stream);
int ica_bitdepth_noise_bwd(const float* g, float* gx, long n, float scale, hipStream_t stream);
int ica_add(const float* a, const float* b, float* y, long n, hipStream_t stream);
int ica_ensemble_grad(const float* o, const float* out_s, float* g, long n, float invN, hipStream_t stream);
int ica_gc_symbols(const float* y4, const float* scales4, const float* means4, const float* table, int T, float bound,
                   int32_t* symbols, int32_t* indexes, int B, int C, int H, int W, hipStream_t stream);
int ica_eb_symbols(const float* z4, const float* medians, int32_t* symbols, int32_t* indexes, int B, int C, int H,
                   int W, hipStream_t stream);
int ica_dequantize(const int32_t* symbols, const float* means4, const float* medians, float* out4, int B, int C, int H,
                   int W, hipStream_t stream);
int ica_pmf_to_quantized_cdf(const float* pmf, int n, int precision, int32_t* cdf_out);
long ica_rans_encode(const int32_t* symbols, const int32_t* indexes, long n, const int32_t* cdfs, int stride,
                     const int32_t* cdf_sizes, const int32_t* offsets, int n_cdfs, uint8_t* out, long cap,
                     long* needed);
int ica_rans_decode(const uint8_t* data, long nbytes, const int32_t* indexes, long n, const int32_t* cdfs, int stride,
                    const int32_t* cdf_sizes, const int32_t* offsets, int n_cdfs, int32_t* symbols);
int ica_rans_dec_open(const uint8_t* data, long nbytes, void** decoder);
int ica_rans_dec_step(void* const* decoders, int B, const int32_t* indexes, long n, const int32_t* cdfs, int stride,
                      const int32_t* cdf_sizes, const int32_t* offsets, int n_cdfs, int32_t* symbols, int* bad);
int ica_rans_dec_close(void* decoder);

typedef struct ica_ar_args {
  const float* y;
  const float* params;
  float* yhat;
  int32_t* sym;
  int32_t* idx;
  const int32_t* sym_in;
  float* means;
  const float* wc;
  const float* bc;
  const float* w1;
  const float* b1;
  const float* w2;
  const float* b2;
  const float* w3;
  const float* b3;
  const float* table;
  int T;
  float bound;
  int B, M, H, W, E1, E2;
} ica_ar_args;
size_t ica_ar_lds_bytes(int M, int E1, int E2);
int ica_ar_step(const ica_ar_args* args, int p0, int p1, int mode, hipStream_t stream);
enum { ICA_EPI_LRELU = 6, ICA_EPI_LRELU_BWD = 7 };
enum { ICA_ORDER_DOWN = 0, ICA_ORDER_UP = 1, ICA_ORDER_RGB5 = 2, ICA_ORDER_TG = 3, ICA_ORDER_UP3 = 4 };
typedef struct ica_conv_args {
  const float* x;
  float* y;
  const float* wp;
  const float* bias;
  const float* gp;
  const float* beta;
  float* save_x;
  float* save_s;
  const float* in_x;
  const float* in_s;
  float* save_t;
  const float* res;
  const float* mask;
  int N, Cin, Hin, Win, Cout, Hout, Wout;
  int kind, KS, S, epi, it, fill_mode, ps;
  int prec;
  int layout;
  int order;
} ica_conv_args;
int ica_conv_ex(const ica_conv_args* args, hipStream_t stream);
int ica_last_launch(char* name, int cap, unsigned long long* threads);
int ica_x6_tiling(int mode);
size_t ica_pack_up3_size(int Cin);
int ica_pack_up3(const float* w, void* dst, int Cin, int prec, hipStream_t stream);
int ica_conv_up3(const float* x, float* y, const void* wp, const float* bias, int N, int Cin, int Hin, int Win,
                 int layout, int prec, hipStream_t stream);

int ica_elem_blocks_per_image(void);
int ica_nchw_to_nc4(const float* src, float* dst, int N, int C, int H, int W, hipStream_t stream);
int ica_nc4_to_nchw(const float* src, float* dst, int N, int C, int H, int W, hipStream_t stream);
int ica_reduce_rows(const float* part, float* out, int B, int nblk, float scale, hipStream_t stream);
int ica_attack_prologue(const float* noise, const float* im_s, float* im_in4, float* part, int B, int H, int W,
                        float eps, hipStream_t stream);
int ica_attack_prologue_ex(const float* noise, const float* im_s, float* im_in4, float* part, int B, int H, int W,
                           float eps, int clamp_in, hipStream_t stream);
int ica_attack_loss(const float* xhat4, const float* out_s, float* grad4, float* part, int B, int H, int W,
                    float invN, int clamp, int mode, hipStream_t stream);
int ica_attack_adam(float* noise, const float* im_s, const float* gnet4, const float* loss_i, const float* cheap_grad,
                    float* m, float* v, float* im_in_out, int B, int H, int W, float eps, float thr, float invN,
                    float bc2s, float neg_step, int* branch, const int* gpos, int* census, hipStream_t stream);
int ica_attack_adam_ex(float* noise, const float* im_s, const float* gnet4, const float* loss_i,
                       const float* cheap_grad, float* m, float* v, float* im_in_out, int B, int H, int W, float eps,
                       float thr, float invN, float bc2s, float neg_step, int* branch, const int* gpos, int* census,
                       int clamp_in, hipStream_t stream);
int ica_universal_prologue(const float* noise, const float* im_s, float* im_in4, float* part, int B, int H, int W,
                           float eps, hipStream_t stream);
int ica_universal_adam(float* noise, const float* im_s, const float* gnet4, const float* loss_i, float* m, float* v,
                       float* im_in_out, int B, int H, int W, float eps, float thr, float gscale, float bc2s,
                       float neg_step, int* branch, int* census, hipStream_t stream);
int ica_branch_select(const float* loss_i, float thr, int B, int* sel, int* gpos, hipStream_t stream);
int ica_gather_images(const float* src, float* dst, const int* idx, int E, long floats_per_image, hipStream_t stream);
int ica_roi_prologue(const float* noise, const float* im_s, float* im_in4, float* part, int B, int H, int W, float eps,
                     int x0, int x1, int y0, int y1, float w_in_tar, float w_in_bkg, hipStream_t stream);
int ica_roi_loss(const float* xhat4, const float* out_s, const float* out_t, float* grad4, float* part, int B, int H,
                 int W, int x0, int x1, int y0, int y1, float w_out_tar, float w_out_bkg, int clamp, hipStream_t stream);
int ica_roi_adam(float* noise, const float* im_s, const float* gnet4, const float* loss_i, float* m, float* v,
                 float* im_in_out, int B, int H, int W, float eps, float thr, float bc2s, float neg_step, int* branch,
                 int x0, int x1, int y0, int y1, float w_in_tar, float w_in_bkg, const int* gpos, int* census,
                 hipStream_t stream);
int ica_ifgsm_step(float* x, const float* im_s, const float* grad4, float* gacc, const float* l1, int B, int H, int W,
                   float alpha, float eps, int momentum, hipStream_t stream);
int ica_l1_partial(const float* g4, float* part, int B, int H, int W, hipStream_t stream);
int ica_gc_likelihood(const float* y, const float* scales, const float* means, const float* qnoise, float* y_hat,
                      float* lik, float* part, int B, int C, int H, int W, int training, hipStream_t stream);
int ica_eb_likelihood(const float* z, const float* prm, const float* med, const float* qnoise, float* z_hat,
                      float* lik, float* part, int B, int C, int H, int W, int training, hipStream_t stream);
int ica_pack_eb(const float* const* params, float* prm, float* med, int C, hipStream_t stream);
int ica_abs(const float* x, float* y, long n, hipStream_t stream);
int ica_round(const float* x, float* y, long n, hipStream_t stream);
int ica_clamp01(const float* x, float* y, long n, hipStream_t stream);
int ica_sqdiff_partial(const float* a, const float* b, float* part, int B, long len, int clamp_a, hipStream_t stream);
int ica_nc4_bound_to_nchw(const float* x4, float* out, int B, int H, int W, int clamp, hipStream_t stream);
int ica_bound_bwd_nc4(const float* x4, const float* g, float* g4, int B, int H, int W, int clamp, hipStream_t stream);

int ica_cw_gate(const float* part, int nblk, float invN, const double* sd, int* si, float* mse_o, float* c_eff, int B,
                hipStream_t stream);
int ica_cw_adam(float* noise, const float* im_s, const float* gnet4, const float* c_eff, float* m, float* v,
                float* im_in_out, int B, int H, int W, float eps, float invN, const float* tab, int ntab, const int* si,
                int clamp_in, hipStream_t stream);
int ica_cw_round(const float* loss_i, const float* mse_o, double* sd, float* lold, int* si, int* n_active, int B,
                 int fast, int ssteps, int max_rounds, const double* cfg, hipStream_t stream);
int ica_cw_reset(float* noise, float* m, float* v, const int* si, int B, long floats_per_image, hipStream_t stream);

int ica_latent_range(const float* y4, int B, int C, int H, int W, float* out_max, float* out_min, float* out_absmax,
                     hipStream_t stream);
int ica_latent_clamp(const float* y4, const float* cmax, const float* cmin, float* out4, int B, int C, int H, int W,
                     int* nclamped, hipStream_t stream);
int ica_latent_clamp_bwd(float* g4, const float* y4, const float* cmax, const float* cmin, int B, int C, int H, int W,
                         hipStream_t stream);
int ica_latent_detect(const float* imax, const float* imin, const float* cmax, const float* cmin, float* score, int B,
                      int C, hipStream_t stream);

size_t ica_latent_distrib_ws_size(int B, int C, int H, int W, int nbins);
int ica_latent_distrib(const float* y4, const float* scales4, const float* means4, const float* lik4, int B, int C,
                       int H, int W, float vmin, int nbins, float scale_floor, float pred_floor, int* hist,
                       float* pred, float* bits, float* work, hipStream_t stream);

enum { ICA_LAYER_PAIR = 0, ICA_LAYER_QUANT = 1, ICA_LAYER_TRIPLE = 2 };
enum { ICA_LAYERS_MAX = 16 };
typedef struct ica_layer_desc {
  const float* a;
  const float* b;
  const float* c;
  int C, H, W, mode;
} ica_layer_desc;
int ica_layer_sums_blocks(int C, int H, int W);
size_t ica_layer_sums_ws_size(int n, int B);
int ica_layer_sums(const ica_layer_desc* layers, int n, int B, float* sums, float* work, hipStream_t stream);

int ica_rate_gc_blocks(void);
int ica_rate_eb_blocks(int C, int H, int W);
int ica_rate_gc(const float* y4, const float* sigma4, float* gy4, float* gsig4, float* part, int B, int C, int H,
                int W, float scale, hipStream_t stream);
int ica_rate_eb(const float* v4, const float* prm, float* gv4, float* part, int B, int C, int H, int W, float scale,
                hipStream_t stream);

int ica_rd_metrics_blocks(void);
int ica_rd_metrics(const float* xhat4, const float* target, const float* liky4, const float* likz4, float* out,
                   float* part, int* nclamp, int B, int H, int W, int Cy, int Hy, int Wy, int Cz, int Hz, int Wz,
                   hipStream_t stream);
int ica_val_metrics(const float* xhat4, const float* target, const float* liky4, const float* likz4, float* out,
                    float* part, int B, int H, int W, int Cy, int Hy, int Wy, int Cz, int Hz, int Wz,
                    hipStream_t stream);

size_t ica_patch_vi_ws_size(int B, int H, int W, int win, int stride);
int ica_patch_vi(const float* im_adv, const float* out_adv, const float* im_s, const float* out_s, int B, int H, int W,
                 int win, int stride, int border, float* ws, void* key_ws, float* mse_in, float* mse_out, float* vi,
                 float* val, int* pos, hipStream_t stream);
int ica_patch_gather(const float* im_adv, const float* out_adv, const float* im_s, const float* out_s, const int* pos,
                     float* patches, int B, int H, int W, int win, int stride, hipStream_t stream);

size_t ica_gauss_blur_ws_size(int B, int H, int W);
int ica_gauss_blur(const float* x, const float* wx, const float* wy, int B, int H, int W, int kx, int ky, int clamp,
                   const float* ref, float* out, float* mse, float* ws, hipStream_t stream);
int ica_blur_sweep_chunk(void);
size_t ica_blur_sweep_ws_size(int B, int H, int W);
int ica_blur_sweep(const float* x, const float* wx, const float* wy, int S, int B, int H, int W, int kx, int ky,
                   float budget, int s0, float* mse, long ld, int* idx, int* done, int* remaining, float* ws,
// ... 67 lines not shown
```

Baseline: 1570 attack-step·images/s.

## Skip converged images inside captured graph via device-side live-image list

Adds a device-resident live-image list (count plus indices from ica_branch_select) that conv, up-conv and loss kernels read to restrict their tile walks to images still needing network gradients. A second graph is captured with this list, so the compacted batch can be replayed without a host sync or gather. Before, a full-batch graph ran only when no image had converged; otherwise the code synced to the host and fell back to eager gathered execution. This adds per-kernel indirection and early-exit blocks, and falls back when a layer's precision or shape doesn't support the live path.

```diff
diff --git a/imagecompression_adversarial_amd/_lib.py b/imagecompression_adversarial_amd/_lib.py
--- a/imagecompression_adversarial_amd/_lib.py
+++ b/imagecompression_adversarial_amd/_lib.py
@@ -35,6 +35,7 @@
     "ica_pack_up3_size": [_i],
     "ica_pack_up3": [_p, _p, _i, _i, _p],
     "ica_conv_up3": [_p, _p, _p, _p, _i, _i, _i, _i, _i, _i, _p],
+    "ica_conv_up3_live": [_p, _p, _p, _p, _i, _i, _i, _i, _i, _i, _p, _p],
     "ica_elem_blocks_per_image": [],
     "ica_nchw_to_nc4": [_p, _p, _i, _i, _i, _i, _p],
     "ica_nc4_to_nchw": [_p, _p, _i, _i, _i, _i, _p],
@@ -42,6 +43,7 @@
     "ica_attack_prologue": [_p, _p, _p, _p, _i, _i, _i, _f, _p],
     "ica_attack_prologue_ex": [_p, _p, _p, _p, _i, _i, _i, _f, _i, _p],
     "ica_attack_loss": [_p, _p, _p, _p, _i, _i, _i, _f, _i, _i, _p],
+    "ica_attack_loss_live": [_p, _p, _p, _p, _i, _i, _i, _f, _i, _i, _p, _p],
     "ica_attack_adam": [_p, _p, _p, _p, _p, _p, _p, _p, _i, _i, _i, _f, _f, _f, _f, _f, _p, _p, _p, _p],
     "ica_attack_adam_ex": [_p, _p, _p, _p, _p, _p, _p, _p, _i, _i, _i, _f, _f, _f, _f, _f, _p, _p, _p, _i, _p],
     "ica_universal_prologue": [_p, _p, _p, _p, _i, _i, _i, _f, _p],
@@ -50,6 +52,7 @@
     "ica_gather_images": [_p, _p, _p, _i, _l, _p],
     "ica_roi_prologue": [_p, _p, _p, _p, _i, _i, _i, _f, _i, _i, _i, _i, _f, _f, _p],
     "ica_roi_loss": [_p, _p, _p, _p, _p, _i, _i, _i, _i, _i, _i, _i, _f, _f, _i, _p],
+    "ica_roi_loss_live": [_p, _p, _p, _p, _p, _i, _i, _i, _i, _i, _i, _i, _f, _f, _i, _p, _p],
     "ica_roi_adam": [_p, _p, _p, _p, _p, _p, _p, _i, _i, _i, _f, _f, _f, _f, _p, _i, _i, _i, _i, _f, _f, _p, _p, _p],
     "ica_ifgsm_step": [_p, _p, _p, _p, _p, _i, _i, _i, _f, _f, _i, _p],
     "ica_l1_partial": [_p, _p, _i, _i, _i, _p],
@@ -163,7 +166,8 @@
     _fields_ = ([(n, C.c_void_p) for n in ("x", "y", "wp", "bias", "gp", "beta", "save_x", "save_s", "in_x", "in_s",
                                             "save_t", "res", "mask")]
                 + [(n, C.c_int) for n in ("N", "Cin", "Hin", "Win", "Cout", "Hout", "Wout", "kind", "KS", "S", "epi",
-                                           "it", "fill_mode", "ps", "prec", "layout", "order")])
+                                           "it", "fill_mode", "ps", "prec", "layout", "order")]
+                + [("live", C.c_void_p)])
 
 
 class ArArgs(C.Structure):
diff --git a/imagecompression_adversarial_amd/attack.py b/imagecompression_adversarial_amd/attack.py
--- a/imagecompression_adversarial_amd/attack.py
+++ b/imagecompression_adversarial_amd/attack.py
@@ -3,6 +3,7 @@
 import math
 import os
 import time
+import warnings
 from dataclasses import dataclass, field
 
 import torch
@@ -148,7 +149,8 @@
         self.sync_wait_s = 0.0
         self.graph_ok = (ATTACK_GRAPH and dev.type == "cuda" and att_metric == "L2"
                          and type(self).network_grad is AttackLoop.network_grad)
-        self._graph, self._graph_out = None, None
+        self._graphs = {}
+        self.live_ok = True
         self.graph_replays = 0
         if pad:
             self.output_s, self.bpp_ori = padded_eval_forward(kern, self.im_s, int(pad), padding_mode)
@@ -171,6 +173,21 @@
         bc2 = 1 - 0.999 ** t
         step_size = self.lrs[i] / bc1
         return float(bc2 ** 0.5), float(-step_size)
+
+    def _masked(self):
+        return self.compact and self.graph_ok and self.live_ok
+
+    def _network_step(self):
+        B = self.B
+        if self._masked():
+            call("ica_branch_select", ptr(self.loss_i), self.thr, B, ptr(self.sel), ptr(self.gpos), stream())
+            gx4 = self._network_graph(live=True)
+            if gx4 is not None:
+                return gx4, None
+        E, idx = self._select()
+        if E == B and idx is None and self.graph_ok:
+            return self._network_graph(), None
+        return (self.network_grad(idx, E) if E > 0 else None), idx
 
     def _select(self):
         B = self.B
@@ -219,11 +236,11 @@
         if self.roi is not None:
             x0, x1, y0, y1, _, _, wot, wob = self.roi
             out_t = self._gather(self.output_t, idx, Bn)
-            call("ica_roi_loss", ptr(xh4), ptr(out_s), ptr(out_t), ptr(grad4), ptr(part),
-                 Bn, H, W, x0, x1, y0, y1, wot, wob, int(self.clamp), stream())
+            call("ica_roi_loss_live", ptr(xh4), ptr(out_s), ptr(out_t), ptr(grad4), ptr(part),
+                 Bn, H, W, x0, x1, y0, y1, wot, wob, int(self.clamp), ptr(K.LIVE), stream())
         elif self.metric == "L2":
-            call("ica_attack_loss", ptr(xh4), ptr(out_s), ptr(grad4), ptr(part), Bn, H, W,
-                 self.gscale, int(self.clamp), 0, stream())
+            call("ica_attack_loss_live", ptr(xh4), ptr(out_s), ptr(grad4), ptr(part), Bn, H, W,
+                 self.gscale, int(self.clamp), 0, ptr(K.LIVE), stream())
         else:
             out = torch.empty_like(out_s)
             call("ica_nc4_bound_to_nchw", ptr(xh4), ptr(out), Bn, H, W, int(self.clamp), stream())
@@ -234,22 +251,31 @@
         del ss, xh4
         return kern.g_a_backward(gy4, sa)
 
-    def _network_graph(self):
-        if self._graph is None:
+    def _network_graph(self, live=False):
+        if live not in self._graphs:
             hooks = (K.EVENT_HOOK, K.LAUNCH_HOOK)
             K.EVENT_HOOK = K.LAUNCH_HOOK = None
             g = torch.cuda.CUDAGraph()
             try:
-                with torch.cuda.graph(g, capture_error_mode="relaxed"):
-                    out = self.network_grad(None, self.B)
+                with warnings.catch_warnings():
+                    if live:
+                        warnings.filterwarnings("ignore", message="The CUDA Graph is empty")
+                    with torch.cuda.graph(g, capture_error_mode="relaxed"), K.live_images(self.sel if live else None):
+                        out = self.network_grad(None, self.B)
+            except RuntimeError as e:
+                if live and "failed with status -4" in str(e):
+                    self.live_ok = False
+                    return None
+                raise
             finally:
                 K.EVENT_HOOK, K.LAUNCH_HOOK = hooks
-            self._graph, self._graph_out = g, out
+            self._graphs[live] = (g, out)
             GRAPH_STATS["captures"] += 1
-        self._graph.replay()
+        g, out = self._graphs[live]
+        g.replay()
         self.graph_replays += 1
         GRAPH_STATS["replays"] += 1
-        return self._graph_out
+        return out
 
     def step(self, i, record_im_in=False, census=False):
         B, H, W = self.B, self.H, self.W
@@ -260,13 +286,9 @@
         K.reduce_rows(self.part, B, self.invN, out=self.loss_i)
         if self.coupled:
             D.couple_loss_i(self.loss_i, self.B_global, self.group)
-        E, idx = self._select()
-        if E == B and idx is None and self.graph_ok:
-            gx4 = self._network_graph()
-        else:
-            gx4 = self.network_grad(idx, E) if E > 0 else None
+        gx4, idx = self._network_step()
         cheap_grad = None
-        if self.metric == "ms-ssim" and E < B:
+        if self.metric == "ms-ssim" and (idx is not None or gx4 is None):
             im_in = torch.empty_like(self.im_s)
             call("ica_nc4_bound_to_nchw", ptr(self.im_in4), ptr(im_in), B, H, W, 0, stream())
             _, _, gY = MS.ms_ssim_value_and_grad(self.im_s, im_in, torch.full((B,), -self.dval, device=im_in.device))
@@ -287,11 +309,7 @@
         call("ica_roi_prologue", ptr(self.noise), ptr(self.im_s), ptr(self.im_in4), ptr(self.part), B, H, W,
              self.eps, x0, x1, y0, y1, wit, wib, stream())
         K.reduce_rows(self.part, B, 1.0, out=self.loss_i)
-        E, idx = self._select()
-        if E == B and idx is None and self.graph_ok:
-            gx4 = self._network_graph()
-        else:
-            gx4 = self.network_grad(idx, E) if E > 0 else None
+        gx4, idx = self._network_step()
         bc2s, neg_step = self._adam_scalars(i)
         call("ica_roi_adam", ptr(self.noise), ptr(self.im_s), ptr(gx4), ptr(self.loss_i), ptr(self.m), ptr(self.v),
              ptr(self.im_in if record_im_in else None), B, H, W, self.eps, self.thr, bc2s, neg_step,
diff --git a/imagecompression_adversarial_amd/csrc/ica_conv.hip b/imagecompression_adversarial_amd/csrc/ica_conv.hip
--- a/imagecompression_adversarial_amd/csrc/ica_conv.hip
+++ b/imagecompression_adversarial_amd/csrc/ica_conv.hip
@@ -1238,7 +1238,8 @@
   constexpr int R = u3_rows<CT>(), NPX = u3_npx<CT>();
   __shared__ float zs[T3_ROWS * NPX];
   const int tiles_x = (p.Win + U3_OW - 1) / U3_OW, tiles_y = (p.Hin + R - 1) / R;
-  const int total = tiles_x * tiles_y * p.N;
+  const LiveList ll(p);
+  const int total = tiles_x * tiles_y * ll.count();
   const int nb = (int)(gridDim.x >> 3), xcd = (int)(blockIdx.x & 7), bi = (int)(blockIdx.x >> 3);
   const int q8 = total >> 3, r8 = total & 7;
   const int t_end = xcd * q8 + min(xcd, r8) + q8 + (xcd < r8 ? 1 : 0);
@@ -1252,7 +1253,7 @@
     const int tx = t % tiles_x, r = t / tiles_x;
     a0 = (r % tiles_y) * R;
     b0 = tx * U3_OW;
-    n = r / tiles_y;
+    n = ll.image(r / tiles_y);
   };
   const bool split_in = (p.pl & PL_IN) != 0;
   constexpr unsigned QB = BF ? 8u : 16u;
@@ -1878,6 +1879,7 @@
   int prec;
   int layout;
   int order;
+  const int* live;
 } ica_conv_args;
 
 int ica_conv_it(int cout) {
@@ -1980,14 +1982,16 @@
   return 0;
 }
 
-int ica_conv_up3(const float* x, float* y, const void* wp, const float* bias, int N, int Cin, int Hin, int Win,
-                 int layout, int prec, hipStream_t st) {
+int ica_conv_up3_live(const float* x, float* y, const void* wp, const float* bias, int N, int Cin, int Hin, int Win,
+                      int layout, int prec, const int* live, hipStream_t st) {
   if (Cin % 16 != 0) return -2;
   if (const int rc = up3_layout_ok(layout, Hin, Win)) return rc;
   if (prec < 0 || prec > 2) return -4;
+  if (live && !(prec == 2 && (Cin == 128 || Cin == 192))) return -4;
   ConvParams p{x, y, reinterpret_cast<const float*>(wp), bias, nullptr, nullptr, nullptr, nullptr, nullptr, nullptr,
                N, Cin, Hin, Win, 3, 2 * Hin, 2 * Win, nullptr};
   p.pl = layout;
+  p.live = live;
   auto tiled = [&](auto kern) {
     const int tiles = ((Win + T3_TW - 1) / T3_TW) * ((Hin + T3_TH - 1) / T3_TH) * N;
     ICA_LAUNCH(kern, dim3(tiles), dim3(256), 0, st, p);
@@ -2009,6 +2013,11 @@
   }
   ICA_CHECK_LAUNCH();
   return 0;
+}
+
+int ica_conv_up3(const float* x, float* y, const void* wp, const float* bias, int N, int Cin, int Hin, int Win,
+                 int layout, int prec, hipStream_t st) {
+  return ica_conv_up3_live(x, y, wp, bias, N, Cin, Hin, Win, layout, prec, nullptr, st);
 }
 
 __global__ void pack_gdn_bf16_kernel(const float* __restrict__ gamma, const float* __restrict__ beta,
@@ -2064,8 +2073,9 @@
 int ica_conv_ex(const ica_conv_args* a, hipStream_t st) {
   ConvParams p{a->x,    a->y,    a->wp,   a->bias, a->gp,   a->beta, a->save_x, a->save_s, a->in_x, a->in_s,
                a->N,    a->Cin,  a->Hin,  a->Win,  a->Cout, a->Hout, a->Wout,   a->save_t, a->res,  a->mask,
-               a->fill_mode, a->ps, a->prec, a->layout};
+               a->fill_mode, a->ps, a->prec, a->layout, a->live};
   if (a->prec < 0 || a->prec > 3) return -4;
+  if (a->live && !(a->prec == 2 && a->KS == 5 && a->S == 2)) return -4;
   if (a->layout & ~(PL_IN | PL_OUT)) return -4;
   if (a->layout && (a->KS != 5 || a->S != 2 || a->fill_mode != 0 || a->ps)) return -4;
   if (((a->layout & PL_IN) && ((a->Hin | a->Win) & 1)) || ((a->layout & PL_OUT) && ((a->Hout | a->Wout) & 1)))
diff --git a/imagecompression_adversarial_amd/csrc/ica_conv_epi.h b/imagecompression_adversarial_amd/csrc/ica_conv_epi.h
--- a/imagecompression_adversarial_amd/csrc/ica_conv_epi.h
+++ b/imagecompression_adversarial_amd/csrc/ica_conv_epi.h
@@ -32,8 +32,46 @@
   int ps;
   int prec;
   int pl;
+  const int* live;
 };
 enum { PL_IN = 1, PL_OUT = 2 };
+
+struct LiveList {
+  const int* live;
+  int N, lv;
+  ICA_DEV explicit LiveList(const ConvParams& p) : live(p.live), N(p.N), lv(0) {
+    if (live) lv = live[min((int)(threadIdx.x & 63), N)];
+  }
+  ICA_DEV int count() const {
+    return live ? (int)min((unsigned)__builtin_amdgcn_readlane(lv, 0), (unsigned)N) : N;
+  }
+  ICA_DEV int image(int v) const {
+    if (!live) return v;
+    const int n = v < 63 ? __builtin_amdgcn_readlane(lv, 1 + v) : __builtin_amdgcn_readfirstlane(live[1 + v]);
+    return (int)min((unsigned)n, (unsigned)N - 1u);
+  }
+};
+ICA_DEV bool xcd_block_first(unsigned total, unsigned nx, int& bx, int& by) {
+  const unsigned lin = blockIdx.y * gridDim.x + blockIdx.x;
+  if (lin >= total) return false;
+  const unsigned q = total >> 3, r = total & 7, x = lin & 7;
+  const unsigned L = x * q + (x < r ? x : r) + (lin >> 3);
+  bx = (int)(L % nx);
+  by = (int)(L / nx);
+  return true;
+}
+ICA_DEV bool live_block(const LiveList& ll, int& bx, int& by) {
+  if (!ll.live) {
+    xcd_block<true>(bx, by);
+    return true;
+  }
+  const unsigned nx = gridDim.x / (unsigned)ll.N * (unsigned)ll.count();
+  return xcd_block_first(nx * gridDim.y, nx, bx, by);
+}
+ICA_DEV int live_walk_blocks(const LiveList& ll, int total, int WPB) {
+  const int nblk = (int)gridDim.x;
+  return ll.live ? min(nblk, (total + WPB - 1) / WPB) : nblk;
+}
 enum { ORDER_DOWN = 0, ORDER_UP = 1, ORDER_RGB5 = 2, ORDER_TG = 3 };
 
 ICA_DEV void split3(f32x4 v, u32x2& hi, u32x2& mid, u32x2& lo) {
diff --git a/imagecompression_adversarial_amd/csrc/ica_conv_x6.hip b/imagecompression_adversarial_amd/csrc/ica_conv_x6.hip
--- a/imagecompression_adversarial_amd/csrc/ica_conv_x6.hip
+++ b/imagecompression_adversarial_amd/csrc/ica_conv_x6.hip
@@ -23,11 +23,12 @@
   __shared__ f32x4 patch[3 * 2 * PLANE];
   const int tiles_x = (p.Wout + TW - 1) / TW, tiles_y = (p.Hout + TH - 1) / TH;
   int bid, cb;
-  xcd_block<true>(bid, cb);
+  const LiveList ll(p);
+  if (!live_block(ll, bid, cb)) return;
   const int tx = bid % tiles_x;
   bid /= tiles_x;
   const int ty = bid % tiles_y;
-  const int n = bid / tiles_y;
+  const int n = ll.image(bid / tiles_y);
   const int lane = threadIdx.x & 63, wave = threadIdx.x >> 6, h = lane >> 5, j = lane & 31;
   if constexpr (CS == 2) cb = __builtin_amdgcn_readfirstlane(wave >> 1);
   auto trow = [&](int t) { return CS == 1 ? wave * PT + t : 2 * (wave & 1) + (j >> 4); };
@@ -340,11 +341,12 @@
   __shared__ f32x4 lds[(2 * BUF > XCH) ? 2 * BUF : XCH];
   const int tiles_x = (p.Wout + TW - 1) / TW, tiles_y = (p.Hout + TH - 1) / TH;
   int bid, cb;
-  xcd_block<true>(bid, cb);
+  const LiveList ll(p);
+  if (!live_block(ll, bid, cb)) return;
   const int tx = bid % tiles_x;
   bid /= tiles_x;
   const int ty = bid % tiles_y;
-  const int n = bid / tiles_y;
+  const int n = ll.image(bid / tiles_y);
   const int lane = threadIdx.x & 63, h = lane >> 5, j = lane & 31;
   const int wave = __builtin_amdgcn_readfirstlane(threadIdx.x >> 6);
   const int rp = wave & 3, chh = wave >> 2;
@@ -705,15 +707,18 @@
 __global__ __launch_bounds__(512, 1) void conv_rgb5_x6_kernel(ConvParams p, long ps, int nblk) {
   extern __shared__ __attribute__((aligned(16))) char rgb5_lds[];
   constexpr bool GDN = EPI == EPI_GDN || EPI == EPI_IGDN;
+  const LiveList ll(p);
+  const int tiles_x = (p.Wout + 31) / 32, total = tiles_x * p.Hout * ll.count();
+  nblk = live_walk_blocks(ll, total, 8);
+  int b, cb;
+  if (!xcd_block_first(nblk, nblk, b, cb)) return;
   rgb5_stage<GDN>(p, ps, rgb5_lds);
-  const int tiles_x = (p.Wout + 31) / 32, total = tiles_x * p.Hout * p.N, per = (total + nblk - 1) / nblk;
-  int b, cb;
-  xcd_block<true>(b, cb);
+  const int per = (total + nblk - 1) / nblk;
   const int t_end = min(total, b * per + per), wave = __builtin_amdgcn_readfirstlane(threadIdx.x >> 6);
 #pragma unroll 1
   for (int t = b * per + wave; t < t_end; t += 8) {
     const int tx = t % tiles_x, r = t / tiles_x;
-    const int oy = r % p.Hout, n = r / p.Hout, ox = tx * 32 + (threadIdx.x & 31);
+    const int oy = r % p.Hout, n = ll.image(r / p.Hout), ox = tx * 32 + (threadIdx.x & 31);
     const bool valid = ox < p.Wout;
     f32x4 q[RGB5_KY][3];
     rgb5_load(p, n, oy, ox, valid, q);
@@ -787,15 +792,18 @@
 __global__ __launch_bounds__(256, 1) void conv_rgb5_bwd_x6_kernel(ConvParams p, long ps, int nblk) {
   extern __shared__ __attribute__((aligned(16))) char rgb5_lds[];
   static_assert(EPI == EPI_IGDN_BWD || EPI == EPI_GDN_BWD, "GDN-backward epilogues");
+  const LiveList ll(p);
+  const int tiles_x = (p.Wout + 31) / 32, total = tiles_x * p.Hout * ll.count();
+  nblk = live_walk_blocks(ll, total, 4);
+  int b, cb;
+  if (!xcd_block_first(nblk, nblk, b, cb)) return;
   rgb5_stage<true>(p, ps, rgb5_lds);
-  const int tiles_x = (p.Wout + 31) / 32, total = tiles_x * p.Hout * p.N, per = (total + nblk - 1) / nblk;
-  int b, cb;
-  xcd_block<true>(b, cb);
+  const int per = (total + nblk - 1) / nblk;
   const int t_end = min(total, b * per + per), wave = __builtin_amdgcn_readfirstlane(threadIdx.x >> 6);
   auto coords = [&](int t, int& n, int& oy, int& ox) {
     const int tx = t % tiles_x, r = t / tiles_x;
     oy = r % p.Hout;
-    n = r / p.Hout;
+    n = ll.image(r / p.Hout);
     ox = tx * 32 + (threadIdx.x & 31);
   };
   int t = b * per + wave;
@@ -902,11 +910,12 @@
   extern __shared__ f32x4 patch[];
   const int tiles_x = (p.Win + XU_TW - 1) / XU_TW, tiles_y = (p.Hin + XU_TH - 1) / XU_TH;
   int bid, cb;
-  xcd_block<true>(bid, cb);
+  const LiveList ll(p);
+  if (!live_block(ll, bid, cb)) return;
   const int tx = bid % tiles_x;
   bid /= tiles_x;
   const int ty = bid % tiles_y;
-  const int n = bid / tiles_y;
+  const int n = ll.image(bid / tiles_y);
   const int a0 = ty * XU_TH, b0 = tx * XU_TW;
   const int Cin4 = p.Cin >> 2, nch = p.Cin / 16, ngrp = p.Cin / CG;
   const unsigned xplane = (unsigned)p.Hin * p.Win;
@@ -1162,11 +1171,12 @@
   extern __shared__ f32x4 patch[];
   const int tiles_x = (p.Win + XU_TW - 1) / XU_TW, tiles_y = (p.Hin + XU_TH - 1) / XU_TH;
   int bid, cb;
-  xcd_block<true>(bid, cb);
+  const LiveList ll(p);
+  if (!live_block(ll, bid, cb)) return;
   const int tx = bid % tiles_x;
   bid /= tiles_x;
   const int ty = bid % tiles_y;
-  const int n = bid / tiles_y;
+  const int n = ll.image(bid / tiles_y);
   const int a0 = ty * XU_TH, b0 = tx * XU_TW;
   const int Cin4 = p.Cin >> 2, nch = p.Cin / 16, ngrp = p.Cin / CG;
   const unsigned xplane = (unsigned)p.Hin * p.Win;
@@ -1298,11 +1308,12 @@
   __shared__ f32x4 red[xs_red_entries<IT>()];
   const int tiles_x = (p.Wout + TW - 1) / TW, tiles_y = (p.Hout + TH - 1) / TH;
   int bid, cb;
-  xcd_block<true>(bid, cb);
+  const LiveList ll(p);
+  if (!live_block(ll, bid, cb)) return;
   const int tx = bid % tiles_x;
   bid /= tiles_x;
   const int ty = bid % tiles_y;
-  const int n = bid / tiles_y;
+  const int n = ll.image(bid / tiles_y);
   const int lane = threadIdx.x & 63, wave = __builtin_amdgcn_readfirstlane(threadIdx.x >> 6), h = lane >> 5,
             j = lane & 31;
   const int oy0 = ty * TH, ox0 = tx * TW, iy0 = oy0 * S - PAD, ix0 = ox0 * S - PAD;
@@ -1397,13 +1408,14 @@
   extern __shared__ f32x4 patch[];
   const int tiles_x = (p.Win + TW - 1) / TW, tiles_y = (p.Hin + XSU_TH - 1) / XSU_TH;
   int bid, cb;
-  xcd_block<true>(bid, cb);
+  const LiveList ll(p);
+  if (!live_block(ll, bid, cb)) return;
   const int cls = bid & 3;
   bid >>= 2;
   const int tx = bid % tiles_x;
   bid /= tiles_x;
   const int ty = bid % tiles_y;
-  const int n = bid / tiles_y;
+  const int n = ll.image(bid / tiles_y);
   const int a0 = ty * XSU_TH, b0 = tx * TW;
   const int Cin4 = p.Cin >> 2, nch = p.Cin / 16, NQ8 = p.Cin / 8;
   const unsigned xplane = (unsigned)p.Hin * p.Win;
diff --git a/imagecompression_adversarial_amd/csrc/ica_elem.hip b/imagecompression_adversarial_amd/csrc/ica_elem.hip
--- a/imagecompression_adversarial_amd/csrc/ica_elem.hip
+++ b/imagecompression_adversarial_amd/csrc/ica_elem.hip
@@ -75,11 +75,18 @@
   if (threadIdx.x == 0) part[(long)b * gridDim.x + blockIdx.x] = r;
 }
 
+ICA_DEV int live_slot_image(const int* __restrict__ live, unsigned v, unsigned B) {
+  if (!live) return (int)v;
+  if (v >= min((unsigned)live[0], B)) return -1;
+  return (int)min((unsigned)live[1 + v], B - 1u);
+}
+
 __global__ void attack_loss_kernel(const float* __restrict__ xhat4, const float* __restrict__ out_s,
                                    float* __restrict__ grad4, float* __restrict__ part, long HW, float invN,
-                                   int clamp, int mode) {
-  __shared__ float sh[4];
-  const int b = blockIdx.y;
+                                   int clamp, int mode, const int* __restrict__ live) {
+  __shared__ float sh[4];
+  const int b = live_slot_image(live, blockIdx.y, gridDim.y);
+  if (b < 0) return;
   const float* x4 = xhat4 + (long)b * 4 * HW;
   const float* os = out_s + (long)b * 3 * HW;
   float* g4 = grad4 + (long)b * 4 * HW;
@@ -138,9 +145,10 @@
 
 __global__ void roi_loss_kernel(const float* __restrict__ xhat4, const float* __restrict__ out_s,
                                 const float* __restrict__ out_t, float* __restrict__ grad4, float* __restrict__ part,
-                                long HW, long W, RoiBox roi, int clamp) {
-  __shared__ float sh[4];
-  const int b = blockIdx.y;
+                                long HW, long W, RoiBox roi, int clamp, const int* __restrict__ live) {
+  __shared__ float sh[4];
+  const int b = live_slot_image(live, blockIdx.y, gridDim.y);
+  if (b < 0) return;
   const float* x4 = xhat4 + (long)b * 4 * HW;
   const float* os = out_s + (long)b * 3 * HW;
   const float* ot = out_t + (long)b * 3 * HW;
@@ -578,12 +586,17 @@
   return ica_attack_prologue_ex(noise, im_s, im_in4, part, B, H, W, eps, 1, st);
 }
 
+int ica_attack_loss_live(const float* xhat4, const float* out_s, float* grad4, float* part, int B, int H, int W,
+                         float invN, int clamp, int mode, const int* live, hipStream_t st) {
+  ICA_LAUNCH(attack_loss_kernel, dim3(ELEM_BLOCKS_PER_IMAGE, B), dim3(256), 0, st, xhat4, out_s, grad4, part,
+                     (long)H * W, invN, clamp, mode, live);
+  ICA_CHECK_LAUNCH();
+  return 0;
+}
+
 int ica_attack_loss(const float* xhat4, const float* out_s, float* grad4, float* part, int B, int H, int W,
                     float invN, int clamp, int mode, hipStream_t st) {
-  ICA_LAUNCH(attack_loss_kernel, dim3(ELEM_BLOCKS_PER_IMAGE, B), dim3(256), 0, st, xhat4, out_s, grad4, part,
-                     (long)H * W, invN, clamp, mode);
-  ICA_CHECK_LAUNCH();
-  return 0;
+  return ica_attack_loss_live(xhat4, out_s, grad4, part, B, H, W, invN, clamp, mode, nullptr, st);
 }
 
 int ica_attack_adam_ex(float* noise, const float* im_s, const float* gnet4, const float* loss_i,
@@ -613,13 +626,20 @@
   return 0;
 }
 
+int ica_roi_loss_live(const float* xhat4, const float* out_s, const float* out_t, float* grad4, float* part, int B,
+                      int H, int W, int x0, int x1, int y0, int y1, float w_out_tar, float w_out_bkg, int clamp,
+                      const int* live, hipStream_t st) {
+  const RoiBox roi{x0, x1, y0, y1, 0.f, 0.f, w_out_tar, w_out_bkg};
+  ICA_LAUNCH(roi_loss_kernel, dim3(ELEM_BLOCKS_PER_IMAGE, B), dim3(256), 0, st, xhat4, out_s, out_t, grad4,
+                     part, (long)H * W, (long)W, roi, clamp, live);
+  ICA_CHECK_LAUNCH();
+  return 0;
+}
+
 int ica_roi_loss(const float* xhat4, const float* out_s, const float* out_t, float* grad4, float* part, int B, int H,
                  int W, int x0, int x1, int y0, int y1, float w_out_tar, float w_out_bkg, int clamp, hipStream_t st) {
-  const RoiBox roi{x0, x1, y0, y1, 0.f, 0.f, w_out_tar, w_out_bkg};
-  ICA_LAUNCH(roi_loss_kernel, dim3(ELEM_BLOCKS_PER_IMAGE, B), dim3(256), 0, st, xhat4, out_s, out_t, grad4,
-                     part, (long)H * W, (long)W, roi, clamp);
-  ICA_CHECK_LAUNCH();
-  return 0;
+  return ica_roi_loss_live(xhat4, out_s, out_t, grad4, part, B, H, W, x0, x1, y0, y1, w_out_tar, w_out_bkg, clamp,
+                           nullptr, st);
 }
 
 int ica_roi_adam(float* noise, const float* im_s, const float* gnet4, const float* loss_i, float* m, float* v,
diff --git a/imagecompression_adversarial_amd/hip_ops.py b/imagecompression_adversarial_amd/hip_ops.py
--- a/imagecompression_adversarial_amd/hip_ops.py
+++ b/imagecompression_adversarial_amd/hip_ops.py
@@ -93,6 +93,32 @@
 
 
 FLOPS_HOOK = {}
+
+LIVE = None
+
+
+class live_images:
+
+    def __init__(self, sel):
+        if sel is not None and (sel.dtype != torch.int32 or not sel.is_cuda or not sel.is_contiguous()):
+            raise RuntimeError("live-image list: a contiguous int32 device tensor [N + 1]")
+        self.sel = sel
+
+    def __enter__(self):
+        global LIVE
+        self.prev, LIVE = LIVE, self.sel
+        return self
+
+    def __exit__(self, *exc):
+        global LIVE
+        LIVE = self.prev
+        return False
+
+
+def _live(N):
+    if LIVE is not None and LIVE.numel() < N + 1:
+        raise RuntimeError(f"live-image list of {LIVE.numel()} entries for a batch of {N}")
+    return LIVE
 
 
 def _dev_check(t: torch.Tensor, name="tensor"):
@@ -381,7 +407,8 @@
     N, _, H, W, _ = x4.shape
     y = out if out is not None else empty_nc4(N, 3, 2 * H, 2 * W, x4.device)
     ev = _ev_begin(_prec_note(tag, wp.prec), N)
-    call("ica_conv_up3", ptr(x4), ptr(y), ptr(wp.data), ptr(bias), N, Cin, H, W, int(layout), int(wp.prec), stream())
+    call("ica_conv_up3_live", ptr(x4), ptr(y), ptr(wp.data), ptr(bias), N, Cin, H, W, int(layout), int(wp.prec),
+         ptr(_live(N)), stream())
     _ev_end(ev)
     return y, None, None
 
@@ -425,7 +452,8 @@
             gp = gdn.gpT if epi in (EPI_GDN_BWD, EPI_IGDN_BWD) else gdn.gp
     a = ConvArgs(ptr(x4), ptr(y), ptr(wp.data), ptr(bias), ptr(gp), ptr(None if gdn is None else gdn.beta),
                  ptr(save_x), ptr(save_s), ptr(in_x), ptr(in_s), ptr(save_t), ptr(res), ptr(mask), N, Cin, H, W, Cout,
-                 Ho, Wo, kind, KS, S, epi, wp.it, fill_mode, int(bool(ps)), prec, int(layout), wp.order)
+                 Ho, Wo, kind, KS, S, epi, wp.it, fill_mode, int(bool(ps)), prec, int(layout), wp.order,
+                 ptr(_live(N)))
     import ctypes
     tag = _prec_note(tag, prec)
     ev = _ev_begin(tag, N)
diff --git a/include/ica_hip.h b/include/ica_hip.h
--- a/include/ica_hip.h
+++ b/include/ica_hip.h
@@ -104,6 +104,7 @@
   int prec;
   int layout;
   int order;
+  const int* live;
 } ica_conv_args;
 int ica_conv_ex(const ica_conv_args* args, hipStream_t stream);
 int ica_last_launch(char* name, int cap, unsigned long long* threads);
@@ -112,6 +113,8 @@
 int ica_pack_up3(const float* w, void* dst, int Cin, int prec, hipStream_t stream);
 int ica_conv_up3(const float* x, float* y, const void* wp, const float* bias, int N, int Cin, int Hin, int Win,
                  int layout, int prec, hipStream_t stream);
+int ica_conv_up3_live(const float* x, float* y, const void* wp, const float* bias, int N, int Cin, int Hin, int Win,
+                      int layout, int prec, const int* live, hipStream_t stream);
 
 int ica_elem_blocks_per_image(void);
 int ica_nchw_to_nc4(const float* src, float* dst, int N, int C, int H, int W, hipStream_t stream);
@@ -123,6 +126,8 @@
                            float eps, int clamp_in, hipStream_t stream);
 int ica_attack_loss(const float* xhat4, const float* out_s, float* grad4, float* part, int B, int H, int W,
                     float invN, int clamp, int mode, hipStream_t stream);
+int ica_attack_loss_live(const float* xhat4, const float* out_s, float* grad4, float* part, int B, int H, int W,
+                         float invN, int clamp, int mode, const int* live, hipStream_t stream);
 int ica_attack_adam(float* noise, const float* im_s, const float* gnet4, const float* loss_i, const float* cheap_grad,
                     float* m, float* v, float* im_in_out, int B, int H, int W, float eps, float thr, float invN,
                     float bc2s, float neg_step, int* branch, const int* gpos, int* census, hipStream_t stream);
@@ -141,6 +146,9 @@
                      int x0, int x1, int y0, int y1, float w_in_tar, float w_in_bkg, hipStream_t stream);
 int ica_roi_loss(const float* xhat4, const float* out_s, const float* out_t, float* grad4, float* part, int B, int H,
                  int W, int x0, int x1, int y0, int y1, float w_out_tar, float w_out_bkg, int clamp, hipStream_t stream);
+int ica_roi_loss_live(const float* xhat4, const float* out_s, const float* out_t, float* grad4, float* part, int B,
+                      int H, int W, int x0, int x1, int y0, int y1, float w_out_tar, float w_out_bkg, int clamp,
+                      const int* live, hipStream_t stream);
 int ica_roi_adam(float* noise, const float* im_s, const float* gnet4, const float* loss_i, float* m, float* v,
                  float* im_in_out, int B, int H, int W, float eps, float thr, float bc2s, float neg_step, int* branch,
                  int x0, int x1, int y0, int y1, float w_in_tar, float w_in_bkg, const int* gpos, int* census,
```

After: 1565 attack-step·images/s. About the same (-0.3%).
